# NVIDIA/vid2vid

Measured on AMD Instinct MI355X. Metric: synthesized frames/sec (Vid2VidModelG.inference, 512x256), higher is better.
Workload: dtype bf16; 1 GPU; label2city 512x256 inference, n_scales_spatial=1, --fg --use_instance, ngf=128 n_blocks=9 (411.3M params random-init, 2115 GFLOP/frame as dense convolutions, of which the 2 one-hot label stems (266 GFLOP dense) run as exact weight gather-sums), batch 1 per sequence, 1 sequence per GPU; launches_per_frame=113, hipgraph=True, graph_lanes=3, paired_launches=True, tile_selection=profiles/tune_cache.json, world_size=1, parallelism=replicas x1 (independent sequences, no collective), output_finite=True

## Files before the change

### include/v2v_hip.h

```cpp
#ifndef V2V_HIP_H
#define V2V_HIP_H

#include <stdint.h>

#ifdef __cplusplus
extern "C" {
#endif

#define V2V_EINVAL (-1)

#define V2V_F32  0
#define V2V_BF16 1

#define V2V_PAD_ZERO    0
#define V2V_PAD_REFLECT 1

#define V2V_ACT_NONE    0
#define V2V_ACT_RELU    1
#define V2V_ACT_LEAKY   2
#define V2V_ACT_TANH    3
#define V2V_ACT_SIGMOID 4

#define V2V_OUT_RAW_F32_NHWC 0
#define V2V_OUT_ACT_NHWC     1
// ... 376 lines not shown
int       v2v_plan_run(v2v_plan* p, void* stream);
int       v2v_plan_instantiate_graph(v2v_plan* p, void* stream);
int       v2v_plan_launch_graph(v2v_plan* p, void* stream);
int       v2v_plan_segment_program(const v2v_plan* p, int32_t* steps, int32_t max_steps, int32_t* seg_of_op, int32_t n_ops);
int       v2v_plan_profile(v2v_plan* p, void* stream, float* ms, int32_t n);
int       v2v_plan_timeline(v2v_plan* p, void* stream, float* t0_ms, float* t1_ms, int32_t* lanes, int32_t n);
int       v2v_plan_timeline_graph(v2v_plan* p, void* stream, float* t0_ms, float* t1_ms, int32_t* lanes, int32_t n);
const char* v2v_plan_op_name(const v2v_plan* p, int32_t i);
int       v2v_plan_op_lane(const v2v_plan* p, int32_t i);
int       v2v_plan_set_label(v2v_plan* p, const char* label);
const char* v2v_plan_op_label(const v2v_plan* p, int32_t i);
int       v2v_plan_set_lane(int32_t lane);
int       v2v_plan_lane_wait(int32_t waiter, int32_t signal);

int v2v_tensor2im(const float* x, uint8_t* out, int32_t C, int32_t H, int32_t W, int32_t normalize, void* stream);
int v2v_frames_u8(const float* frames, uint8_t* out, const int32_t* mode, const int32_t* row_slot, int32_t K, int32_t S,
                  int32_t C, int32_t H, int32_t W, int32_t normalize, void* stream);
int v2v_label_image(const void* labels, const void* inst, int32_t in_u8, const uint8_t* cmap, int32_t label_nc, uint8_t* out,
                    const int32_t* mode, const int32_t* row_slot, int32_t K, int32_t S, int32_t T, int32_t H, int32_t W,
                    void* stream);
int v2v_tensor2flow(const float* flow, uint8_t* out, uint32_t* range_ws, int32_t H, int32_t W, void* stream);
int v2v_tensor2label(const float* x, uint8_t* out, const uint8_t* cmap, int32_t n_label, int32_t C, int32_t H, int32_t W,
                     void* stream);

int     v2v_label_codes(const void* labels, const void* inst, int32_t in_u8, uint8_t* codes, int32_t T, int32_t H, int32_t W,
                        int32_t label_nc, void* stream);
int64_t v2v_onehot_conv_table_bytes(int32_t cin, int32_t cout, int32_t dtype, int32_t slice, int32_t T, int32_t label_nc);
int     v2v_onehot_conv_pack_weights(const float* w, void* table, int32_t cin, int32_t cout, int32_t dtype, int32_t slice,
                                     int32_t T, int32_t label_nc, void* stream);
int     v2v_onehot_conv_stats_rows(int32_t H, int32_t W);
int     v2v_onehot_conv7x7(const void* labels, const void* inst, int32_t in_u8, const void* table, const float* bias,
                           float* out, float* stats, int32_t T, int32_t H, int32_t W, int32_t label_nc,
                           int32_t cout, int32_t cout_stride, int32_t dtype, int32_t slice, void* stream);
typedef struct v2v_onehot_norm {
    int32_t* counter;
    const float* gamma;
    const float* beta;
    float* scale_shift;
    float* running_mean;
    float* running_var;
    float eps, momentum;
    int64_t count;
} v2v_onehot_norm;
int     v2v_onehot_conv7x7_norm(const void* labels, const void* inst, int32_t in_u8, const void* table, const float* bias,
                                float* out, float* stats, int32_t T, int32_t H, int32_t W, int32_t label_nc,
                                int32_t cout, int32_t cout_stride, int32_t dtype, int32_t slice, const v2v_onehot_norm* fin,
                                void* stream);
int     v2v_onehot_conv7x7_batch(const void* labels, const void* inst, int32_t in_u8, const void* table, const float* bias,
                                 float* out, float* stats, int32_t N, int32_t T, int32_t H, int32_t W, int32_t label_nc,
                                 int32_t cout, int32_t cout_stride, int32_t dtype, int32_t slice, void* stream);
int     v2v_onehot_conv_ppt(int32_t N, int32_t T, int32_t H, int32_t W, int32_t label_nc, int32_t has_inst,
                            int32_t cout, int32_t dtype, int32_t slice);

int v2v_memcpy_d2d(void* dst, const void* src, int64_t bytes, void* stream);

int         v2v_set_dry_run(int32_t on);
int         v2v_get_dry_run(void);

int         v2v_version(void);
const char* v2v_last_error(void);
int         v2v_device_status(int32_t clear);
int         v2v_device_info(int32_t* cus, int32_t* lds_per_cu, int64_t* hbm_bytes, char* arch, int32_t arch_len);

#ifdef __cplusplus
}
#endif
#endif
```

### vid2vid_amd/csrc/label_image.hip

```cpp
#include "v2v_internal.h"

namespace v2v {

struct LabelImageArgs {
    const void* labels; const void* inst; const unsigned char* cmap; unsigned char* out;
    const int* mode; const int* row_slot;
    int K, S, T, H, W, label_nc, planes;
};

static constexpr int LABEL_IMAGE_GRID_CAP = 256;

__device__ __forceinline__ int label_image_row(const LabelImageArgs& a, int s) {
    for (int k = 0; k < a.K; ++k) {
        if ((a.row_slot ? a.row_slot[k] : k) != s) continue;
        const int m = a.mode ? a.mode[k] : 0;
        if (m == 0 || m == 1) return k;
    }
    return -1;
}

template <typename T, int R>
__device__ __forceinline__ void load_run(const T* p, int n, T (&v)[R]) {
    constexpr int BYTES = R * (int)sizeof(T);
    constexpr int VB = BYTES < 16 ? 4 : 16;
    static_assert(BYTES % VB == 0, "whole vectors");
    if (n == R && (reinterpret_cast<uintptr_t>(p) & (VB - 1)) == 0) {
        if constexpr (VB == 4) {
            const unsigned w = *reinterpret_cast<const unsigned*>(p);
            __builtin_memcpy(v, &w, 4);
        } else {
            uint4 w[BYTES / 16];
#pragma unroll
            for (int i = 0; i < BYTES / 16; ++i) w[i] = reinterpret_cast<const uint4*>(p)[i];
            __builtin_memcpy(v, w, BYTES);
        }
    } else {
#pragma unroll
        for (int i = 0; i < R; ++i) v[i] = i < n ? p[i] : T(0);
    }
}

template <typename LT, typename IT, int R>
__global__ __launch_bounds__(256) void label_image_kernel(const LabelImageArgs a) {
    constexpr int NW = 3 * R / 4;
    constexpr unsigned BLACK = 255;
    __shared__ unsigned pal[256];
    {
        const int c = threadIdx.x;
        unsigned w = 0;
        if (c < a.label_nc) w = a.cmap[3 * c] | ((unsigned)a.cmap[3 * c + 1] << 8) | ((unsigned)a.cmap[3 * c + 2] << 16);
        pal[c] = w;
    }
    __syncthreads();
    const int s = blockIdx.y;
    const int row = label_image_row(a, s);
    const long long hw = (long long)a.H * a.W;
    const int rpr = (a.W + R - 1) / R;
    const long long runs = (long long)a.H * rpr;
    const long long stride = (long long)gridDim.x * blockDim.x;
    const long long frame = ((long long)(row < 0 ? 0 : row) * a.T + (a.T - 1)) * hw;
    const LT* const labels = reinterpret_cast<const LT*>(a.labels) + frame;
    const IT* const inst = a.inst ? reinterpret_cast<const IT*>(a.inst) + frame : nullptr;
    unsigned char* const out = a.out + (long long)s * hw * 3;
    for (long long r = (long long)blockIdx.x * blockDim.x + threadIdx.x; r < runs; r += stride) {
        const int y = (int)(r / rpr);
        const int x0 = (int)(r - (long long)y * rpr) * R;
        const int n = a.W - x0 < R ? a.W - x0 : R;
        const long long p0 = (long long)y * a.W + x0;
        unsigned w[NW + 1];
#pragma unroll
        for (int j = 0; j <= NW; ++j) w[j] = 0u;
        if (row >= 0) {
            LT lab[R];
            load_run<LT, R>(labels + p0, n, lab);
            int idx[R];
            bool outside = false;
#pragma unroll
            for (int i = 0; i < R; ++i) {
                idx[i] = (int)lab[i];
                outside |= i < n && (idx[i] < 0 || idx[i] >= a.label_nc);
            }
            bool edge[R];
#pragma unroll
            for (int i = 0; i < R; ++i) edge[i] = false;
            if (inst && outside) {
                IT c[R], up[R], dn[R];
                load_run<IT, R>(inst + p0, n, c);
                const bool has_up = y > 0, has_dn = y + 1 < a.H, has_l = x0 > 0, has_r = x0 + n < a.W;
                if (has_up) load_run<IT, R>(inst + p0 - a.W, n, up);
                if (has_dn) load_run<IT, R>(inst + p0 + a.W, n, dn);
                const IT lft = has_l ? inst[p0 - 1] : IT(0);
                const IT rgt = has_r ? inst[p0 + n] : IT(0);
#pragma unroll
                for (int i = 0; i < R; ++i) {
                    bool e = false;
                    if (i > 0) e |= c[i - 1] != c[i];
                    else       e |= has_l && lft != c[0];
                    if (i + 1 < n)       e |= c[(i + 1) % R] != c[i];
                    else if (i + 1 == n) e |= has_r && rgt != c[i];
                    if (has_up) e |= up[i] != c[i];
                    if (has_dn) e |= dn[i] != c[i];
                    edge[i] = e;
                }
            }
#pragma unroll
            for (int i = 0; i < R; ++i) {
                unsigned k;
                if (a.planes == 1) k = idx[i] == 0 ? BLACK : 0u;
                else if (idx[i] >= 0 && idx[i] < a.label_nc) k = (unsigned)idx[i];
                else k = edge[i] ? BLACK : 0u;
                const unsigned col = i < n ? pal[k] : 0u;
                const int word = (3 * i) >> 2, sh = ((3 * i) & 3) * 8;
                w[word] |= col << sh;
                if (sh > 8) w[word + 1] |= col >> (32 - sh);
            }
        }
        unsigned char* const dst = out + p0 * 3;
        const int nbytes = 3 * n;
        const uintptr_t addr = reinterpret_cast<uintptr_t>(dst);
        if (R == 16 && n == R && (addr & 15) == 0) {
#pragma unroll
            for (int j = 0; j < NW / 4; ++j)
                reinterpret_cast<uint4*>(dst)[j] = make_uint4(w[4 * j], w[4 * j + 1], w[4 * j + 2], w[4 * j + 3]);
        } else {
            int head = (int)((4 - (addr & 3)) & 3);
            if (head > nbytes) head = nbytes;
#pragma unroll
            for (int b = 0; b < 3; ++b)
                if (b < head) dst[b] = (unsigned char)(w[0] >> (8 * b));
            const int nd = (nbytes - head) >> 2, tail = (nbytes - head) & 3;
            unsigned* const dw = reinterpret_cast<unsigned*>(dst + head);
#pragma unroll
            for (int j = 0; j < NW; ++j) {
                const unsigned v = __builtin_amdgcn_alignbyte(w[j + 1], w[j], (unsigned)head);
                if (j < nd) dw[j] = v;
                else if (j == nd) {
#pragma unroll
                    for (int b = 0; b < 3; ++b)
                        if (b < tail) dst[head + 4 * nd + b] = (unsigned char)(v >> (8 * b));
                }
            }
        }
    }
}

struct LabelImageOp : Op {
    LabelImageArgs a; int in_u8;
    template <typename LT, typename IT>
    void go(hipStream_t s) {
        const dim3 b(256);
        if (a.W >= 16) {
            long long gx = ceil_div((long long)a.H * ceil_div(a.W, 16), 256);
            if (gx > LABEL_IMAGE_GRID_CAP) gx = LABEL_IMAGE_GRID_CAP;
            hipLaunchKernelGGL((label_image_kernel<LT, IT, 16>), dim3((unsigned)gx, (unsigned)a.S), b, 0, s, a);
        } else {
            long long gx = ceil_div((long long)a.H * ceil_div(a.W, 4), 256);
            if (gx > LABEL_IMAGE_GRID_CAP) gx = LABEL_IMAGE_GRID_CAP;
            hipLaunchKernelGGL((label_image_kernel<LT, IT, 4>), dim3((unsigned)gx, (unsigned)a.S), b, 0, s, a);
        }
    }
    int launch(hipStream_t s) override {
        if (in_u8) go<unsigned char, int>(s);
        else       go<float, float>(s);
        return check_launch();
    }
    const char* name() const override { return "label_image"; }
};

static bool ranges_overlap(const void* p, long long pb, const void* q, long long qb) {
    const char* a = (const char*)p; const char* b = (const char*)q;
    return p && q && a < b + qb && b < a + pb;
}

}

using namespace v2v;

extern "C" int v2v_label_image(const void* labels, const void* inst, int32_t in_u8, const uint8_t* cmap, int32_t label_nc,
                               uint8_t* out, const int32_t* mode, const int32_t* row_slot, int32_t K, int32_t S, int32_t T,
                               int32_t H, int32_t W, void* stream) {
    if (!labels || !cmap || !out) { set_error("label_image: null pointer"); return V2V_EINVAL; }
    if (label_nc < 1 || label_nc > 255) {
        set_error("label_image: label_nc %d (1..255: the palette and its black entry are 256 words of LDS)", label_nc); return V2V_EINVAL;
    }
    if ((in_u8 != 0 && in_u8 != 1) || K < 1 || S < K || S > 65535 || T < 1 || H < 1 || W < 1 ||
        (long long)K * T * H * W > 0x7fffffffffffll) {
        set_error("label_image: bad argument (1 <= K <= S <= 65535 rows / images, T, H, W >= 1)"); return V2V_EINVAL;
    }
    if (!row_slot && K != S) { set_error("label_image: without row_slot row k is image k: K == S"); return V2V_EINVAL; }
    const int lsize = in_u8 ? 1 : 4;
    if ((((uintptr_t)labels & (lsize - 1)) | ((uintptr_t)inst & 3) | ((uintptr_t)mode & 3) | ((uintptr_t)row_slot & 3)) != 0) {
        set_error("label_image: misaligned buffer (fp32 labels, inst, mode and row_slot are 4-byte aligned)"); return V2V_EINVAL;
    }
    const long long hw = (long long)H * W;
    const long long out_bytes = (long long)S * hw * 3, in_elems = (long long)K * T * hw;
    if (ranges_overlap(out, out_bytes, labels, in_elems * lsize) || ranges_overlap(out, out_bytes, inst, in_elems * 4) ||
        ranges_overlap(out, out_bytes, cmap, 3ll * label_nc) || ranges_overlap(out, out_bytes, mode, 4ll * K) ||
        ranges_overlap(out, out_bytes, row_slot, 4ll * K)) {
        set_error("label_image: out must not overlap an input"); return V2V_EINVAL;
    }
    auto op = std::make_unique<LabelImageOp>();
    op->a = LabelImageArgs{labels, inst, cmap, out, mode, row_slot, K, S, T, H, W, label_nc, label_nc + (inst ? 1 : 0)};
    op->in_u8 = in_u8;
    return submit(std::move(op), stream);
}
```

### vid2vid_amd/csrc/pointwise.hip

```cpp
#include "v2v_internal.h"
#include "layout_vec.h"

namespace v2v {

static inline unsigned grid_for(long long n, int threads = 256, long long cap = 4096) {
    long long b = ceil_div(n, threads);
    if (b > cap) b = cap;
    if (b < 1) b = 1;
    return (unsigned)b;
}

struct EncodeArgs {
    const void* labels; const void* inst; void* out; float* mask;
    int T, H, W, label_nc, c_stride; const int* fg; int n_fg;
};

template <typename T, typename LT, typename IT>
__global__ __launch_bounds__(256) void encode_labels_kernel(const EncodeArgs a) {
    constexpr int VEC = ElemTraits<T>::VEC;
    const int vpr = a.c_stride / VEC;
    const long long hw = (long long)a.H * a.W;
    const long long nvec = hw * vpr;
    const int per_frame = a.label_nc + (a.inst ? 1 : 0);
    const long long stride = (long long)gridDim.x * blockDim.x;
// ... 275 lines not shown
            const int c = cv * VEC + q;
            vals[q] = c < a.C ? a.x[(n * a.C + c) * hw + pix] : 0.f;
        }
        store_vec(y, pixg * a.c_stride + cv * VEC, vals);
    }
}

template <typename T>
__global__ __launch_bounds__(256) void unpack_nhwc_to_nchw_kernel(const PackArgs2 a) {
    constexpr int VEC = ElemTraits<T>::VEC;
    const int vpr = (a.C + VEC - 1) / VEC;
    const long long hw = (long long)a.H * a.W;
    const long long npix = (long long)a.N * hw;
    const long long nvec = npix * vpr;
    const long long stride = (long long)gridDim.x * blockDim.x;
    const T* y = reinterpret_cast<const T*>(a.y);
    float* x = const_cast<float*>(a.x);
    for (long long v = (long long)blockIdx.x * blockDim.x + threadIdx.x; v < nvec; v += stride) {
        const long long pixg = v % npix;
        const int cv = (int)(v / npix);
        const long long n = pixg / hw, pix = pixg - n * hw;
        float vals[VEC];
        load_vec(y, pixg * a.c_stride + cv * VEC, vals);
#pragma unroll
        for (int q = 0; q < VEC; ++q) {
            const int c = cv * VEC + q;
            if (c < a.C) x[(n * a.C + c) * hw + pix] = vals[q];
        }
    }
}

struct LayoutOp : Op {
    PackArgs2 a; int dtype; bool pack;
    int launch(hipStream_t s) override {
        const int vec = dtype == V2V_BF16 ? 8 : 4;
        const long long n = (long long)a.N * a.H * a.W * (pack ? (a.c_stride / vec) : ((a.C + vec - 1) / vec));
        if (pack) {
            if (dtype == V2V_BF16) hipLaunchKernelGGL(pack_nchw_to_nhwc_kernel<bf16_t>, dim3(grid_for(n)), dim3(256), 0, s, a);
            else                   hipLaunchKernelGGL(pack_nchw_to_nhwc_kernel<float>, dim3(grid_for(n)), dim3(256), 0, s, a);
        } else {
            if (dtype == V2V_BF16) hipLaunchKernelGGL(unpack_nhwc_to_nchw_kernel<bf16_t>, dim3(grid_for(n)), dim3(256), 0, s, a);
            else                   hipLaunchKernelGGL(unpack_nhwc_to_nchw_kernel<float>, dim3(grid_for(n)), dim3(256), 0, s, a);
        }
        return check_launch();
    }
    const char* name() const override { return pack ? "pack_nchw_to_nhwc" : "unpack_nhwc_to_nchw"; }
};

struct PrologueArgs {
    const void* labels; const void* inst; unsigned char* codes; float* mask; const int* fg; int n_fg;
    const float* window; void* packed; float* last;
    int T, H, W, label_nc, win_C, c_stride, last_C;
    int N = 1;
};

template <typename T, typename LT, typename IT>
__device__ __forceinline__ void frame_prologue_row(const PrologueArgs& a, long long nb, long long wrow, unsigned block_dim,
                                                   unsigned grid_dim) {
    constexpr int VEC = ElemTraits<T>::VEC;
    const long long hw = (long long)a.H * a.W;
    const long long ncode = hw * a.T;
    const int vpr = a.window ? a.c_stride / VEC : 0;
    const long long total = ncode + hw * vpr;
    const long long stride = (long long)grid_dim * block_dim;
    const LT* labels = reinterpret_cast<const LT*>(a.labels) + nb * ncode;
    const IT* inst = a.inst ? reinterpret_cast<const IT*>(a.inst) + nb * ncode : nullptr;
    unsigned char* codes = a.codes + nb * ncode;
    float* mask = a.mask ? a.mask + nb * hw : nullptr;
    const float* window = a.window ? a.window + wrow * a.win_C * hw : nullptr;
    float* last = a.last ? a.last + nb * a.last_C * hw : nullptr;
    T* y = reinterpret_cast<T*>(a.packed) + nb * hw * a.c_stride;
    for (long long e = (long long)blockIdx.x * block_dim + threadIdx.x; e < total; e += stride) {
        if (e < ncode) {
            const long long t = e / hw, q = e - t * hw;
            const int lab = (int)labels[e];
            bool edge = false;
            if (inst) {
                const int py = (int)(q / a.W), px = (int)(q - (long long)py * a.W);
                const IT* ip = inst + t * hw;
                const IT ctr = ip[q];
                if (px > 0)       edge |= ip[q - 1] != ctr;
                if (px < a.W - 1) edge |= ip[q + 1] != ctr;
                if (py > 0)       edge |= ip[q - a.W] != ctr;
                if (py < a.H - 1) edge |= ip[q + a.W] != ctr;
            }
            codes[e] = (unsigned char)(((unsigned)lab < (unsigned)a.label_nc ? lab : 127) | (edge ? 128 : 0));
            if (mask && t == a.T - 1) {
                float m = 0.f;
                for (int i = 0; i < a.n_fg; ++i) m += (a.fg[i] == lab) ? 1.f : 0.f;
                mask[q] = fminf(fmaxf(m, 0.f), 1.f);
            }
        } else {
            const long long v = e - ncode;
            window_pack_item<T>(window, y, last, v % hw, (int)(v / hw), hw, a.win_C, a.c_stride, a.last_C);
        }
    }
}

template <typename T, typename LT, typename IT, bool BATCH>
__global__ __launch_bounds__(256) void frame_prologue_kernel(const PrologueArgs a) {
    const long long nb = BATCH ? (long long)blockIdx.y : 0ll;
    frame_prologue_row<T, LT, IT>(a, nb, nb, blockDim.x, gridDim.x);
}

struct PrologueOp : Op {
    PrologueArgs a; int dtype; int in_u8;
    int launch(hipStream_t s) override {
        const int vec = dtype == V2V_BF16 ? 8 : 4;
        const long long hw = (long long)a.H * a.W;
        const dim3 g(grid_for(hw * a.T + (a.window ? hw * (a.c_stride / vec) : 0)), (unsigned)a.N), b(256);
        if (a.N > 1) return go<true>(g, b, s);
        return go<false>(g, b, s);
    }
    template <bool BATCH> int go(dim3 g, dim3 b, hipStream_t s) {
        if (in_u8) {
            if (dtype == V2V_BF16) hipLaunchKernelGGL((frame_prologue_kernel<bf16_t, unsigned char, int, BATCH>), g, b, 0, s, a);
            else                   hipLaunchKernelGGL((frame_prologue_kernel<float, unsigned char, int, BATCH>), g, b, 0, s, a);
        } else {
            if (dtype == V2V_BF16) hipLaunchKernelGGL((frame_prologue_kernel<bf16_t, float, float, BATCH>), g, b, 0, s, a);
            else                   hipLaunchKernelGGL((frame_prologue_kernel<float, float, float, BATCH>), g, b, 0, s, a);
        }
        return check_launch();
    }
    const char* name() const override { return "frame_prologue"; }
};

struct ProloguePoolArgs { PrologueArgs p; const int* row_slot; int S; };

template <typename T, typename LT, typename IT>
__global__ __launch_bounds__(256) void frame_prologue_pool_kernel(const ProloguePoolArgs s) {
    const PrologueArgs& a = s.p;
    const int slot = s.row_slot[blockIdx.y];
    if (slot < 0 || slot >= s.S) return;
    __builtin_assume(a.window != nullptr);
    frame_prologue_row<T, LT, IT>(a, blockIdx.y, slot, blockDim.x, gridDim.x);
}

struct ProloguePoolOp : Op {
    ProloguePoolArgs a; int dtype; int in_u8;
    int launch(hipStream_t s) override {
        const int vec = dtype == V2V_BF16 ? 8 : 4;
        const long long hw = (long long)a.p.H * a.p.W;
        const dim3 g(grid_for(hw * a.p.T + hw * (a.p.c_stride / vec)), (unsigned)a.p.N), b(256);
        if (in_u8) {
            if (dtype == V2V_BF16) hipLaunchKernelGGL((frame_prologue_pool_kernel<bf16_t, unsigned char, int>), g, b, 0, s, a);
            else                   hipLaunchKernelGGL((frame_prologue_pool_kernel<float, unsigned char, int>), g, b, 0, s, a);
        } else {
            if (dtype == V2V_BF16) hipLaunchKernelGGL((frame_prologue_pool_kernel<bf16_t, float, float>), g, b, 0, s, a);
            else                   hipLaunchKernelGGL((frame_prologue_pool_kernel<float, float, float>), g, b, 0, s, a);
        }
        return check_launch();
    }
    const char* name() const override { return "frame_prologue_pool"; }
};

struct PoolArgs { const void* x; void* y; long long planes; int N, H, W, OH, OW, c_stride; };

__global__ __launch_bounds__(256) void avgpool_planar_kernel(const PoolArgs a) {
    const float* x = reinterpret_cast<const float*>(a.x);
    float* y = reinterpret_cast<float*>(a.y);
    const long long total = a.planes * a.OH * a.OW;
    const long long stride = (long long)gridDim.x * blockDim.x;
    for (long long e = (long long)blockIdx.x * blockDim.x + threadIdx.x; e < total; e += stride) {
        const int ox = (int)(e % a.OW);
        const long long t = e / a.OW;
        const int oy = (int)(t % a.OH);
        const long long pl = t / a.OH;
        const float* xp = x + pl * (long long)a.H * a.W;
        float s = 0.f; int cnt = 0;
#pragma unroll
        for (int dy = -1; dy <= 1; ++dy) {
            const int iy = 2 * oy + dy;
            if (iy < 0 || iy >= a.H) continue;
#pragma unroll
            for (int dx = -1; dx <= 1; ++dx) {
                const int ix = 2 * ox + dx;
                if (ix < 0 || ix >= a.W) continue;
                s += xp[(long long)iy * a.W + ix];
                ++cnt;
            }
        }
        y[e] = s / (float)cnt;
    }
}

template <typename T>
__global__ __launch_bounds__(256) void avgpool_nhwc_kernel(const PoolArgs a) {
    constexpr int VEC = ElemTraits<T>::VEC;
// ... 43 lines not shown
            pk.w = pack_bf16x2(s[6] / fc, s[7] / fc);
            *reinterpret_cast<uint4*>(o) = pk;
        }
    }
}

struct PoolOp : Op {
    PoolArgs a; int dtype; bool planar;
    int launch(hipStream_t s) override {
        if (planar) {
            hipLaunchKernelGGL(avgpool_planar_kernel, dim3(grid_for(a.planes * a.OH * a.OW)), dim3(256), 0, s, a);
        } else {
            const long long n = (long long)a.N * a.OH * a.OW * (a.c_stride / (dtype == V2V_BF16 ? 8 : 4));
            if (dtype == V2V_BF16) hipLaunchKernelGGL(avgpool_nhwc_kernel<bf16_t>, dim3(grid_for(n)), dim3(256), 0, s, a);
            else                   hipLaunchKernelGGL(avgpool_nhwc_kernel<float>, dim3(grid_for(n)), dim3(256), 0, s, a);
        }
        return check_launch();
    }
    const char* name() const override { return planar ? "avgpool3s2_planar" : "avgpool3s2_nhwc"; }
};

__device__ __forceinline__ float unnormalize(float coord, int size, int align_corners) {
    if (align_corners) return ((coord + 1.f) / 2.f) * (float)(size - 1);
    return ((coord + 1.f) * (float)size - 1.f) / 2.f;
}

__device__ __forceinline__ void bilinear_setup(float fx, float fy, float gxv, float gyv, int H, int W, int ac,
                                               int& x0, int& y0, float& wx, float& wy) {
    const float nx = gxv + fx / (((float)W - 1.0f) / 2.0f);
    const float ny = gyv + fy / (((float)H - 1.0f) / 2.0f);
    float ix = unnormalize(nx, W, ac), iy = unnormalize(ny, H, ac);
    ix = fminf((float)(W - 1), fmaxf(ix, 0.f));
    iy = fminf((float)(H - 1), fmaxf(iy, 0.f));
    const float fx0 = floorf(ix), fy0 = floorf(iy);
    x0 = (int)fx0; y0 = (int)fy0;
    wx = ix - fx0; wy = iy - fy0;
}

__device__ __forceinline__ float bilinear_fetch(const float* img, int H, int W, int x0, int y0, float wx, float wy) {
    const int x1 = x0 + 1, y1 = y0 + 1;
    const bool xin = x1 < W, yin = y1 < H;
    const float nw = img[(long long)y0 * W + x0];
    const float ne = xin ? img[(long long)y0 * W + x1] : 0.f;
    const float sw = yin ? img[(long long)y1 * W + x0] : 0.f;
    const float se = (xin && yin) ? img[(long long)y1 * W + x1] : 0.f;
    return nw * ((1.f - wx) * (1.f - wy)) + ne * (wx * (1.f - wy)) + sw * ((1.f - wx) * wy) + se * (wx * wy);
}

struct WarpArgs {
    float* img_raw; const float* flow; const float* weight; const float* prev; const float* fg; const float* mask;
    float* img_final; float* img_warp; const float* gx; const float* gy;
    int N, C, H, W, align_corners;
    float* roll = nullptr; int roll_slots = 0;
};

__device__ __forceinline__ void warp_blend_pixel(const WarpArgs& a, long long n, long long pix, bool do_warp, float* win) {
    const long long hw = (long long)a.H * a.W;
    const int y = (int)(pix / a.W), x = (int)(pix - (long long)y * a.W);
    int x0 = 0, y0 = 0; float wx = 0.f, wy = 0.f;
    float wgt = 1.f;
    if (do_warp) {
        const float fx = a.flow[(n * 2 + 0) * hw + pix], fy = a.flow[(n * 2 + 1) * hw + pix];
        bilinear_setup(fx, fy, a.gx[x], a.gy[y], a.H, a.W, a.align_corners, x0, y0, wx, wy);
        wgt = a.weight[n * hw + pix];
    }
    const float m = a.fg ? a.mask[n * hw + pix] : 0.f;
    for (int c = 0; c < a.C; ++c) {
        const long long o = (n * a.C + c) * hw + pix;
        float raw = a.img_raw[o];
        float fin = raw;
        if (do_warp) {
            const float wv = bilinear_fetch(a.prev + (n * a.C + c) * hw, a.H, a.W, x0, y0, wx, wy);
            if (a.img_warp) a.img_warp[o] = wv;
            fin = raw * wgt + wv * (1.f - wgt);
        }
        if (a.fg) {
            const float f = a.fg[o];
            fin = f * m + fin * (1.f - m);
            raw = f * m + raw * (1.f - m);
            a.img_raw[o] = raw;
        }
        a.img_final[o] = fin;
        if (win) {
            float* w = win + c * hw + pix;
            const long long slot = (long long)a.C * hw;
            for (int k = 0; k + 1 < a.roll_slots; ++k) w[k * slot] = w[(k + 1) * slot];
            w[(a.roll_slots - 1) * slot] = fin;
        }
    }
}

__device__ __forceinline__ float* warp_row_window(const WarpArgs& a, long long n) {
    return a.roll ? a.roll + n * a.roll_slots * a.C * a.H * a.W : nullptr;
}

template <bool ROLLB>
__global__ __launch_bounds__(256) void warp_blend_kernel(const WarpArgs a) {
    const long long hw = (long long)a.H * a.W;
    const long long total = (long long)a.N * hw;
    const long long stride = (long long)gridDim.x * blockDim.x;
    for (long long e = (long long)blockIdx.x * blockDim.x + threadIdx.x; e < total; e += stride) {
        const long long n = e / hw;
        warp_blend_pixel(a, n, e - n * hw, a.flow != nullptr, ROLLB ? warp_row_window(a, n) : a.roll);
    }
}

struct WarpOp : Op {
    WarpArgs a;
    int launch(hipStream_t s) override {
        const dim3 g(grid_for((long long)a.N * a.H * a.W));
        if (a.roll && a.N > 1) hipLaunchKernelGGL(warp_blend_kernel<true>, g, dim3(256), 0, s, a);
        else                   hipLaunchKernelGGL(warp_blend_kernel<false>, g, dim3(256), 0, s, a);
        return check_launch();
    }
    const char* name() const override { return "warp_blend"; }
};

struct WarpSlotArgs { WarpArgs w; const int* mode; };

__global__ __launch_bounds__(256) void warp_blend_slots_kernel(const WarpSlotArgs s) {
    const WarpArgs& a = s.w;
    const long long hw = (long long)a.H * a.W;
    const long long total = (long long)a.N * hw;
    const long long stride = (long long)gridDim.x * blockDim.x;
    for (long long e = (long long)blockIdx.x * blockDim.x + threadIdx.x; e < total; e += stride) {
        const long long n = e / hw, pix = e - n * hw;
        const int md = s.mode[n];
        if (md != 0 && md != 1) {
            for (int c = 0; c < a.C; ++c) a.img_final[(n * a.C + c) * hw + pix] = 0.f;
            continue;
        }
        warp_blend_pixel(a, n, pix, a.flow != nullptr && md == 0, warp_row_window(a, n));
    }
}

struct WarpSlotsOp : Op {
    WarpSlotArgs a;
    int launch(hipStream_t s) override {
        hipLaunchKernelGGL(warp_blend_slots_kernel, dim3(grid_for((long long)a.w.N * a.w.H * a.w.W)), dim3(256), 0, s, a);
        return check_launch();
    }
    const char* name() const override { return "warp_blend_slots"; }
};

struct WindowRollArgs { float* window; const float* frame; const int* mode; long long frame_elems; int N, slots; };

__global__ __launch_bounds__(256) void window_roll_slots_kernel(const WindowRollArgs a) {
    const long long total = (long long)a.N * a.frame_elems;
    const long long stride = (long long)gridDim.x * blockDim.x;
    for (long long e = (long long)blockIdx.x * blockDim.x + threadIdx.x; e < total; e += stride) {
        const long long n = e / a.frame_elems, r = e - n * a.frame_elems;
        const int md = a.mode[n];
        if (md != 0 && md != 1) continue;
        float* w = a.window + n * a.slots * a.frame_elems + r;
        for (int k = 0; k + 1 < a.slots; ++k) w[k * a.frame_elems] = w[(k + 1) * a.frame_elems];
        w[(a.slots - 1) * a.frame_elems] = a.frame[e];
    }
}

struct WindowRollOp : Op {
    WindowRollArgs a;
    int launch(hipStream_t s) override {
        hipLaunchKernelGGL(window_roll_slots_kernel, dim3(grid_for((long long)a.N * a.frame_elems)), dim3(256), 0, s, a);
        return check_launch();
    }
// ... 613 lines not shown
extern "C" int v2v_avgpool3s2_nhwc(const void* x, void* y, int32_t N, int32_t H, int32_t W, int32_t c_stride,
                                   int32_t dtype, void* stream) {
    if (!x || !y || c_stride % (dtype == V2V_BF16 ? 8 : 4) != 0) { set_error("avgpool: null pointer or a channel stride that is not whole 16-byte vectors"); return V2V_EINVAL; }
    auto op = std::make_unique<PoolOp>();
    op->a = PoolArgs{x, y, 0, N, H, W, (H - 1) / 2 + 1, (W - 1) / 2 + 1, c_stride}; op->planar = false; op->dtype = dtype;
    return submit(std::move(op), stream);
}

extern "C" int v2v_warp_blend(float* img_raw, const float* flow, const float* weight, const float* prev,
                              const float* fg, const float* mask, float* img_final, float* img_warp,
                              const float* gx, const float* gy,
                              int32_t N, int32_t C, int32_t H, int32_t W, int32_t align_corners, void* stream) {
    if (!img_raw || !img_final || (flow && (!weight || !prev || !gx || !gy)) || (fg && !mask)) {
        set_error("warp_blend: bad argument"); return V2V_EINVAL;
    }
    auto op = std::make_unique<WarpOp>();
    op->a = WarpArgs{img_raw, flow, weight, prev, fg, mask, img_final, img_warp, gx, gy, N, C, H, W, align_corners};
    return submit(std::move(op), stream);
}

static bool warp_roll_args_ok(const char* who, const WarpArgs& a, bool need_window, long long win_rows, const char* what) {
    if (!a.img_raw || !a.img_final || (a.flow && (!a.weight || !a.prev || !a.gx || !a.gy)) || (a.fg && !a.mask) ||
        (need_window && !a.roll) || (a.roll && a.roll_slots < 1) || a.N < 1 || win_rows < 1 || a.C < 1 || a.H < 1 || a.W < 1) {
        set_error("%s: bad argument", who); return false;
    }
    if (!a.roll) return true;
    const float* wend = a.roll + win_rows * a.roll_slots * a.C * a.H * a.W;
    const long long frame = (long long)a.N * a.C * a.H * a.W;
    auto overlaps = [&](const float* p) { return p && p + frame > a.roll && p < wend; };
    if (overlaps(a.prev) || overlaps(a.img_final) || overlaps(a.img_raw) || overlaps(a.fg)) {
        set_error("%s: the %s must not overlap the gather source or the frame buffers", who, what); return false;
    }
    return true;
}

extern "C" int v2v_warp_blend_roll(float* img_raw, const float* flow, const float* weight, const float* prev,
                                   const float* fg, const float* mask, float* img_final, float* img_warp,
                                   const float* gx, const float* gy, float* window, int32_t slots,
                                   int32_t C, int32_t H, int32_t W, int32_t align_corners, void* stream) {
    return v2v_warp_blend_roll_batch(img_raw, flow, weight, prev, fg, mask, img_final, img_warp, gx, gy, window, slots, 1, C, H, W,
                                     align_corners, stream);
}

extern "C" int v2v_warp_blend_roll_batch(float* img_raw, const float* flow, const float* weight, const float* prev,
                                         const float* fg, const float* mask, float* img_final, float* img_warp,
                                         const float* gx, const float* gy, float* window, int32_t slots,
                                         int32_t N, int32_t C, int32_t H, int32_t W, int32_t align_corners, void* stream) {
    auto op = std::make_unique<WarpOp>();
    op->a = WarpArgs{img_raw, flow, weight, prev, fg, mask, img_final, img_warp, gx, gy, N, C, H, W, align_corners, window, slots};
    if (!warp_roll_args_ok("warp_blend_roll", op->a, true, N, "rolled window")) return V2V_EINVAL;
    return submit(std::move(op), stream);
}

extern "C" int v2v_warp_blend_slots(float* img_raw, const float* flow, const float* weight, const float* prev,
                                    const float* fg, const float* mask, float* img_final, float* img_warp,
                                    const float* gx, const float* gy, float* window, int32_t slots, const int32_t* mode,
                                    int32_t N, int32_t C, int32_t H, int32_t W, int32_t align_corners, void* stream) {
    if (!mode) { set_error("warp_blend_slots: null mode"); return V2V_EINVAL; }
    auto op = std::make_unique<WarpSlotsOp>();
    op->a.w = WarpArgs{img_raw, flow, weight, prev, fg, mask, img_final, img_warp, gx, gy, N, C, H, W, align_corners, window, slots};
    op->a.mode = mode;
    if (!warp_roll_args_ok("warp_blend_slots", op->a.w, false, N, "rolled window")) return V2V_EINVAL;
    if (!window) op->a.w.roll_slots = 0;
    return submit(std::move(op), stream);
}

extern "C" int v2v_window_roll_slots(float* window, const float* frame, const int32_t* mode, int32_t N, int32_t slots,
                                     int32_t C, int32_t H, int32_t W, void* stream) {
    if (!mode) { set_error("window_roll_slots: null mode"); return V2V_EINVAL; }
    if (!window || !frame || N < 1 || slots < 1 || C < 1 || H < 1 || W < 1) {
        set_error("window_roll_slots: bad argument"); return V2V_EINVAL;
    }
    const long long elems = (long long)C * H * W;
    if (frame + N * elems > window && frame < window + (long long)N * slots * elems) {
        set_error("window_roll_slots: the frame must not overlap the window"); return V2V_EINVAL;
    }
    auto op = std::make_unique<WindowRollOp>();
    op->a = WindowRollArgs{window, frame, mode, elems, N, slots};
    return submit(std::move(op), stream);
}

extern "C" int v2v_warp_blend_pool(float* img_raw, const float* flow, const float* weight, const float* prev,
                                   const float* fg, const float* mask, float* img_final, float* img_warp,
                                   const float* gx, const float* gy, float* window, int32_t slots, const int32_t* mode,
                                   const int32_t* row_slot, int32_t K, int32_t S, int32_t C, int32_t H, int32_t W,
                                   int32_t align_corners, void* stream) {
    if (!mode || !row_slot) { set_error("warp_blend_pool: null %s", !mode ? "mode" : "row_slot"); return V2V_EINVAL; }
    auto op = std::make_unique<WarpPoolOp>();
    op->a.w = WarpArgs{img_raw, flow, weight, prev, fg, mask, img_final, img_warp, gx, gy, K, C, H, W, align_corners, window, slots};
    op->a.mode = mode; op->a.row_slot = row_slot; op->a.S = S;
    if (K > 65535) { set_error("warp_blend_pool: bad argument"); return V2V_EINVAL; }
    if (!warp_roll_args_ok("warp_blend_pool", op->a.w, true, S, "pool")) return V2V_EINVAL;
    return submit(std::move(op), stream);
}

static int window_pool_copy(const char* what, float* dst, const float* src, bool scatter, const int32_t* row_slot, int32_t K,
                            int32_t S, int32_t slots, int32_t C, int32_t H, int32_t W, void* stream) {
    if (!dst || !src || !row_slot || K < 1 || K > 65535 || S < 1 || slots < 1 || C < 1 || H < 1 || W < 1) {
        set_error("%s: null pointer or bad argument", what); return V2V_EINVAL;
    }
    const long long elems = (long long)slots * C * H * W;
    const float* dense = scatter ? src : dst; const float* pool = scatter ? dst : src;
    if (dense + K * elems > pool && dense < pool + S * elems) {
        set_error("%s: dense and pool must not overlap", what); return V2V_EINVAL;
    }
    auto op = std::make_unique<WindowPoolOp>();
    op->a = WindowPoolArgs{dst, src, row_slot, elems, K, S}; op->scatter = scatter;
    return submit(std::move(op), stream);
}

extern "C" int v2v_window_gather_pool(float* dense, const float* pool, const int32_t* row_slot, int32_t K, int32_t S, int32_t slots,
                                      int32_t C, int32_t H, int32_t W, void* stream) {
    return window_pool_copy("window_gather_pool", dense, pool, false, row_slot, K, S, slots, C, H, W, stream);
}

extern "C" int v2v_window_scatter_pool(float* pool, const float* dense, const int32_t* row_slot, int32_t K, int32_t S, int32_t slots,
                                       int32_t C, int32_t H, int32_t W, void* stream) {
    return window_pool_copy("window_scatter_pool", pool, dense, true, row_slot, K, S, slots, C, H, W, stream);
}

static bool prologue_args_ok(const char* who, const PrologueArgs& a, int in_u8, int dtype) {
    const int vec = dtype == V2V_BF16 ? 8 : 4;
    if (!a.labels || !a.codes || a.T < 1 || a.H < 1 || a.W < 1 || a.label_nc < 1 || a.label_nc > 126 || (in_u8 != 0 && in_u8 != 1) ||
        (dtype != V2V_F32 && dtype != V2V_BF16) || a.n_fg < 0 || (a.mask && a.n_fg > 0 && !a.fg) ||
        (in_u8 ? ((uintptr_t)a.inst & 3) != 0 : (((uintptr_t)a.labels | (uintptr_t)a.inst) & 3) != 0)) {
        set_error("%s: bad argument (label_nc <= 126)", who); return false;
    }
    if (a.window && (!a.packed || a.win_C < 1 || a.c_stride % vec != 0 || a.win_C > a.c_stride || ((uintptr_t)a.packed & 15) != 0 ||
                     (a.last && (a.last_C < 1 || a.last_C > a.win_C)))) {
        set_error("%s: bad window pack argument", who); return false;
    }
    return true;
}

extern "C" int v2v_frame_prologue(const void* labels, const void* inst, int32_t in_u8, uint8_t* codes, float* mask,
                                  const int32_t* fg_labels_dev, int32_t n_fg, int32_t T, int32_t H, int32_t W, int32_t label_nc,
                                  const float* window, int32_t win_C, void* packed, int32_t c_stride, float* last, int32_t last_C,
                                  int32_t dtype, void* stream) {
    return v2v_frame_prologue_batch(labels, inst, in_u8, codes, mask, fg_labels_dev, n_fg, 1, T, H, W, label_nc, window, win_C, packed,
                                    c_stride, last, last_C, dtype, stream);
}

extern "C" int v2v_frame_prologue_batch(const void* labels, const void* inst, int32_t in_u8, uint8_t* codes, float* mask,
                                        const int32_t* fg_labels_dev, int32_t n_fg, int32_t N, int32_t T, int32_t H, int32_t W,
                                        int32_t label_nc, const float* window, int32_t win_C, void* packed, int32_t c_stride,
                                        float* last, int32_t last_C, int32_t dtype, void* stream) {
    if (N < 1 || N > 65535) { set_error("frame_prologue: bad sample count %d", N); return V2V_EINVAL; }
    auto op = std::make_unique<PrologueOp>();
    op->a = PrologueArgs{labels, inst, codes, mask, fg_labels_dev, n_fg, window, packed, last,
                         T, H, W, label_nc, win_C, c_stride, last_C, N};
    op->dtype = dtype; op->in_u8 = in_u8;
    if (!prologue_args_ok("frame_prologue", op->a, in_u8, dtype)) return V2V_EINVAL;
    if (!window) op->a.packed = op->a.last = nullptr;
    return submit(std::move(op), stream);
}

extern "C" int v2v_frame_prologue_pool(const void* labels, const void* inst, int32_t in_u8, uint8_t* codes, float* mask,
                                       const int32_t* fg_labels_dev, int32_t n_fg, int32_t K, int32_t T, int32_t H, int32_t W,
                                       int32_t label_nc, const float* window, int32_t S, const int32_t* row_slot, int32_t win_C,
                                       void* packed, int32_t c_stride, float* last, int32_t last_C, int32_t dtype, void* stream) {
    if (!row_slot || !window) { set_error("frame_prologue_pool: null %s", !row_slot ? "row_slot" : "window"); return V2V_EINVAL; }
    if (K < 1 || K > 65535 || S < 1) { set_error("frame_prologue_pool: bad row count %d / pool size %d", K, S); return V2V_EINVAL; }
    auto op = std::make_unique<ProloguePoolOp>();
    op->a.p = PrologueArgs{labels, inst, codes, mask, fg_labels_dev, n_fg, window, packed, last,
                           T, H, W, label_nc, win_C, c_stride, last_C, K};
    op->a.row_slot = row_slot; op->a.S = S;
    op->dtype = dtype; op->in_u8 = in_u8;
    if (!prologue_args_ok("frame_prologue_pool", op->a.p, in_u8, dtype)) return V2V_EINVAL;
    return submit(std::move(op), stream);
}

extern "C" int v2v_resample_flow(const float* img, const float* flow, float* out, const float* gx, const float* gy,
                                 int32_t N, int32_t C, int32_t H, int32_t W, int32_t align_corners, void* stream) {
    if (!img || !flow || !out || !gx || !gy) { set_error("resample_flow: null"); return V2V_EINVAL; }
    auto op = std::make_unique<ResampleOp>();
    op->a = ResampleArgs{img, flow, out, gx, gy, N, C, H, W, align_corners};
    return submit(std::move(op), stream);
}

extern "C" int v2v_add_nhwc(const void* a, const void* b, void* y, int64_t n_elems, int32_t dtype, void* stream) {
    const int vec = dtype == V2V_BF16 ? 8 : 4;
    if (!a || !b || !y || n_elems % vec != 0) { set_error("add: bad argument"); return V2V_EINVAL; }
    auto op = std::make_unique<AddOp>();
    op->a = AddArgs{a, b, y, n_elems / vec}; op->dtype = dtype;
    return submit(std::move(op), stream);
}

extern "C" int v2v_fg_mask_nhwc(const void* x, float* mask, int64_t P, int32_t c_stride, int32_t base_ch,
                                const int32_t* fg_labels_dev, int32_t n_fg, int32_t dtype, void* stream) {
    if (!x || !mask || !fg_labels_dev || n_fg <= 0) { set_error("fg_mask: bad argument"); return V2V_EINVAL; }
    auto op = std::make_unique<FgMaskOp>();
    op->a = FgMaskArgs{x, mask, P, c_stride, base_ch, fg_labels_dev, n_fg}; op->dtype = dtype;
    return submit(std::move(op), stream);
}

extern "C" int v2v_pack_concat_nhwc(const float* x0, int32_t C0, const float* x1, int32_t C1, float scale1, void* y,
                                    int32_t N, int32_t H, int32_t W, int32_t c_stride, int32_t dtype, void* stream) {
    const int vec = dtype == V2V_BF16 ? 8 : 4;
    if (!x0 || !y || (C1 > 0 && !x1) || c_stride % vec != 0 || C0 + C1 > c_stride) { set_error("pack_concat: bad argument"); return V2V_EINVAL; }
    auto op = std::make_unique<Pack2Op>();
    op->a = Pack2Args{x0, x1, y, N, C0, C1 > 0 ? C1 : 0, H, W, c_stride, scale1}; op->dtype = dtype;
    return submit(std::move(op), stream);
}

extern "C" int v2v_unpack_channels_nchw(const void* y, float* x, int32_t N, int32_t C, int32_t H, int32_t W,
                                        int32_t c_stride, int32_t c_offset, int32_t dtype, void* stream) {
// ... 45 lines not shown
```

### vid2vid_amd/csrc/v2v_internal.h

```cpp
#pragma once
#include <hip/hip_runtime.h>
#include <stdint.h>
#include <string>
#include <vector>
#include <memory>
#include "../../include/v2v_hip.h"

namespace v2v {

typedef __bf16 bf16_t;
typedef __attribute__((ext_vector_type(8)))  __bf16 bf16x8;
typedef __attribute__((ext_vector_type(4)))  float  f32x4;
typedef __attribute__((ext_vector_type(16))) float  f32x16;

__device__ __forceinline__ float bf16_bits_to_f32(unsigned short b) {
    return __uint_as_float(((unsigned)b) << 16);
}
typedef __attribute__((ext_vector_type(2))) float v2v_f32x2;
typedef __attribute__((ext_vector_type(2))) __bf16 v2v_bf16x2;
__device__ __forceinline__ unsigned pack_bf16x2(float lo, float hi) {
    const v2v_f32x2 v = {lo, hi};
    const v2v_bf16x2 r = __builtin_convertvector(v, v2v_bf16x2);
    return __builtin_bit_cast(unsigned, r);
}
// ... 23 lines not shown
}

__device__ __forceinline__ float apply_act(float v, int act, float param) {
    switch (act) {
        case V2V_ACT_RELU:    return v > 0.f ? v : 0.f;
        case V2V_ACT_LEAKY:   return v > 0.f ? v : v * param;
        case V2V_ACT_TANH:    return tanhf(v);
        case V2V_ACT_SIGMOID: return 1.f / (1.f + expf(-v));
        default:              return v;
    }
}

template <int U>
__device__ __forceinline__ void sum_stat_rows(const float* stats, long long col2, long long row_stride, int ph, int PH, int total,
                                              double& s1, double& s2) {
    const unsigned long long* const base = reinterpret_cast<const unsigned long long*>(stats + col2);
    const long long rs = row_stride / 2;
    int r = ph;
    for (; r + (U - 1) * PH < total; r += U * PH) {
        unsigned long long b[U];
#pragma unroll
        for (int u = 0; u < U; ++u)
            b[u] = __hip_atomic_load(base + (long long)(r + u * PH) * rs, __ATOMIC_RELAXED, __HIP_MEMORY_SCOPE_AGENT);
#pragma unroll
        for (int u = 0; u < U; ++u) {
            s1 += (double)__uint_as_float((unsigned)(b[u] & 0xffffffffull));
            s2 += (double)__uint_as_float((unsigned)(b[u] >> 32));
        }
    }
    for (; r < total; r += PH) {
        const unsigned long long b = __hip_atomic_load(base + (long long)r * rs, __ATOMIC_RELAXED, __HIP_MEMORY_SCOPE_AGENT);
        s1 += (double)__uint_as_float((unsigned)(b & 0xffffffffull));
        s2 += (double)__uint_as_float((unsigned)(b >> 32));
    }
}

struct Op {
    virtual ~Op() {}
    virtual int launch(hipStream_t s) = 0;
    virtual const char* name() const = 0;
    std::string label;
    int lane = 0;
};

int submit(std::unique_ptr<Op> op, void* stream);
void set_error(const char* fmt, ...);

inline int check_launch() {
    hipError_t e = hipGetLastError();
    if (e != hipSuccess) { set_error("HIP launch failed: %s", hipGetErrorString(e)); return (int)e; }
    return 0;
}

inline int64_t round_up(int64_t a, int64_t b) { return (a + b - 1) / b * b; }
inline int64_t ceil_div(int64_t a, int64_t b) { return (a + b - 1) / b; }

}
```

### vid2vid_amd/csrc/vgg_ops.hip

```cpp
#include "v2v_internal.h"

namespace v2v {

static inline unsigned grid_for(long long n, int threads = 256, long long cap = 8192) {
    long long g = (n + threads - 1) / threads;
    if (g < 1) g = 1;
    if (g > cap) g = cap;
    return (unsigned)g;
}

struct MaxPoolArgs {
    const void* x; const void* dy; void* y;
    int N, H, W, OH, OW, c_stride;
};

template <typename T>
__global__ __launch_bounds__(256) void maxpool2_nhwc_kernel(const MaxPoolArgs a) {
    constexpr int VEC = ElemTraits<T>::VEC;
    const T* x = reinterpret_cast<const T*>(a.x);
    T* y = reinterpret_cast<T*>(a.y);
    const int vpr = a.c_stride / VEC;
    const long long total = (long long)a.N * a.OH * a.OW * vpr;
    const long long stride = (long long)gridDim.x * blockDim.x;
    for (long long e = (long long)blockIdx.x * blockDim.x + threadIdx.x; e < total; e += stride) {
// ... 63 lines not shown
        const int vec = dtype == V2V_BF16 ? 8 : 4;
        const long long n = (long long)a.N * (bwd ? (long long)a.H * a.W : (long long)a.OH * a.OW) * (a.c_stride / vec);
        if (!bwd) {
            if (dtype == V2V_BF16) hipLaunchKernelGGL(maxpool2_nhwc_kernel<bf16_t>, dim3(grid_for(n)), dim3(256), 0, s, a);
            else                   hipLaunchKernelGGL(maxpool2_nhwc_kernel<float>, dim3(grid_for(n)), dim3(256), 0, s, a);
        } else {
            if (dtype == V2V_BF16) hipLaunchKernelGGL(maxpool2_nhwc_bwd_kernel<bf16_t>, dim3(grid_for(n)), dim3(256), 0, s, a);
            else                   hipLaunchKernelGGL(maxpool2_nhwc_bwd_kernel<float>, dim3(grid_for(n)), dim3(256), 0, s, a);
        }
        return check_launch();
    }
    const char* name() const override { return bwd ? "maxpool2_nhwc_backward" : "maxpool2_nhwc"; }
};

struct AvgPool2Args { const float* x; float* y; long long planes; int H, W, OH, OW; };

__global__ __launch_bounds__(256) void avgpool2_planar_kernel(const AvgPool2Args a) {
    const long long total = a.planes * a.OH * a.OW;
    const long long stride = (long long)gridDim.x * blockDim.x;
    for (long long e = (long long)blockIdx.x * blockDim.x + threadIdx.x; e < total; e += stride) {
        const int ow = (int)(e % a.OW);
        long long t = e / a.OW;
        const int oh = (int)(t % a.OH);
        const long long p = t / a.OH;
        const float* r0 = a.x + (p * a.H + 2 * oh) * a.W + 2 * ow;
        const float* r1 = r0 + a.W;
        a.y[e] = (r0[0] + r0[1] + r1[0] + r1[1]) * 0.25f;
    }
}

__global__ __launch_bounds__(256) void avgpool2_planar_bwd_kernel(const AvgPool2Args a) {
    const long long total = a.planes * a.H * a.W;
    const long long stride = (long long)gridDim.x * blockDim.x;
    for (long long e = (long long)blockIdx.x * blockDim.x + threadIdx.x; e < total; e += stride) {
        const int w = (int)(e % a.W);
        long long t = e / a.W;
        const int h = (int)(t % a.H);
        const long long p = t / a.H;
        const int oh = h >> 1, ow = w >> 1;
        a.y[e] = (oh < a.OH && ow < a.OW) ? a.x[(p * a.OH + oh) * a.OW + ow] * 0.25f : 0.f;
    }
}

struct AvgPool2Op : Op {
    AvgPool2Args a; bool bwd;
    int launch(hipStream_t s) override {
        if (!bwd) hipLaunchKernelGGL(avgpool2_planar_kernel, dim3(grid_for(a.planes * a.OH * a.OW)), dim3(256), 0, s, a);
        else      hipLaunchKernelGGL(avgpool2_planar_bwd_kernel, dim3(grid_for(a.planes * a.H * a.W)), dim3(256), 0, s, a);
        return check_launch();
    }
    const char* name() const override { return bwd ? "avgpool2_planar_backward" : "avgpool2_planar"; }
};

struct OneHotArgs { const void* labels; const void* inst; float* out; int H, W, label_nc; long long in_stride = 0; int N = 1; };

template <typename LT, typename IT, bool BATCH>
__global__ __launch_bounds__(256) void onehot_planar_kernel(const OneHotArgs a) {
    const long long hw = (long long)a.H * a.W;
    const long long stride = (long long)gridDim.x * blockDim.x;
    const long long nb = BATCH ? (long long)blockIdx.y : 0ll;
    const LT* labels = reinterpret_cast<const LT*>(a.labels) + nb * a.in_stride;
    const IT* inst = a.inst ? reinterpret_cast<const IT*>(a.inst) + nb * a.in_stride : nullptr;
    float* out = a.out + nb * (a.label_nc + (inst ? 1 : 0)) * hw;
    for (long long p = (long long)blockIdx.x * blockDim.x + threadIdx.x; p < hw; p += stride) {
        const int lab = (int)labels[p];
        for (int c = 0; c < a.label_nc; ++c) out[(long long)c * hw + p] = (c == lab) ? 1.f : 0.f;
        if (inst) {
            const int y = (int)(p / a.W), x = (int)(p - (long long)y * a.W);
            const IT v = inst[p];
            bool e = false;
            if (x > 0)       e |= inst[p - 1] != v;
            if (x + 1 < a.W) e |= inst[p + 1] != v;
            if (y > 0)       e |= inst[p - a.W] != v;
            if (y + 1 < a.H) e |= inst[p + a.W] != v;
            out[(long long)a.label_nc * hw + p] = e ? 1.f : 0.f;
        }
    }
}

struct OneHotOp : Op {
    OneHotArgs a; int in_u8 = 0;
    int launch(hipStream_t s) override {
        const dim3 g(grid_for((long long)a.H * a.W), (unsigned)a.N), b(256);
        if (a.N > 1) {
            if (in_u8) hipLaunchKernelGGL((onehot_planar_kernel<unsigned char, int, true>), g, b, 0, s, a);
            else       hipLaunchKernelGGL((onehot_planar_kernel<float, float, true>), g, b, 0, s, a);
        } else {
            if (in_u8) hipLaunchKernelGGL((onehot_planar_kernel<unsigned char, int, false>), g, b, 0, s, a);
            else       hipLaunchKernelGGL((onehot_planar_kernel<float, float, false>), g, b, 0, s, a);
        }
        return check_launch();
    }
    const char* name() const override { return "onehot_planar"; }
};

}

using namespace v2v;

extern "C" int v2v_maxpool2_nhwc(const void* x, void* y, int32_t N, int32_t H, int32_t W, int32_t c_stride,
                                 int32_t dtype, void* stream) {
    const int vec = dtype == V2V_BF16 ? 8 : 4;
    if (!x || !y || N <= 0 || H < 2 || W < 2 || c_stride <= 0 || c_stride % vec) { set_error("maxpool2: bad argument"); return V2V_EINVAL; }
    auto op = std::make_unique<MaxPoolOp>();
    op->a = MaxPoolArgs{x, nullptr, y, N, H, W, H / 2, W / 2, c_stride}; op->dtype = dtype; op->bwd = false;
    return submit(std::move(op), stream);
}

extern "C" int v2v_maxpool2_nhwc_backward(const void* dy, const void* x, void* dx, int32_t N, int32_t H, int32_t W,
                                          int32_t c_stride, int32_t dtype, void* stream) {
    const int vec = dtype == V2V_BF16 ? 8 : 4;
    if (!dy || !x || !dx || N <= 0 || H < 2 || W < 2 || c_stride <= 0 || c_stride % vec) { set_error("maxpool2_backward: bad argument"); return V2V_EINVAL; }
    auto op = std::make_unique<MaxPoolOp>();
    op->a = MaxPoolArgs{x, dy, dx, N, H, W, H / 2, W / 2, c_stride}; op->dtype = dtype; op->bwd = true;
    return submit(std::move(op), stream);
}

extern "C" int v2v_avgpool2_planar(const float* x, float* y, int64_t planes, int32_t H, int32_t W, void* stream) {
    if (!x || !y || planes <= 0 || H < 2 || W < 2) { set_error("avgpool2: bad argument"); return V2V_EINVAL; }
    auto op = std::make_unique<AvgPool2Op>();
    op->a = AvgPool2Args{x, y, planes, H, W, H / 2, W / 2}; op->bwd = false;
    return submit(std::move(op), stream);
}

extern "C" int v2v_avgpool2_planar_backward(const float* dy, float* dx, int64_t planes, int32_t H, int32_t W, void* stream) {
    if (!dy || !dx || planes <= 0 || H < 2 || W < 2) { set_error("avgpool2_backward: bad argument"); return V2V_EINVAL; }
    auto op = std::make_unique<AvgPool2Op>();
    op->a = AvgPool2Args{dy, dx, planes, H, W, H / 2, W / 2}; op->bwd = true;
    return submit(std::move(op), stream);
}

extern "C" int v2v_onehot_planar(const float* labels, const float* inst, float* out, int32_t H, int32_t W,
                                 int32_t label_nc, void* stream) {
    if (!labels || !out || H <= 0 || W <= 0 || label_nc <= 0) { set_error("onehot_planar: bad argument"); return V2V_EINVAL; }
    auto op = std::make_unique<OneHotOp>();
    op->a = OneHotArgs{labels, inst, out, H, W, label_nc};
    return submit(std::move(op), stream);
}

extern "C" int v2v_onehot_planar_u8(const uint8_t* labels, const int32_t* inst, float* out, int32_t H, int32_t W,
                                    int32_t label_nc, void* stream) {
    if (!labels || !out || H <= 0 || W <= 0 || label_nc <= 0 || label_nc > 256) { set_error("onehot_planar_u8: bad argument"); return V2V_EINVAL; }
    auto op = std::make_unique<OneHotOp>();
    op->a = OneHotArgs{labels, inst, out, H, W, label_nc}; op->in_u8 = 1;
    return submit(std::move(op), stream);
}

extern "C" int v2v_onehot_planar_batch(const void* labels, const void* inst, int32_t in_u8, float* out, int32_t N, int64_t in_stride,
                                       int32_t H, int32_t W, int32_t label_nc, void* stream) {
    if (!labels || !out || N <= 0 || N > 65535 || H <= 0 || W <= 0 || label_nc <= 0 || (in_u8 != 0 && in_u8 != 1) || (in_u8 && label_nc > 256) ||
        in_stride < (int64_t)H * W) {
        set_error("onehot_planar_batch: bad argument"); return V2V_EINVAL;
    }
    auto op = std::make_unique<OneHotOp>();
    op->a = OneHotArgs{labels, inst, out, H, W, label_nc}; op->a.in_stride = in_stride; op->a.N = N; op->in_u8 = in_u8;
    return submit(std::move(op), stream);
}
```

### vid2vid_amd/csrc/visual_ops.hip

```cpp
#include "v2v_internal.h"

namespace v2v {

static inline unsigned grid_for(long long n, int threads = 256, long long cap = 4096) {
    long long b = (n + threads - 1) / threads;
    if (b > cap) b = cap;
    if (b < 1) b = 1;
    return (unsigned)b;
}

struct Im2Args { const float* x; unsigned char* out; int C, H, W, normalize; };

__global__ __launch_bounds__(256) void tensor2im_kernel(const Im2Args a) {
    const long long hw = (long long)a.H * a.W;
    const long long total = hw * a.C;
    const long long stride = (long long)gridDim.x * blockDim.x;
    for (long long e = (long long)blockIdx.x * blockDim.x + threadIdx.x; e < total; e += stride) {
        const long long pix = e / a.C;
        const int c = (int)(e - pix * a.C);
        const float x = a.x[(long long)c * hw + pix];
        float v = a.normalize ? ((x + 1.f) / 2.f) * 255.f : x * 255.f;
        v = fminf(fmaxf(v, 0.f), 255.f);
        a.out[e] = (unsigned char)(int)v;
    }
}

struct FramesU8Args {
    const float* x; unsigned char* out; const int* mode; const int* row_slot;
    long long hw; int K, S, C, normalize;
};

__device__ __forceinline__ unsigned frames_u8_byte(float x, int normalize) {
    float v = normalize ? ((x + 1.f) / 2.f) * 255.f : x * 255.f;
    v = fminf(fmaxf(v, 0.f), 255.f);
    return (unsigned)(unsigned char)(int)v;
}

__device__ __forceinline__ int frames_u8_row(const FramesU8Args& a, int s) {
    for (int k = 0; k < a.K; ++k) {
        if ((a.row_slot ? a.row_slot[k] : k) != s) continue;
        const int m = a.mode ? a.mode[k] : 0;
        if (m == 0 || m == 1) return k;
    }
    return -1;
}

template <int CC>
__global__ __launch_bounds__(256) void frames_u8_wide_kernel(const FramesU8Args a) {
    const int s = blockIdx.y;
    const int row = frames_u8_row(a, s);
    const long long nvec = a.hw >> 2;
    const long long stride = (long long)gridDim.x * blockDim.x;
    unsigned* const out = reinterpret_cast<unsigned*>(a.out + (long long)s * a.hw * CC);
    const float* const x = a.x + (long long)(row < 0 ? 0 : row) * CC * a.hw;
    for (long long v = (long long)blockIdx.x * blockDim.x + threadIdx.x; v < nvec; v += stride) {
        unsigned w[CC];
#pragma unroll
        for (int j = 0; j < CC; ++j) w[j] = 0u;
        if (row >= 0) {
#pragma unroll
            for (int c = 0; c < CC; ++c) {
                const f32x4 p = *reinterpret_cast<const f32x4*>(x + (long long)c * a.hw + 4 * v);
#pragma unroll
                for (int i = 0; i < 4; ++i) {
                    const int byte = i * CC + c;
                    w[byte >> 2] |= frames_u8_byte(p[i], a.normalize) << (8 * (byte & 3));
                }
            }
        }
#pragma unroll
        for (int j = 0; j < CC; ++j) out[v * CC + j] = w[j];
    }
}

__global__ __launch_bounds__(256) void frames_u8_scalar_kernel(const FramesU8Args a) {
    const int s = blockIdx.y;
    const int row = frames_u8_row(a, s);
    const long long total = a.hw * a.C;
    const long long stride = (long long)gridDim.x * blockDim.x;
    unsigned char* const out = a.out + (long long)s * total;
    const float* const x = a.x + (long long)(row < 0 ? 0 : row) * total;
    for (long long e = (long long)blockIdx.x * blockDim.x + threadIdx.x; e < total; e += stride) {
        unsigned char b = 0;
        if (row >= 0) {
            const long long pix = e / a.C;
            const int c = (int)(e - pix * a.C);
            b = (unsigned char)frames_u8_byte(x[(long long)c * a.hw + pix], a.normalize);
        }
        out[e] = b;
    }
}

struct Lab2Args { const float* x; unsigned char* out; const unsigned char* cmap; int C, H, W, n; };

__global__ __launch_bounds__(256) void tensor2label_kernel(const Lab2Args a) {
    const long long hw = (long long)a.H * a.W;
    const long long stride = (long long)gridDim.x * blockDim.x;
    for (long long p = (long long)blockIdx.x * blockDim.x + threadIdx.x; p < hw; p += stride) {
        int lab = -1;
        if (a.C > 1) {
            float best = a.x[p];
            lab = 0;
            for (int c = 1; c < a.C; ++c) {
                const float v = a.x[(long long)c * hw + p];
                if (v > best) { best = v; lab = c; }
            }
        } else {
            const float v = a.x[p];
            const int iv = (int)v;
            lab = ((float)iv == v) ? iv : -1;
        }
        unsigned char r = 0, g = 0, b = 0;
        if (lab >= 0 && lab < a.n) { r = a.cmap[lab * 3]; g = a.cmap[lab * 3 + 1]; b = a.cmap[lab * 3 + 2]; }
        a.out[p * 3 + 0] = r; a.out[p * 3 + 1] = g; a.out[p * 3 + 2] = b;
    }
}

struct FlowImArgs { const float* flow; unsigned char* out; unsigned* range; int H, W; };

__global__ __launch_bounds__(256) void flow_range_kernel(const FlowImArgs a) {
    const long long hw = (long long)a.H * a.W;
    const long long stride = (long long)gridDim.x * blockDim.x;
    unsigned lo = 0x7f800000u, hi = 0u;
    for (long long p = (long long)blockIdx.x * blockDim.x + threadIdx.x; p < hw; p += stride) {
        const float fx = a.flow[p], fy = a.flow[hw + p];
        const unsigned m = __float_as_uint(sqrtf(fx * fx + fy * fy));
        lo = m < lo ? m : lo; hi = m > hi ? m : hi;
    }
    for (int off = 32; off > 0; off >>= 1) {
        const unsigned l2 = __shfl_down(lo, off), h2 = __shfl_down(hi, off);
        lo = l2 < lo ? l2 : lo; hi = h2 > hi ? h2 : hi;
    }
    if ((threadIdx.x & 63) == 0) { atomicMin(a.range, lo); atomicMax(a.range + 1, hi); }
}

__global__ __launch_bounds__(256) void flow_colour_kernel(const FlowImArgs a) {
    const long long hw = (long long)a.H * a.W;
    const long long stride = (long long)gridDim.x * blockDim.x;
    const float mn = __uint_as_float(a.range[0]), mx = __uint_as_float(a.range[1]);
    const float scale = (mx - mn) > 1.1920929e-07f ? 255.f / (mx - mn) : 0.f;
    for (long long p = (long long)blockIdx.x * blockDim.x + threadIdx.x; p < hw; p += stride) {
        const float fx = a.flow[p], fy = a.flow[hw + p];
        float ang = atan2f(fy, fx);
        if (ang < 0.f) ang += 6.283185307179586f;
        const float mag = sqrtf(fx * fx + fy * fy);
        const int H8 = (int)(ang * 180.f / 3.14159265358979323846f / 2.f) & 255;
        const int V8 = (int)((mag - mn) * scale) & 255;
        const float v = (float)V8 * (1.f / 255.f);
        float h = (float)H8 * (6.f / 180.f);
        int sector = (int)floorf(h);
        h -= (float)sector;
        sector = ((sector % 6) + 6) % 6;
        const float tab[4] = {v, 0.f, v * (1.f - h), v * h};
        const int sd[6][3] = {{1, 3, 0}, {1, 0, 2}, {3, 0, 1}, {0, 2, 1}, {0, 1, 3}, {2, 1, 0}};
        const float b = tab[sd[sector][0]], g = tab[sd[sector][1]], r = tab[sd[sector][2]];
        a.out[p * 3 + 0] = (unsigned char)__float2int_rn(fminf(fmaxf(r * 255.f, 0.f), 255.f));
        a.out[p * 3 + 1] = (unsigned char)__float2int_rn(fminf(fmaxf(g * 255.f, 0.f), 255.f));
        a.out[p * 3 + 2] = (unsigned char)__float2int_rn(fminf(fmaxf(b * 255.f, 0.f), 255.f));
    }
}

struct FlowImOp : Op {
    FlowImArgs a;
    int launch(hipStream_t s) override {
        const unsigned init[2] = {0x7f800000u, 0u};
        if (hipMemcpyAsync(a.range, init, sizeof(init), hipMemcpyHostToDevice, s) != hipSuccess) return check_launch();
        const dim3 g(grid_for((long long)a.H * a.W, 256, 1024)), b(256);
        hipLaunchKernelGGL(flow_range_kernel, g, b, 0, s, a);
        hipLaunchKernelGGL(flow_colour_kernel, g, b, 0, s, a);
        return check_launch();
    }
    const char* name() const override { return "tensor2flow"; }
};

struct Im2Op : Op {
    Im2Args a;
    int launch(hipStream_t s) override {
        hipLaunchKernelGGL(tensor2im_kernel, dim3(grid_for((long long)a.H * a.W * a.C)), dim3(256), 0, s, a);
        return check_launch();
    }
    const char* name() const override { return "tensor2im"; }
};
struct FramesU8Op : Op {
    FramesU8Args a;
    bool wide;
    int launch(hipStream_t s) override {
        const dim3 b(256);
        if (wide) {
            const dim3 g(grid_for(a.hw >> 2, 256, 1024), (unsigned)a.S);
            switch (a.C) {
                case 1: hipLaunchKernelGGL(frames_u8_wide_kernel<1>, g, b, 0, s, a); break;
                case 2: hipLaunchKernelGGL(frames_u8_wide_kernel<2>, g, b, 0, s, a); break;
                case 3: hipLaunchKernelGGL(frames_u8_wide_kernel<3>, g, b, 0, s, a); break;
                default: hipLaunchKernelGGL(frames_u8_wide_kernel<4>, g, b, 0, s, a); break;
            }
        } else {
            hipLaunchKernelGGL(frames_u8_scalar_kernel, dim3(grid_for(a.hw * a.C, 256, 1024), (unsigned)a.S), b, 0, s, a);
        }
        return check_launch();
    }
    const char* name() const override { return "frames_u8"; }
};
struct Lab2Op : Op {
    Lab2Args a;
    int launch(hipStream_t s) override {
        hipLaunchKernelGGL(tensor2label_kernel, dim3(grid_for((long long)a.H * a.W)), dim3(256), 0, s, a);
        return check_launch();
    }
    const char* name() const override { return "tensor2label"; }
};

}

using namespace v2v;

extern "C" int v2v_tensor2im(const float* x, uint8_t* out, int32_t C, int32_t H, int32_t W, int32_t normalize, void* stream) {
    if (!x || !out || C < 1 || C > 3 || H < 1 || W < 1) { set_error("tensor2im: bad argument (1..3 planes)"); return V2V_EINVAL; }
    auto op = std::make_unique<Im2Op>();
    op->a = Im2Args{x, out, C, H, W, normalize};
    return submit(std::move(op), stream);
}

extern "C" int v2v_frames_u8(const float* frames, uint8_t* out, const int32_t* mode, const int32_t* row_slot, int32_t K, int32_t S,
                             int32_t C, int32_t H, int32_t W, int32_t normalize, void* stream) {
    if (!frames || !out || K < 1 || S < K || S > 65535 || C < 1 || C > 4 || H < 1 || W < 1) {
        set_error("frames_u8: bad argument (1 <= K <= S <= 65535 rows / images, 1..4 planes)"); return V2V_EINVAL;
    }
    if (!row_slot && K != S) { set_error("frames_u8: without row_slot row k is image k: K == S"); return V2V_EINVAL; }
    const long long hw = (long long)H * W;
    const unsigned char* const fb = reinterpret_cast<const unsigned char*>(frames);
    if (fb + 4 * hw * C * K > out && fb < out + hw * C * S) { set_error("frames_u8: out must not overlap frames"); return V2V_EINVAL; }
    auto op = std::make_unique<FramesU8Op>();
    op->a = FramesU8Args{frames, out, mode, row_slot, hw, K, S, C, normalize};
    op->wide = hw % 4 == 0 && reinterpret_cast<uintptr_t>(frames) % 16 == 0 && reinterpret_cast<uintptr_t>(out) % 4 == 0;
    return submit(std::move(op), stream);
}

extern "C" int v2v_tensor2label(const float* x, uint8_t* out, const uint8_t* cmap, int32_t n_label, int32_t C, int32_t H, int32_t W,
                                void* stream) {
    if (!x || !out || !cmap || C < 1 || H < 1 || W < 1 || n_label < 1) { set_error("tensor2label: bad argument"); return V2V_EINVAL; }
    auto op = std::make_unique<Lab2Op>();
    op->a = Lab2Args{x, out, cmap, C, H, W, n_label};
    return submit(std::move(op), stream);
}

extern "C" int v2v_tensor2flow(const float* flow, uint8_t* out, uint32_t* range_ws, int32_t H, int32_t W, void* stream) {
    if (!flow || !out || !range_ws || H < 1 || W < 1) { set_error("tensor2flow: bad argument"); return V2V_EINVAL; }
    auto op = std::make_unique<FlowImOp>();
    op->a = FlowImArgs{flow, out, range_ws, H, W};
    return submit(std::move(op), stream);
}
```

### vid2vid_amd/engine.py

```python
import contextlib
import ctypes as C
import json
import math
import os
import sys

import torch
import torch.nn as nn

from . import lib as L
from .lib import lib, check, ConvDesc
from . import tile_search as TS
from .tile_search import (TILE_CFGS, PATCH_CFGS, S2_CFGS, T2_CFGS, S7_CFGS, ABLATION_TILES, PAIR_TILES, BWD_PATCH_TILES,
                          ONE_TILES, PERSISTENT_TILES, ONE_FIN, EXP_TILES, HEAD_TILE, C8_TILE, ROWSUM_TILE, tile_korder,
                          is_patch_tile, _flag, _cfg3)

_TORCH_DTYPE = {L.F32: torch.float32, L.BF16: torch.bfloat16}


def _ptr(t):
    return None if t is None else C.c_void_p(t.data_ptr())


_HAS_GPU = []
# ... 262 lines not shown
    @property
    def weight(self):
        w = self.src.weight.detach().float()
        cin = w.shape[0]
        w3 = torch.zeros(2, 32, 2, 16, 3, 3, dtype=torch.float32, device=w.device)
        for b in range(2):
            for e in range(2):
                for kxp, kx in ((1, e + 1 - 2 * b), (2, 3 + e - 2 * b), (0, e - 1 - 2 * b)):
                    if 0 <= kx <= 2:
                        w3[b, :cin, e, :, :, kxp] = w[:, :, :, kx]
        return w3.view(64, 32, 3, 3)

    @property
    def bias(self):
        return None if self.src.bias is None else torch.cat([self.src.bias.detach(), self.src.bias.detach()], 0)


class PackedOneHot:

    def __init__(self, eng, mod, slice_, T, label_nc):
        self.mod = mod
        self.cout, self.cin = mod.weight.shape[0], mod.weight.shape[1]
        self.dtype, self.slice, self.T, self.label_nc = eng.dtype, slice_, T, label_nc
        n = lib.v2v_onehot_conv_table_bytes(self.cin, self.cout, self.dtype, slice_, T, label_nc)
        if n <= 0:
            raise RuntimeError("onehot_conv_table_bytes(%d, %d) failed" % (self.cin, self.cout))
        self.buf = torch.empty(n, dtype=torch.uint8, device=eng.device)
        self.bias = None
        self.version = None
        self.refresh()

    def refresh(self, force=False):
        w = self.mod.weight
        box = getattr(w, "_v2v_epoch", None)
        ver = (w._version, w.data_ptr(), None if self.mod.bias is None else self.mod.bias._version, _PARAM_EPOCH[0],
               0 if box is None else box[0])
        if not force and ver == self.version:
            return
        w32 = w.detach()
        if w32.dtype != torch.float32 or not w32.is_contiguous():
            w32 = w32.float().contiguous()
        check(lib.v2v_onehot_conv_pack_weights(_ptr(w32), _ptr(self.buf), self.cin, self.cout, self.dtype, self.slice,
                                               self.T, self.label_nc, _stream()),
              "onehot_conv_pack_weights")
        self.bias = None if self.mod.bias is None else self.mod.bias.detach().float().contiguous()
        self.version = ver


class Plan:

    def __init__(self):
        self.h = C.c_void_p(lib.v2v_plan_create())
        self.keep = []
        self.graph_ready = False

    def __enter__(self):
        check(lib.v2v_plan_begin_record(self.h), "plan_begin_record")
        return self

    def __exit__(self, *exc):
        check(lib.v2v_plan_end_record(self.h), "plan_end_record")
        return False

    def label(self, text):
        lib.v2v_plan_set_label(self.h, text.encode())

    @property
    def num_ops(self):
        return lib.v2v_plan_num_ops(self.h)

    def run(self):
        check(lib.v2v_plan_run(self.h, _stream()), "plan_run")

    def instantiate_graph(self):
        check(lib.v2v_plan_instantiate_graph(self.h, _stream()), "plan_instantiate_graph")
        self.graph_ready = True

    def launch(self):
        if self.graph_ready:
            check(lib.v2v_plan_launch_graph(self.h, _stream()), "plan_launch_graph")
        else:
            self.run()

    def profile(self):
        n = self.num_ops
        ms = (C.c_float * n)()
        check(lib.v2v_plan_profile(self.h, _stream(), ms, n), "plan_profile")
        out = []
        for i in range(n):
            out.append((lib.v2v_plan_op_name(self.h, i).decode(), lib.v2v_plan_op_label(self.h, i).decode(), ms[i]))
        return out

    def timeline(self, graph=True):
        n = self.num_ops
        t0, t1, ln = (C.c_float * n)(), (C.c_float * n)(), (C.c_int32 * n)()
        fn = lib.v2v_plan_timeline_graph if graph else lib.v2v_plan_timeline
        check(fn(self.h, _stream(), t0, t1, ln, n), "plan_timeline")
        return [(lib.v2v_plan_op_name(self.h, i).decode(), lib.v2v_plan_op_label(self.h, i).decode(), int(ln[i]), t0[i], t1[i])
                for i in range(n)]

    def __del__(self):
        try:
            lib.v2v_plan_destroy(self.h)
        except Exception:
            pass


FUSE_FINALIZE_MAX_PIXELS = 32768
PREFETCH_DIST = 12


FIN_ONEHOT_OFFSET = 256 + 64 * 128
FIN_TAG_OFFSET = FIN_ONEHOT_OFFSET + 256
FIN_COUNTER_WORDS = FIN_TAG_OFFSET + 128


class Engine:

    def __init__(self, device, dtype=L.F32, align_corners=False, record_only=False, x3=False):
        self.device = torch.device(device)
        self.x3 = bool(x3) and dtype == L.F32
        self._x3_engine = None
        self._x3_convs = {}
        self.record_only = record_only
        if self.device.type != "cuda" and not record_only:
            raise RuntimeError("vid2vid_amd runs on MI355X only (got device %s); there is no CPU path" % device)
        if record_only:
            lib.v2v_set_dry_run(1)
        elif lib.v2v_get_dry_run():
            raise RuntimeError("v2v dry-run mode is on (a record-only Engine was created in this process): call "
                               "vid2vid_amd.networks.set_record_only(False) before creating a GPU engine")
        self.dtype = dtype
        self.tdtype = _TORCH_DTYPE[dtype]
        self.align_corners = align_corners
        self._packed = {}
        self._label_cmaps = {}
        self._packed_onehot = {}
        self.onehot_stem = bool(int(os.environ.get("V2V_ONEHOT_STEM", "1")))
        self.onehot_slice = int(os.environ.get("V2V_ONEHOT_SLICE", "0"))
        self.fused_norm = bool(int(os.environ.get("V2V_FUSED_NORM", "1")))
        self.raw_bf16 = bool(int(os.environ.get("V2V_RAW_BF16", "0")))
        self.raw_bf16_one = os.environ.get("V2V_RAW_BF16_ONE", "1") != "0"
        self.rowsum_heads = bool(int(os.environ.get("V2V_HEAD_ROWSUM", "1")))
        self._fused_norm_wgs = None
        self.merge_heads = bool(int(os.environ.get("V2V_MERGE_HEADS", "1")))
        self._merged_heads = {}
        self._scratch = {}
        self._grids = {}
        self._zero_page = None
        self._fin_counters = {}
        self._sk_counters = {}
        self._lane = 0
        self._sset = 0
        self.per_stream = False
        self.last_rows_per_sample = 0
        self.twin_enabled = False
        self.pair_override = None
        if os.environ.get("V2V_PAIR_TILE"):
            self.pair_override = tuple(int(v) for v in os.environ["V2V_PAIR_TILE"].split(","))
        self.lanes_enabled = False
        self._thrash = None
        self.pair_tune_log = {}
        self.wgrad_stream_on = os.environ.get("V2V_WGRAD_STREAM", "1") != "0"
        self._wgrad_stream = None
        self._wgrad_join_queued = False
        self.repack_async_on = os.environ.get("V2V_REPACK_ASYNC", "1") != "0"
        self._repack_event = None
        import weakref
        _ENGINES.append(weakref.ref(self))
        self.plan = None
        self.conv_log = []
        self.tile_override = {}
        for item in os.environ.get("V2V_TILE_OVERRIDE", "").split(";"):
            if ":" in item:
                k, v = item.split(":")
                self.tile_override[tuple(int(x) for x in k.split(","))] = tuple(int(x) for x in v.split(","))
        self.autotune = False
        self._tuned = {}
        self.bwd_tile_override = {}
        self._tune_alts = {}
        self._tune_wide = {}
        self._tune_cache_path = os.environ.get("V2V_TUNE_CACHE", "")
        if self._tune_cache_path and os.path.exists(self._tune_cache_path):
            try:
                with open(self._tune_cache_path) as f:
                    for k, v in json.load(f).get(str(dtype), {}).items():
                        self._tuned[tuple(int(x) for x in k.split(","))] = tuple(v)
            except (OSError, ValueError):
                pass
        self.update_running_stats = False
        self.fused_finalize = True
        self.fused_finalize2 = bool(int(os.environ.get("V2V_FIN2", "0")))
        self.last_finalized = False
        self.ablate = 0

    def empty_act(self, N, H, W, C):
        t = torch.empty((N, H, W, pad_channels(C, self.dtype)), dtype=self.tdtype, device=self.device)
        self._keep(t)
        return Act(t, C)

    def zeros_act(self, N, H, W, C):
        a = self.empty_act(N, H, W, C)
        a.t.zero_()
        return a

    def empty_f32(self, *shape):
        t = torch.empty(shape, dtype=torch.float32, device=self.device)
        self._keep(t)
        return t

    def scratch(self, name, numel, dtype=torch.float32, zero=False):
        key = (name, dtype, self._lane, self._sset)
        t = self._scratch.get(key)
        if t is None or t.numel() < numel:
            if self.plan is not None and t is not None and not self.record_only:
                raise RuntimeError("scratch '%s' must not grow while a plan is recording" % name)
            t = (torch.zeros if zero else torch.empty)(int(numel), dtype=dtype, device=self.device)
            self._scratch[key] = t
        self._keep(t)
        return t

    def reserve_scratch(self, raw_elems, stats_elems):
        self.scratch("raw", raw_elems)
        self.scratch("stats", stats_elems)

    def _keep(self, t):
        if self.plan is not None:
            self.plan.keep.append(t)

    def label(self, text):
        if self.plan is not None:
            self.plan.label(text)

    @property
    def _sk_counter(self):
        return self._sk_counters.get((0, 0))

    @property
    def _fin_counter(self):
        return self._fin_counters.get((0, 0))

    @contextlib.contextmanager
    def scratch_set(self, k):
        prev, self._sset = self._sset, k
        try:
            yield
        finally:
            self._sset = prev

    @contextlib.contextmanager
    def on_lane(self, k):
        parent = self._lane
        if not self.lanes_enabled or k == parent:
            yield
            return
        check(lib.v2v_plan_lane_wait(k, parent), "plan_lane_wait")
        self._lane = k
        check(lib.v2v_plan_set_lane(k), "plan_set_lane")
        try:
            yield
        finally:
            self._lane = parent
            check(lib.v2v_plan_set_lane(parent), "plan_set_lane")

    def join(self, k):
        if self.lanes_enabled and k != self._lane:
            check(lib.v2v_plan_lane_wait(self._lane, k), "plan_lane_wait")

    def wgrad_side_stream(self):
        if not self.wgrad_stream_on or self.record_only or self.device.type != "cuda":
            return None
        if self._wgrad_stream is None:
            self._wgrad_stream = torch.cuda.Stream(device=self.device)
            from . import parallel
            parallel.register_grad_stream(self._wgrad_stream)
        return self._wgrad_stream

    def queue_wgrad_join(self):
        if self._wgrad_join_queued:
            return
        self._wgrad_join_queued = True
        side = self._wgrad_stream

        def join():
            self._wgrad_join_queued = False
            torch.cuda.current_stream(self.device).wait_stream(side)
# ... 38 lines not shown
    def repack_async(self, flat=None):
        side = self.wgrad_side_stream()
        if side is None or self.plan is not None or not self.repack_async_on or torch.cuda.is_current_stream_capturing():
            return
        fid = id(flat) if flat is not None else None
        todo = [pc for pc in self._packed.values() if pc.used and (fid is None or pc.flat_id == fid)]
        if not todo:
            return
        cur = torch.cuda.current_stream(self.device)
        side.wait_stream(cur)
        with torch.cuda.stream(side):
            for pc in todo:
                pc.used = False
                pc.refresh()
            ev = torch.cuda.Event()
            ev.record(side)
        self._repack_event = ev

    def wait_repack(self):
        ev = self._repack_event
        if ev is not None:
            self._repack_event = None
            torch.cuda.current_stream(self.device).wait_event(ev)

    def refresh_weights(self, force=False):
        for pc in self._packed.values():
            pc.refresh(force)
        for pc in self._packed_onehot.values():
            pc.refresh(force)
        if self._x3_engine is not None:
            self._x3_engine.refresh_weights(force)

    def onehot_conv_ok(self, conv, cin, H, W, pad_mode=L.PAD_REFLECT, pad=3):
        return (self.onehot_stem and isinstance(conv, nn.Conv2d) and conv.kernel_size == (7, 7)
                and conv.stride == (1, 1) and conv.groups == 1 and pad_mode == L.PAD_REFLECT and pad == 3
                and conv.out_channels <= 128 and conv.in_channels == cin and H >= 4 and W >= 4
                and not (self.plan is None and torch.is_grad_enabled()))

    def onehot_eligible(self, x, conv, pad_mode, pad_override):
        return (x.onehot is not None and (x.N == 1 or (self.per_stream and x.onehot.codes is not None))
                and self.onehot_conv_ok(conv, x.C, x.H, x.W, pad_mode, conv.padding[0] if pad_override is None else pad_override))

    def label_codes(self, src, H, W):
        if src.label_nc > 126:
            return None
        codes = torch.empty((src.T, H, W), dtype=torch.uint8, device=self.device)
        self._keep(codes)
        check(lib.v2v_label_codes(_ptr(src.labels), _ptr(src.inst), int(src.labels.dtype == torch.uint8), _ptr(codes), src.T, H, W,
                                  src.label_nc, _stream()), "label_codes")
        self.label("label_codes")
        src.codes = codes
        return codes

    def frame_prologue(self, src, H, W, fg_labels, want_mask, window=None, last_C=0, row_slot=None):
        labels, inst, T = src.labels, src.inst, src.T
        N = labels.shape[0] if labels.dim() == 4 else 1
        u8 = labels.dtype == torch.uint8
        if u8 and inst is not None and inst.dtype != torch.int32:
            raise TypeError("uint8 label maps go with int32 instance maps")
        if not u8 and (labels.dtype != torch.float32 or (inst is not None and inst.dtype != torch.float32)):
            raise TypeError("label / instance maps must be fp32-encoded integers, or uint8 + int32")
        if row_slot is not None:
            if (window is None or window.dim() != 4 or window.dtype != torch.float32 or not window.is_contiguous()
                    or row_slot.dtype != torch.int32 or tuple(row_slot.shape) != (N,) or not row_slot.is_contiguous()):
                raise ValueError("frame_prologue: a pooled head reads an fp32 pool (S, C, H, W) through int32 row_slot (N,)")
            self._keep(row_slot)
        elif N > 1 and window is not None and window.shape[0] != N:
            raise ValueError("frame_prologue: %d label streams, window of %d" % (N, window.shape[0]))
        per = src.label_nc + (1 if inst is not None else 0)
        codes = torch.empty((T, H, W) if N == 1 else (N, T, H, W), dtype=torch.uint8, device=self.device)
        self._keep(codes)
        mask = self.empty_f32(N, 1, H, W) if want_mask else None
        fg = None
        if want_mask:
            fg = self._fg_labels(fg_labels)
            self._keep(fg)
        packed = last = None
        win_C = cs = 0
        if window is not None:
            win_C = window.shape[1]
            packed = self.empty_act(N, H, W, win_C)
            cs = packed.Cs
            if last_C:
                last = self.empty_f32(N, last_C, H, W)
        entry, pool = ("frame_prologue_batch", ()) if row_slot is None else ("frame_prologue_pool", (window.shape[0], _ptr(row_slot)))
        check(getattr(lib, "v2v_" + entry)(_ptr(labels), _ptr(inst), int(u8), _ptr(codes), _ptr(mask), _ptr(fg),
                                           0 if fg is None else fg.numel(), N, T, H, W, src.label_nc, _ptr(window), *pool, win_C,
                                           _ptr(None if packed is None else packed.t), cs, _ptr(last), last_C, self.dtype,
                                           _stream()), entry)
        self.label("frame_prologue")
        src.codes = codes
        x0 = Act(torch.empty((N, H, W, pad_channels(T * per, self.dtype)), dtype=self.tdtype, device="meta"), T * per, onehot=src)
        return x0, mask, packed, last

    def image_prologue(self, win, lut, window=None, last_C=0, advance=True, slot_mode=None, row_slot=None, pooled_window=False):
        if not isinstance(win, torch.Tensor) or win.dtype != torch.uint8:
            raise TypeError("image_prologue: the input window is uint8 (N, T, H, W, Cin)")
        if not isinstance(lut, torch.Tensor) or lut.dtype != torch.float32:
            raise TypeError("image_prologue: the table is fp32 (Cin, 256)")
        if win.dim() != 5 or not win.is_contiguous():
            raise ValueError("image_prologue: the input window is contiguous uint8 (N, T, H, W, Cin)")
        N, T, H, W, Cin = win.shape
        S_win = S_window = 0
        if row_slot is not None:
            if (not isinstance(row_slot, torch.Tensor) or row_slot.dtype != torch.int32 or row_slot.dim() != 1
                    or not 1 <= row_slot.numel() <= N or not row_slot.is_contiguous() or row_slot.device != win.device):
                raise ValueError("image_prologue: a pooled head reads a uint8 pool (S, T, H, W, Cin) through int32 row_slot (N,), N <= S")
            S_win, N = N, row_slot.numel()
        elif pooled_window:
            raise ValueError("image_prologue: a pooled generated-frame window goes with row_slot")
        if slot_mode is not None and (not isinstance(slot_mode, torch.Tensor) or slot_mode.dtype != torch.int32
                                      or tuple(slot_mode.shape) != (N,) or not slot_mode.is_contiguous()
                                      or slot_mode.device != win.device):
            raise ValueError("image_prologue: slot_mode is int32 (%d,) on the window's device" % N)
        if Cin > 32:
            raise ValueError("image_prologue: %d input channels; the table of at most 32 channels is held in LDS" % Cin)
        if tuple(lut.shape) != (Cin, 256) or not lut.is_contiguous() or lut.device != win.device:
            raise ValueError("image_prologue: the table is contiguous fp32 (%d, 256) on the window's device, got %s"
                             % (Cin, tuple(lut.shape)))
        if window is not None:
            if window.dtype != torch.float32:
                raise TypeError("image_prologue: the generated-frame window is fp32 (N, C, H, W)")
            if pooled_window:
                if window.dim() != 4 or window.shape[0] < N or tuple(window.shape[2:]) != (H, W) or not window.is_contiguous():
                    raise ValueError("image_prologue: %d rows at %dx%d, pooled window %s" % (N, W, H, tuple(window.shape)))
                S_window = window.shape[0]
            elif window.dim() != 4 or tuple(window.shape[::3]) != (N, W) or window.shape[2] != H or not window.is_contiguous():
                raise ValueError("image_prologue: %d image streams at %dx%d, window %s" % (N, W, H, tuple(window.shape)))
            if not 0 <= last_C <= window.shape[1]:
                raise ValueError("image_prologue: last_C = %d of a window of %d planes" % (last_C, window.shape[1]))
        self._keep(win)
        self._keep(lut)
        x0 = self.empty_act(N, H, W, T * Cin)
        real_last = self.empty_f32(N, Cin, H, W)
        packed = last = None
        win_C = cs = 0
        if window is not None:
            self._keep(window)
            win_C = window.shape[1]
            packed = self.empty_act(N, H, W, win_C)
            cs = packed.Cs
            if last_C:
# ... 1006 lines not shown
        out = self.empty_f32(x.N, x.C, x.H, x.W)
        check(lib.v2v_unpack_nhwc_to_nchw(_ptr(x.t), _ptr(out), x.N, x.C, x.H, x.W, x.Cs, self.dtype, _stream()), "unpack")
        self.label("unpack_nhwc_to_nchw")
        return out

    def avgpool_nhwc(self, x):
        OH, OW = (x.H - 1) // 2 + 1, (x.W - 1) // 2 + 1
        if self._training() and x.t.requires_grad:
            from . import autograd as AG
            return Act(AG.AvgPoolFn.apply(self, x.t), x.C)
        out = self.empty_act(x.N, OH, OW, x.C)
        if out.Cs != x.Cs:
            t = torch.empty((x.N, OH, OW, x.Cs), dtype=self.tdtype, device=self.device)
            self._keep(t)
            out = Act(t, x.C)
        check(lib.v2v_avgpool3s2_nhwc(_ptr(x.t), _ptr(out.t), x.N, x.H, x.W, x.Cs, self.dtype, _stream()), "avgpool_nhwc")
        self.label("avgpool3s2_nhwc")
        return out

    def maxpool2_nhwc(self, x):
        if self._training() and x.t.requires_grad:
            from . import autograd as AG
            return Act(AG.MaxPool2Fn.apply(self, x.t), x.C)
        t = torch.empty((x.N, x.H // 2, x.W // 2, x.Cs), dtype=self.tdtype, device=self.device)
        self._keep(t)
        check(lib.v2v_maxpool2_nhwc(_ptr(x.t), _ptr(t), x.N, x.H, x.W, x.Cs, self.dtype, _stream()), "maxpool2_nhwc")
        self.label("maxpool2_nhwc")
        return Act(t, x.C)

    def avgpool2_planar(self, x):
        if self._training() and x.requires_grad:
            from . import autograd as AG
            return AG.AvgPool2PlanarFn.apply(self, x)
        x = x.contiguous().float()
        H, W = x.shape[-2], x.shape[-1]
        out = self.empty_f32(*x.shape[:-2], H // 2, W // 2)
        check(lib.v2v_avgpool2_planar(_ptr(x), _ptr(out), x.numel() // (H * W), H, W, _stream()), "avgpool2_planar")
        self.label("avgpool2_planar")
        return out

    def instance_mean(self, feat, inst):
        feat = feat.contiguous().float()
        inst = inst.contiguous().float()
        N, Cc, H, W = feat.shape
        out = self.empty_f32(N, Cc, H, W)
        nbytes = lib.v2v_instance_mean_workspace(Cc, H * W)
        ws = self.scratch("instance_mean_ws", (nbytes + 3) // 4)
        for n in range(N):
            check(lib.v2v_instance_mean_planar(_ptr(feat[n]), _ptr(inst[n]), _ptr(out[n]), _ptr(ws), Cc, H * W, _stream()),
                  "instance_mean")
            self.label("instance_mean")
        return out

    def onehot_planar(self, labels, inst, H, W, label_nc):
        per = label_nc + (1 if inst is not None else 0)
        if labels.dim() == 3:
            N = labels.shape[0]
            if labels.stride(1) != W or labels.stride(2) != 1 or (inst is not None and inst.stride() != labels.stride()):
                raise ValueError("onehot_planar: dense frames, the same sample stride for labels and instance maps")
            out = self.empty_f32(N, per, H, W)
            check(lib.v2v_onehot_planar_batch(_ptr(labels), _ptr(inst), int(labels.dtype == torch.uint8), _ptr(out), N,
                                              labels.stride(0), H, W, label_nc, _stream()), "onehot_planar_batch")
            self.label("onehot_planar")
            return out
        out = self.empty_f32(per, H, W)
        fn = lib.v2v_onehot_planar_u8 if labels.dtype == torch.uint8 else lib.v2v_onehot_planar
        check(fn(_ptr(labels), _ptr(inst), _ptr(out), H, W, label_nc, _stream()), "onehot_planar")
        self.label("onehot_planar")
        return out

    def avgpool_planar(self, x):
        H, W = x.shape[-2], x.shape[-1]
        OH, OW = (H - 1) // 2 + 1, (W - 1) // 2 + 1
        planes = x.numel() // (H * W)
        out = self.empty_f32(*x.shape[:-2], OH, OW)
        check(lib.v2v_avgpool3s2_planar(_ptr(x), _ptr(out), planes, H, W, _stream()), "avgpool_planar")
        self.label("avgpool3s2_planar")
        return out

    def warp_blend(self, img_raw, flow, weight, prev, fg, mask, want_warp=False, roll=None, slot_mode=None, row_slot=None):
        N, Cc, H, W = img_raw.shape
        if self._training() and any(t is not None and t.requires_grad for t in (img_raw, flow, weight, prev, fg)):
            from . import autograd as AG
            final, raw_blend = AG.WarpBlendFn.apply(self, img_raw, flow, weight, prev, fg, mask)
            return (final, raw_blend), None
        gx, gy = self.grid(H, W)
        final = self.empty_f32(N, Cc, H, W)
        warp = self.empty_f32(N, Cc, H, W) if (want_warp and flow is not None) else None
        for t in (gx, gy):
            self._keep(t)
        words = [t for t in (slot_mode, row_slot) if t is not None]
        if row_slot is not None and (slot_mode is None or roll is None):
            raise ValueError("warp_blend: a pooled blend rolls an fp32 pool (S, slots, C, H, W) under int32 slot_mode, row_slot (N,)")
        if any(t.dtype != torch.int32 or tuple(t.shape) != (N,) or not t.is_contiguous() for t in words):
            raise ValueError("warp_blend: slot_mode and row_slot are int32 (N,)")
        if roll is not None:
            lead = tuple(roll.shape[:-4])
            if (roll.dim() < 4 or tuple(roll.shape[-3:]) != (Cc, H, W) or roll.dtype != torch.float32 or not roll.is_contiguous()
                    or not (len(lead) == 1 if row_slot is not None else lead == (N,) or (lead == () and N == 1 and not words))):
                raise ValueError("warp_blend: the rolled window is fp32 (slots, C, H, W) of one sample, (N, slots, C, H, W) of N "
                                 "streams, or with row_slot the pool (S, slots, C, H, W)")
        for t in words:
            self._keep(t)
        win = (_ptr(roll), 0 if roll is None else roll.shape[-4])
        if row_slot is not None:
            entry, extra = "warp_blend_pool", win + (_ptr(slot_mode), _ptr(row_slot), N, roll.shape[0])
        elif slot_mode is not None:
            entry, extra = "warp_blend_slots", win + (_ptr(slot_mode), N)
        elif roll is None:
            entry, extra = "warp_blend", (N,)
        else:
            entry, extra = ("warp_blend_roll", win) if roll.dim() == 4 else ("warp_blend_roll_batch", win + (N,))
        check(getattr(lib, "v2v_" + entry)(_ptr(img_raw), _ptr(flow), _ptr(weight), _ptr(prev), _ptr(fg), _ptr(mask), _ptr(final),
                                           _ptr(warp), _ptr(gx), _ptr(gy), *extra, Cc, H, W, int(self.align_corners), _stream()), entry)
        self.label("warp_blend")
        return final, warp

    def window_roll(self, window, frame, slot_mode):
        N, slots, Cc, H, W = window.shape
        if (tuple(frame.shape) != (N, Cc, H, W) or tuple(slot_mode.shape) != (N,) or slot_mode.dtype != torch.int32
                or window.dtype != torch.float32 or frame.dtype != torch.float32
                or not (window.is_contiguous() and frame.is_contiguous() and slot_mode.is_contiguous())):
            raise ValueError("window_roll: fp32 window (N, slots, C, H, W), fp32 frame (N, C, H, W), int32 slot_mode (N,)")
        self._keep(slot_mode)
        check(lib.v2v_window_roll_slots(_ptr(window), _ptr(frame), _ptr(slot_mode), N, slots, Cc, H, W, _stream()),
              "window_roll_slots")
        self.label("window_roll")

    def _window_pool_args(self, dense, pool, row_slot, what):
        K, S = dense.shape[0], pool.shape[0]
        if (dense.dim() != 5 or pool.dim() != 5 or tuple(dense.shape[1:]) != tuple(pool.shape[1:]) or tuple(row_slot.shape) != (K,)
                or row_slot.dtype != torch.int32 or dense.dtype != torch.float32 or pool.dtype != torch.float32
                or not (dense.is_contiguous() and pool.is_contiguous() and row_slot.is_contiguous())):
            raise ValueError("%s: fp32 dense (K, slots, C, H, W), fp32 pool (S, slots, C, H, W), int32 row_slot (K,)" % what)
        self._keep(row_slot)
        return (_ptr(row_slot), K, S) + tuple(dense.shape[1:]) + (_stream(),)

    def window_gather(self, dense, pool, row_slot):
        check(lib.v2v_window_gather_pool(_ptr(dense), _ptr(pool), *self._window_pool_args(dense, pool, row_slot, "window_gather")),
              "window_gather_pool")
        self.label("window_gather")

    def window_scatter(self, pool, dense, row_slot):
        check(lib.v2v_window_scatter_pool(_ptr(pool), _ptr(dense), *self._window_pool_args(dense, pool, row_slot, "window_scatter")),
              "window_scatter_pool")
        self.label("window_scatter")

    def frames_u8(self, frames, mode=None, row_slot=None, S=None, normalize=True):
        K, Cc, H, W = frames.shape
        S = K if S is None else int(S)
        if frames.dtype != torch.float32 or not frames.is_contiguous():
            raise ValueError("frames_u8: contiguous fp32 frames (K, C, H, W)")
        for t in (mode, row_slot):
            if t is not None and (t.dtype != torch.int32 or tuple(t.shape) != (K,) or not t.is_contiguous()):
                raise ValueError("frames_u8: mode and row_slot are int32 (K,)")
            if t is not None:
                self._keep(t)
        out = torch.empty((S, H, W, Cc), dtype=torch.uint8, device=self.device)
        self._keep(out)
        check(lib.v2v_frames_u8(_ptr(frames), _ptr(out), _ptr(mode), _ptr(row_slot), K, S, Cc, H, W, int(bool(normalize)),
                                _stream()), "frames_u8")
        self.label("frames_u8")
        return out

    def label_image(self, labels, inst, label_nc, slot_mode=None, row_slot=None, S=None):
        if labels.dim() != 4 or not labels.is_contiguous() or labels.dtype not in (torch.uint8, torch.float32):
            raise ValueError("label_image: contiguous uint8 or fp32 label maps (K, T, H, W)")
        K, T, H, W = labels.shape
        u8 = labels.dtype == torch.uint8
        if inst is not None and (inst.dtype != (torch.int32 if u8 else torch.float32) or inst.shape != labels.shape
                                 or not inst.is_contiguous()):
            raise ValueError("label_image: the instance maps are int32 beside uint8 labels, fp32 beside fp32 ones, of their shape")
        if not 1 <= label_nc <= 255:
            raise ValueError("label_image: label_nc within 1..255, got %d" % label_nc)
        S = K if S is None else int(S)
        for t in (slot_mode, row_slot):
            if t is not None and (t.dtype != torch.int32 or tuple(t.shape) != (K,) or not t.is_contiguous()):
                raise ValueError("label_image: slot_mode and row_slot are int32 (K,)")
            if t is not None:
                self._keep(t)
        cmap = self._label_cmaps.get(label_nc)
        if cmap is None:
            from .visual import labelcolormap
            cmap = self._label_cmaps[label_nc] = torch.from_numpy(labelcolormap(label_nc)[:label_nc].copy()).to(self.device)
        out = torch.empty((S, H, W, 3), dtype=torch.uint8, device=self.device)
        for t in (labels, inst, cmap, out):
            if t is not None:
                self._keep(t)
        check(lib.v2v_label_image(_ptr(labels), _ptr(inst), int(u8), _ptr(cmap), label_nc, _ptr(out), _ptr(slot_mode), _ptr(row_slot),
                                  K, S, T, H, W, _stream()), "label_image")
        self.label("label_image")
        return out

    def resample_flow(self, img, flow):
        N, Cc, H, W = img.shape
        if self._training() and (img.requires_grad or flow.requires_grad):
            from . import autograd as AG
            return AG.ResampleFn.apply(self, img, flow)
        gx, gy = self.grid(H, W)
        out = self.empty_f32(N, Cc, H, W)
        check(lib.v2v_resample_flow(_ptr(img), _ptr(flow), _ptr(out), _ptr(gx), _ptr(gy), N, Cc, H, W,
                                    int(self.align_corners), _stream()), "resample_flow")
        self.label("resample_flow")
        return out
```

### vid2vid_amd/lib.py

```python
import ctypes as C
import os

_HERE = os.path.dirname(os.path.abspath(__file__))
LIB_PATH = os.environ.get("V2V_LIB_PATH") or os.path.join(_HERE, "libv2v_hip.so")

F32, BF16 = 0, 1
PAD_ZERO, PAD_REFLECT = 0, 1
ACT_NONE, ACT_RELU, ACT_LEAKY, ACT_TANH, ACT_SIGMOID = 0, 1, 2, 3, 4
OUT_RAW_F32_NHWC, OUT_ACT_NHWC, OUT_F32_NCHW, OUT_NORM_ACT_NHWC, OUT_RAW_ACT_NHWC = 0, 1, 2, 3, 4


class ConvDesc(C.Structure):
    _fields_ = [
        ("in_", C.c_void_p), ("w", C.c_void_p), ("bias", C.c_void_p), ("out", C.c_void_p),
        ("stats", C.c_void_p), ("zero_page", C.c_void_p),
        ("N", C.c_int32), ("H", C.c_int32), ("W", C.c_int32),
        ("cin", C.c_int32), ("cin_stride", C.c_int32),
        ("cout", C.c_int32), ("cout_stride", C.c_int32),
        ("KH", C.c_int32), ("KW", C.c_int32),
        ("stride", C.c_int32), ("pad", C.c_int32), ("pad_mode", C.c_int32),
        ("transposed", C.c_int32),
        ("OH", C.c_int32), ("OW", C.c_int32),
        ("dtype", C.c_int32), ("out_mode", C.c_int32), ("act", C.c_int32),
        ("act_param", C.c_float), ("out_scale", C.c_float),
        ("tile", C.c_int32),
        ("fin_counter", C.c_void_p), ("fin_gamma", C.c_void_p), ("fin_beta", C.c_void_p),
        ("fin_scale_shift", C.c_void_p), ("fin_running_mean", C.c_void_p), ("fin_running_var", C.c_void_p),
        ("fin_eps", C.c_float), ("fin_momentum", C.c_float), ("fin_count", C.c_int64),
        ("splitk", C.c_int32), ("prefetch", C.c_int32), ("slabs", C.c_void_p), ("sk_counter", C.c_void_p),
        ("w_korder", C.c_int32), ("ablate", C.c_int32),
        ("res0", C.c_void_p), ("res1", C.c_void_p),
        ("act_split", C.c_int32), ("act_b", C.c_int32), ("act_param_b", C.c_float), ("out_scale_b", C.c_float),
        ("fin_workspace", C.c_void_p),
    ]


class ConvTileInfo(C.Structure):
    _fields_ = [(n, C.c_int32) for n in ("id", "family", "bm", "bn", "th", "tw", "korder", "flags")]


(TILE_IGEMM, TILE_PATCH, TILE_PP, TILE_PP2, TILE_PP3, TILE_S7, TILE_S2, TILE_T2, TILE_ONE, TILE_T2_ONE, TILE_HEAD, TILE_C8,
 TILE_ROWSUM) = range(13)
(TILE_GROUPED, TILE_FUSED_NORM, TILE_PAD2, TILE_SINGLE_CHUNK, TILE_PERSISTENT, TILE_HELPER, TILE_BF16_ONLY, TILE_ABLATION,
 TILE_EXPERIMENT, TILE_EXACT_BN) = (1 << i for i in range(10))


class OneHotNorm(C.Structure):
    _fields_ = [
        ("counter", C.c_void_p), ("gamma", C.c_void_p), ("beta", C.c_void_p), ("scale_shift", C.c_void_p),
        ("running_mean", C.c_void_p), ("running_var", C.c_void_p), ("eps", C.c_float), ("momentum", C.c_float),
        ("count", C.c_int64),
    ]


class WgradDesc(C.Structure):
    _fields_ = [
        ("p", C.c_void_p), ("q", C.c_void_p), ("grad", C.c_void_p), ("workspace", C.c_void_p), ("zero_page", C.c_void_p),
        ("N", C.c_int32), ("OH", C.c_int32), ("OW", C.c_int32), ("QH", C.c_int32), ("QW", C.c_int32),
        ("rows", C.c_int32), ("cols", C.c_int32), ("p_stride", C.c_int32), ("q_stride", C.c_int32),
        ("KH", C.c_int32), ("KW", C.c_int32), ("stride", C.c_int32), ("pad", C.c_int32), ("pad_mode", C.c_int32),
        ("dtype", C.c_int32), ("accumulate", C.c_int32),
    ]


LOSS_MSE_CONST, LOSS_L1 = 0, 1
FACE_DENSEPOSE, FACE_OPENPOSE = 0, 1
FACE_WIN_WORDS = 8

_P, _I, _L, _F = C.c_void_p, C.c_int32, C.c_int64, C.c_float
PROTOTYPES = {
    "v2v_conv_packed_elems": (_L, [_I, _I, _I, _I, _I, _I, _I, _I, _I]),
    "v2v_conv_pack_weights": (C.c_int, [_P, _P, _I, _I, _I, _I, _I, _I, _I, _I, _I, _I, _P]),
    "v2v_conv_stats_rows": (C.c_int, [C.POINTER(ConvDesc)]),
    "v2v_conv_stats_rows_per_sample": (C.c_int, [C.POINTER(ConvDesc)]),
    "v2v_conv_debug_clocks": (C.c_int, [_P]),
    "v2v_conv_tile_config": (C.c_int, [C.POINTER(ConvDesc)]),
    "v2v_conv_tile_count": (C.c_int, []),
    "v2v_conv_tile_info": (C.c_int, [_I, C.POINTER(ConvTileInfo)]),
    "v2v_conv_fused_norm_max_workgroups": (C.c_int, []),
    "v2v_fastdiv_magic": (C.c_int, [C.c_uint32, C.POINTER(C.c_uint32), C.POINTER(_I)]),
    "v2v_conv_splitk_workspace": (_L, [C.POINTER(ConvDesc), C.POINTER(_I)]),
    "v2v_conv2d": (C.c_int, [C.POINTER(ConvDesc), _P]),
    "v2v_conv2d_pair": (C.c_int, [C.POINTER(ConvDesc), C.POINTER(ConvDesc), _P]),
    "v2v_conv_wgrad_workspace": (_L, [C.POINTER(WgradDesc)]),
    "v2v_conv_wgrad": (C.c_int, [C.POINTER(WgradDesc), _P]),
    "v2v_bn_backward_rows": (C.c_int, [_L]),
    "v2v_bn_backward": (C.c_int, [_P, _P, _I, _P, _P, _I, _P, _P, _I, _P, _L, _I, _I, _I, _F, _I, _P]),
    "v2v_channel_sum": (C.c_int, [_P, _P, _I, _P, _L, _I, _I, _I, _P]),
    "v2v_act_backward": (C.c_int, [_P, _P, _P, _I, _I, _I, _I, _I, _I, _I, _I, _F, _F, _I, _P]),
    "v2v_avgpool3s2_nhwc_backward": (C.c_int, [_P, _P, _I, _I, _I, _I, _I, _P]),
    "v2v_pack_concat_nhwc": (C.c_int, [_P, _I, _P, _I, _F, _P, _I, _I, _I, _I, _I, _P]),
    "v2v_unpack_channels_nchw": (C.c_int, [_P, _P, _I, _I, _I, _I, _I, _I, _I, _P]),
    "v2v_face_window": (C.c_int, [_P, _I, _I, _I, _I, _I, _I, _I, _P, _P]),
    "v2v_pack_concat_window_nhwc": (C.c_int, [_P, _I, _P, _I, _I, _I, _I, _P, _I, _I, _P, _I, _I, _P]),
    "v2v_unpack_window_nchw": (C.c_int, [_P, _P, _I, _I, _I, _I, _I, _I, _I, _I, _P, _I, _P]),
    "v2v_reflect_pad_fold": (C.c_int, [_P, _P, _I, _I, _I, _I, _I, _I, _P]),
    "v2v_warp_blend_backward": (C.c_int, [_P] * 15 + [_I] * 5 + [_P]),
    "v2v_resample_flow_backward": (C.c_int, [_P] * 7 + [_I] * 5 + [_P]),
    "v2v_flownet_normalize": (C.c_int, [_P, _P, _P, _P, _P, _I, _I, _I, _F, _P]),
    "v2v_warp_diff_norm": (C.c_int, [_P, _L, _P, _L, _P, _P, _P, _I, _I, _I, _I, _I, _F, _P]),
    "v2v_resize_planar": (C.c_int, [_P, _P, _L, _I, _I, _I, _I, _I, _F, _P]),
    "v2v_pack_channels_nhwc": (C.c_int, [_P, _P, _I, _I, _I, _I, _I, _I, _F, _F, _I, _P]),
    "v2v_concat_channels_nhwc": (C.c_int, [_P, _I, _I, _P, _I, _I, _I, _L, _I, _P]),
    "v2v_loss_workspace_floats": (C.c_int, []),
    "v2v_loss_forward": (C.c_int, [_I, _P, _P, _P, _F, _F, _L, _I, _I, _L, _L, _L, _I, _P, _P, _I, _P]),
    "v2v_loss_backward": (C.c_int, [_I, _P, _P, _P, _F, _F, _L, _I, _I, _L, _L, _L, _I, _P, _P, _I, _P]),
    "v2v_adam_step": (C.c_int, [_P, _P, _P, _P, _L, _F, _F, _F, _F, _F, _F, _I, _P]),
    "v2v_adam_step_dev": (C.c_int, [_P, _P, _P, _P, _L, _F, _F, _F, _F, _F, _P, _P]),
    "v2v_adam_step_ema": (C.c_int, [_P, _P, _P, _P, _P, _L, _F, _F, _F, _F, _F, _F, _I, _F, _P]),
    "v2v_adam_step_dev_ema": (C.c_int, [_P, _P, _P, _P, _P, _L, _F, _F, _F, _F, _F, _P, _F, _P]),
    "v2v_adam_guard_workspace_bytes": (_L, []),
    "v2v_grad_sumsq": (C.c_int, [_P, _L, _P, _P]),
    "v2v_adam_step_dev_guard": (C.c_int, [_P, _P, _P, _P, _L, _F, _F, _F, _F, _F, _P, _P, _F, _I, _P]),
    "v2v_adam_step_dev_guard_ema": (C.c_int, [_P, _P, _P, _P, _P, _L, _F, _F, _F, _F, _F, _P, _F, _P, _F, _I, _P]),
# ... 3 lines not shown
    "v2v_bn_apply": (C.c_int, [_P, _I, _P, _P, _P, _P, _L, _I, _I, _I, _F, _I, _P]),
    "v2v_bn_apply_pair": (C.c_int, [_P] * 10 + [_I, _L, _I, _I, _I, _F, _I, _P]),
    "v2v_bn_apply_raw": (C.c_int, [_P, _I, _I, _P, _P, _P, _P, _L, _I, _I, _I, _F, _I, _P]),
    "v2v_in_groups": (C.c_int, [_L, _I, _I]),
    "v2v_in_workspace_bytes": (_L, [_L, _I, _I]),
    "v2v_in_ticket_words": (C.c_int, [_I, _I]),
    "v2v_in_stats": (C.c_int, [_P, _I, _I, _P, _P, _F, _P, _P, _P, _I, _L, _I, _P]),
    "v2v_in_finalize_rows_workspace": (_L, [_I, _I, _I]),
    "v2v_in_finalize_rows": (C.c_int, [_P, _I, _I, _I, _L, _P, _P, _F, _P, _P, _P]),
    "v2v_in_apply": (C.c_int, [_P, _I, _I, _P, _P, _P, _P, _P, _I, _L, _I, _I, _I, _F, _I, _P]),
    "v2v_in_backward": (C.c_int, [_P, _P, _I, _P, _P, _I, _P, _P, _I, _P, _P, _I, _L, _I, _I, _I, _F, _I, _P]),
    "v2v_avgpool3s2_planar": (C.c_int, [_P, _P, _L, _I, _I, _P]),
    "v2v_avgpool3s2_nhwc": (C.c_int, [_P, _P, _I, _I, _I, _I, _I, _P]),
    "v2v_maxpool2_nhwc": (C.c_int, [_P, _P, _I, _I, _I, _I, _I, _P]),
    "v2v_maxpool2_nhwc_backward": (C.c_int, [_P, _P, _P, _I, _I, _I, _I, _I, _P]),
    "v2v_avgpool2_planar": (C.c_int, [_P, _P, _L, _I, _I, _P]),
    "v2v_avgpool2_planar_backward": (C.c_int, [_P, _P, _L, _I, _I, _P]),
    "v2v_onehot_planar": (C.c_int, [_P, _P, _P, _I, _I, _I, _P]),
    "v2v_onehot_planar_u8": (C.c_int, [_P, _P, _P, _I, _I, _I, _P]),
    "v2v_onehot_planar_batch": (C.c_int, [_P, _P, _I, _P, _I, _L, _I, _I, _I, _P]),
    "v2v_instance_mean_workspace": (_L, [_I, _L]),
    "v2v_instance_mean_planar": (C.c_int, [_P, _P, _P, _P, _I, _L, _P]),
    "v2v_tensor2im": (C.c_int, [_P, _P, _I, _I, _I, _I, _P]),
    "v2v_frames_u8": (C.c_int, [_P, _P, _P, _P, _I, _I, _I, _I, _I, _I, _P]),
    "v2v_label_image": (C.c_int, [_P, _P, _I, _P, _I, _P, _P, _P, _I, _I, _I, _I, _I, _P]),
    "v2v_tensor2label": (C.c_int, [_P, _P, _P, _I, _I, _I, _I, _P]),
    "v2v_tensor2flow": (C.c_int, [_P, _P, _P, _I, _I, _P]),
    "v2v_onehot_conv_table_bytes": (_L, [_I, _I, _I, _I, _I, _I]),
    "v2v_onehot_conv_pack_weights": (C.c_int, [_P, _P, _I, _I, _I, _I, _I, _I, _P]),
    "v2v_onehot_conv_stats_rows": (C.c_int, [_I, _I]),
    "v2v_label_codes": (C.c_int, [_P, _P, _I, _P, _I, _I, _I, _I, _P]),
    "v2v_onehot_conv7x7": (C.c_int, [_P, _P, _I, _P, _P, _P, _P, _I, _I, _I, _I, _I, _I, _I, _I, _P]),
    "v2v_onehot_conv7x7_batch": (C.c_int, [_P, _P, _I, _P, _P, _P, _P, _I, _I, _I, _I, _I, _I, _I, _I, _I, _P]),
    "v2v_onehot_conv_ppt": (C.c_int, [_I, _I, _I, _I, _I, _I, _I, _I, _I]),
    "v2v_onehot_conv7x7_norm": (C.c_int, [_P, _P, _I, _P, _P, _P, _P, _I, _I, _I, _I, _I, _I, _I, _I, C.POINTER(OneHotNorm), _P]),
    "v2v_encode_labels": (C.c_int, [_P, _P, _P, _P, _I, _I, _I, _I, _I, _P, _I, _I, _P]),
    "v2v_encode_labels_u8": (C.c_int, [_P, _P, _P, _P, _I, _I, _I, _I, _I, _P, _I, _I, _P]),
    "v2v_encode_labels_pooled": (C.c_int, [_P, _P, _P, _P, _I, _I, _I, _I, _I, _P, _I, _I, _I, _P]),
    "v2v_fg_mask_nhwc": (C.c_int, [_P, _P, _L, _I, _I, _P, _I, _I, _P]),
    "v2v_pack_nchw_to_nhwc": (C.c_int, [_P, _P, _I, _I, _I, _I, _I, _I, _P]),
    "v2v_unpack_nhwc_to_nchw": (C.c_int, [_P, _P, _I, _I, _I, _I, _I, _I, _P]),
    "v2v_add_nhwc": (C.c_int, [_P, _P, _P, _L, _I, _P]),
    "v2v_warp_blend": (C.c_int, [_P, _P, _P, _P, _P, _P, _P, _P, _P, _P, _I, _I, _I, _I, _I, _P]),
    "v2v_warp_blend_roll": (C.c_int, [_P] * 11 + [_I] * 5 + [_P]),
    "v2v_warp_blend_roll_batch": (C.c_int, [_P] * 11 + [_I] * 6 + [_P]),
    "v2v_warp_blend_slots": (C.c_int, [_P] * 11 + [_I] + [_P] + [_I] * 5 + [_P]),
    "v2v_window_roll_slots": (C.c_int, [_P, _P, _P, _I, _I, _I, _I, _I, _P]),
    "v2v_frame_prologue": (C.c_int, [_P, _P, _I, _P, _P, _P, _I, _I, _I, _I, _I, _P, _I, _P, _I, _P, _I, _I, _P]),
    "v2v_frame_prologue_batch": (C.c_int, [_P, _P, _I, _P, _P, _P, _I, _I, _I, _I, _I, _I, _P, _I, _P, _I, _P, _I, _I, _P]),
    "v2v_frame_prologue_pool": (C.c_int, [_P, _P, _I, _P, _P, _P, _I, _I, _I, _I, _I, _I, _P, _I, _P, _I, _P, _I, _P, _I, _I, _P]),
    "v2v_image_prologue": (C.c_int, [_P, _P, _I, _P, _I, _P, _I, _I, _I, _I, _I, _P, _I, _P, _I, _P, _I, _I, _P]),
    "v2v_image_prologue_slots": (C.c_int, [_P, _P, _I, _P, _I, _P, _I, _I, _I, _I, _I, _P, _I, _P, _I, _P, _I, _I, _P,
                                           _P, _P, _I, _I]),
    "v2v_warp_blend_pool": (C.c_int, [_P] * 11 + [_I] + [_P, _P] + [_I] * 6 + [_P]),
    "v2v_window_gather_pool": (C.c_int, [_P, _P, _P, _I, _I, _I, _I, _I, _I, _P]),
    "v2v_window_scatter_pool": (C.c_int, [_P, _P, _P, _I, _I, _I, _I, _I, _I, _P]),
    "v2v_resample_flow": (C.c_int, [_P, _P, _P, _P, _P, _I, _I, _I, _I, _I, _P]),
    "v2v_correlation_out_size": (C.c_int, [_I, _I, _I, _I, _I, _I, _I, C.POINTER(_I), C.POINTER(_I), C.POINTER(_I)]),
    "v2v_correlation_forward": (C.c_int, [_P, _P, _P, _I, _I, _I, _I, _I, _I, _I, _I, _I, _I, _P]),
    "v2v_correlation_nhwc": (C.c_int, [_P, _P, _P, _I, _I, _I, _I, _I, _I, _I, _I, _I, _F, _I, _P]),
    "v2v_resample2d_forward": (C.c_int, [_P, _P, _P, _I, _I, _I, _I, _I, _I, _I, _P]),
    "v2v_channelnorm_forward": (C.c_int, [_P, _P, _I, _I, _I, _I, _I, _P]),
    "v2v_correlation_backward": (C.c_int, [_P] * 5 + [_I] * 13 + [_P]),
    "v2v_resample2d_backward": (C.c_int, [_P] * 5 + [_I] * 7 + [_P]),
    "v2v_channelnorm_backward": (C.c_int, [_P] * 4 + [_I] * 5 + [_P]),
    "v2v_plan_create": (_P, []),
    "v2v_plan_destroy": (None, [_P]),
    "v2v_plan_begin_record": (C.c_int, [_P]),
    "v2v_plan_end_record": (C.c_int, [_P]),
    "v2v_plan_num_ops": (C.c_int, [_P]),
    "v2v_plan_run": (C.c_int, [_P, _P]),
    "v2v_plan_instantiate_graph": (C.c_int, [_P, _P]),
    "v2v_plan_launch_graph": (C.c_int, [_P, _P]),
    "v2v_plan_segment_program": (C.c_int, [_P, C.POINTER(_I), _I, C.POINTER(_I), _I]),
    "v2v_plan_profile": (C.c_int, [_P, _P, C.POINTER(C.c_float), _I]),
    "v2v_plan_timeline": (C.c_int, [_P, _P, C.POINTER(C.c_float), C.POINTER(C.c_float), C.POINTER(_I), _I]),
    "v2v_plan_timeline_graph": (C.c_int, [_P, _P, C.POINTER(C.c_float), C.POINTER(C.c_float), C.POINTER(_I), _I]),
    "v2v_plan_op_name": (C.c_char_p, [_P, _I]),
    "v2v_plan_op_lane": (C.c_int, [_P, _I]),
    "v2v_plan_set_label": (C.c_int, [_P, C.c_char_p]),
    "v2v_plan_op_label": (C.c_char_p, [_P, _I]),
    "v2v_plan_set_lane": (C.c_int, [_I]),
    "v2v_plan_lane_wait": (C.c_int, [_I, _I]),
    "v2v_memcpy_d2d": (C.c_int, [_P, _P, _L, _P]),
    "v2v_split_x3": (C.c_int, [_P, _P, _L, _I, _I, _I, _P]),
    "v2v_bn_apply_x3": (C.c_int, [_P] * 12 + [_I, _L, _I, _I, _F, _P]),
    "v2v_set_dry_run": (C.c_int, [_I]),
    "v2v_get_dry_run": (C.c_int, []),
    "v2v_version": (C.c_int, []),
    "v2v_last_error": (C.c_char_p, []),
    "v2v_device_status": (C.c_int, [_I]),
    "v2v_device_info": (C.c_int, [C.POINTER(_I), C.POINTER(_I), C.POINTER(_L), C.c_char_p, _I]),
}


def _load():
    if not os.path.exists(LIB_PATH):
        raise ImportError(
            "vid2vid_amd: %s is missing -- build it with `python -c 'import __graft_entry__ as g; g.build()'` "
            "(or `make -C vid2vid_amd/csrc`).  There is no CPU fallback." % LIB_PATH)
    lib = C.CDLL(LIB_PATH)
    for name, (res, args) in PROTOTYPES.items():
        fn = getattr(lib, name)
        fn.restype = res
        fn.argtypes = args
    return lib

# ... 22 lines not shown
```

### vid2vid_amd/models/vid2vid_model_G.py

```python
import os

import torch

from .. import lib as L
from .. import networks
from ..engine import Act, Plan
from ..optim import FusedAdam
from .base_model import BaseModel


def nearest_face_features(feat_map, inst, features, feat_num):
    import numpy as np
    inst_l = inst.long()
    labels = [int(l) for l in torch.unique(inst_l)]
    num_images = features[6].shape[0]
    ori = torch.zeros(7, feat_num, 1)
    ref = torch.zeros(7, feat_num, num_images)
    for label in labels:
        idx = (inst_l == label).nonzero()
        b, _, y, x = [int(v) for v in idx[0]]
        ori[label, :, 0] = feat_map[b, :feat_num, y, x].detach().float().cpu()
        ref[label] = torch.from_numpy(np.ascontiguousarray(features[label][:num_images, :feat_num].T)).float()
    dists = ((ori - ref) ** 2).sum(0).sum(0)
    cluster = int(torch.argmin(dists))
    out = torch.zeros(inst.size(0), feat_num, inst.size(2), inst.size(3), dtype=torch.float32, device=inst.device)
    for label in labels:
        feat = features[label][:, :-1]
        row = torch.as_tensor(np.asarray(feat[min(cluster, feat.shape[0] - 1), :feat_num], dtype=np.float32), device=inst.device)
        mask = (inst_l[:, 0] == label)
        out.permute(0, 2, 3, 1)[mask] = row
    return out


class _StreamPool:

    def __init__(self, S, tG, nc, H, W, n_scales, device):
        self.S, self.H, self.W = S, H, W
        self.tG, self.device = tG, device
        self.windows = [torch.zeros(S, tG - 1, nc, H >> si, W >> si, dtype=torch.float32, device=device) for si in range(n_scales)]
        self.inputs = {}
        self.idle = []

    def input_windows(self, in_ch):
        win = self.inputs.get(in_ch)
        if win is None:
            win = self.inputs[in_ch] = torch.zeros(self.S, self.tG, self.H, self.W, in_ch, dtype=torch.uint8, device=self.device)
        return win


class _FramePlan:

    def __init__(self, model, H, W, in_ch, has_inst, use_raw_only, use_graph=True, u8=False, B=1, slots=False, pool=None,
                 frames_u8=False, inputs_u8=False, real_A_u8=False, inputs_u8_slots=False):
        opt, eng = model.opt, model.engine
        self.model, self.eng = model, eng
        self.H, self.W, self.use_raw_only, self.B = H, W, use_raw_only, B
        self.slots = bool(slots)
        self.frames_u8 = bool(frames_u8)
        self.real_A_u8 = bool(real_A_u8)
        if self.slots and (B < 2 or use_raw_only):
            raise ValueError("a slot plan has B > 1 streams and decides raw-only frames per stream (slot_mode 1)")
        self.pool = pool
        if pool is not None and (self.slots or use_raw_only or not 1 <= B <= pool.S or (pool.H, pool.W) != (H, W)):
            raise ValueError("a pool plan has 1..S rows at the pool's resolution and decides raw-only frames per row (row_mode 1)")
        lead = (B,) if B > 1 else ()
        tG, S = opt.n_frames_G, model.n_scales
        self.label_mode = opt.label_nc != 0
        dev = eng.device
        self.win_u8 = self.lut = self._lut_src = None
        if inputs_u8 and (self.label_mode or ((self.slots or pool is not None) and not inputs_u8_slots)):
            raise ValueError("uint8 image inputs (opt.inputs_u8) go with label_nc == 0 and plain plans")
        if self.label_mode:
            self.labels = torch.zeros(*lead, tG, H, W, dtype=torch.uint8 if u8 else torch.float32, device=dev)
            self.inst = torch.zeros(*lead, tG, H, W, dtype=torch.int32 if u8 else torch.float32, device=dev) if has_inst else None
            self.raw_in = None
        else:
            self.labels = self.inst = None
            self.raw_in = None if inputs_u8 else torch.zeros(B, tG * in_ch, H, W, dtype=torch.float32, device=dev)
            if inputs_u8:
                self.win_u8 = torch.zeros(B, tG, H, W, in_ch, dtype=torch.uint8, device=dev) if pool is None else \
                    pool.input_windows(in_ch)
                self.lut = torch.zeros(in_ch, 256, dtype=torch.float32, device=dev)
        if pool is not None:
            self.prev = pool.windows
        else:
            self.prev = [torch.zeros(*lead, tG - 1, opt.output_nc, H >> si, W >> si, dtype=torch.float32, device=dev)
                         for si in range(S)]
        self.slot_mode = self.row_slot = self._words = self._words_host = self._words_copied = None
        if self.slots:
            self.slot_mode = self._words = torch.zeros(B, dtype=torch.int32, device=dev)
            self.blend_launch = getattr(model, "netG" + str(S - 1)).blends_in_tail()
        if pool is not None:
            self._words = torch.cat([torch.arange(B, dtype=torch.int32), torch.zeros(B, dtype=torch.int32)]).to(dev)
            self.row_slot, self.slot_mode = self._words[:B], self._words[B:]
            self.dense = {}
        if self._words is not None:
            self._words_host = torch.zeros(self._words.numel(), dtype=torch.int32)
            if dev.type == "cuda":
                self._words_host = self._words_host.pin_memory()
        self.out = {}
        self.lanes = bool(int(getattr(opt, "lanes", os.environ.get("V2V_LANES", "1")))) and use_graph
        self.twin = bool(int(getattr(opt, "twin", os.environ.get("V2V_TWIN", "1"))))
        eng.lanes_enabled = self.lanes
        eng.twin_enabled = self.twin
        eng.per_stream = B > 1
        try:
            self._build(model, opt, eng, use_graph)
        finally:
            eng.lanes_enabled = False
            eng.twin_enabled = False
            eng.per_stream = False

    def _build(self, model, opt, eng, use_graph):
        dev = eng.device
        if not eng.record_only:
            prev_autotune = eng.autotune
            eng.autotune = bool(getattr(opt, "autotune", True))
            try:
                self._emit()
            finally:
                eng.autotune = prev_autotune
            torch.cuda.synchronize(dev)
        self._record(use_graph)
        if use_graph and not eng.record_only and self.lanes and bool(int(getattr(opt, "frame_tune", os.environ.get("V2V_FRAME_TUNE", "1")))):
            self._frame_tune(use_graph)

    def _record(self, use_graph):
        eng = self.eng
        self.plan = Plan()
        eng.plan = self.plan
        try:
            with self.plan:
                self._emit()
        finally:
            eng.plan = None
        if use_graph and not eng.record_only:
            self.plan.instantiate_graph()

    def _time_frames(self, n=16, reps=3):
        ts = []
        for _ in range(reps):
            e0, e1 = torch.cuda.Event(enable_timing=True), torch.cuda.Event(enable_timing=True)
            e0.record()
            for _ in range(n):
                self.plan.launch()
            e1.record()
            e1.synchronize()
            ts.append(e0.elapsed_time(e1) / n)
        return sorted(ts)[len(ts) // 2]

    def _frame_tune(self, use_graph, max_trials=160, min_gain=0.005, max_seconds=40.0):
        eng = self.eng
        work = {}
# ... 86 lines not shown
                return self._emit_image_head()
            if self.slots or self.pool is not None:
                x0, real_last, _, _ = eng.image_prologue(self.win_u8, self.lut, slot_mode=self.slot_mode if self.slots else None,
                                                         row_slot=self.row_slot)
            else:
                x0, real_last, _, _ = eng.image_prologue(self.win_u8, self.lut)
            mask0 = x1 = None
        else:
            x0, mask0, x1 = eng.pack(self.raw_in), None, None
        xs, masks = [x0], [mask0]
        for si in range(1, S):
            xs.append(x1 if (si == 1 and x1 is not None) else eng.avgpool_nhwc(xs[-1]))
            masks.append(None)
        per = x0.C // tG
        feat = flow_feat = fg_feat = None
        fake_B = None
        for s in range(S):
            si = S - 1 - s
            netG = getattr(m, "netG" + str(s))
            x = xs[si]
            mask = masks[si]
            if opt.fg and mask is None:
                mask = self._mask_from_pooled(x, per, tG)
            window = self._gathered(si) if self.pool is not None else self.prev[si]
            prev_nchw = window.view(B, -1, H >> si, W >> si)
            fake_B, flow, weight, raw, feat, flow_feat, fg_feat = netG.emit(
                eng, x, eng.pack(prev_nchw), prev_nchw, mask, feat, flow_feat, fg_feat, self.use_raw_only,
                tag="G%d" % s, slot_mode=self.slot_mode)
            self._roll(window, fake_B)
            if self.pool is not None:
                eng.window_scatter(self.prev[si], window, self.row_slot)
            self.out["flow%d" % si], self.out["weight%d" % si], self.out["raw%d" % si] = flow, weight, raw
        self.out["fake_B"] = fake_B
        if self.label_mode:
            self._emit_real_A()
        elif self.win_u8 is not None:
            self.out["real_A_last"] = real_last[0] if B == 1 else real_last
        else:
            last = Act(x0.t[..., (tG - 1) * per:], per)
            last = eng.unpack(last)
            self.out["real_A_last"] = last[0] if B == 1 else last
        self._emit_input_image()
        self._emit_image()
        self.conv_log = list(eng.conv_log)

    def _emit_real_A(self):
        if self.real_A_u8:
            opt = self.model.opt
            labels, inst = (self.labels, self.inst) if self.B > 1 else \
                (self.labels.unsqueeze(0), None if self.inst is None else self.inst.unsqueeze(0))
            if self.pool is not None:
                self.out["real_A_image"] = self.eng.label_image(labels, inst, opt.label_nc, self.slot_mode, self.row_slot, S=self.pool.S)
            else:
                self.out["real_A_image"] = self.eng.label_image(labels, inst, opt.label_nc, self.slot_mode if self.slots else None)
        else:
            self.out["real_A_last"] = self._real_A_last()

    def _emit_input_image(self):
        if not self.real_A_u8 or self.label_mode:
            return
        H, W, B = self.H, self.W, self.B
        last = self.out["real_A_last"].view(B, -1, H, W)
        c = 3 if last.shape[1] == 3 else 1
        planes = last[:, :c]
        if not planes.is_contiguous():
            planes = self.eng.empty_f32(B, c, H, W)
            for b in range(B):
                self.eng.memcpy(planes[b], last[b], c * H * W * 4)
        if self.pool is not None:
            self.out["real_A_image"] = self.eng.frames_u8(planes, self.slot_mode, self.row_slot, S=self.pool.S, normalize=False)
        else:
            self.out["real_A_image"] = self.eng.frames_u8(planes, self.slot_mode if self.slots else None, normalize=False)

    def _real_A_last(self):
        tG, opt = self.model.opt.n_frames_G, self.model.opt
        lab = self.labels[tG - 1] if self.B == 1 else self.labels[:, tG - 1]
        inst = None if self.inst is None else (self.inst[tG - 1] if self.B == 1 else self.inst[:, tG - 1])
        return self.eng.onehot_planar(lab, inst, self.H, self.W, opt.label_nc)

    def _emit_fused_head(self, src):
        m, eng, opt = self.model, self.eng, self.model.opt
        tG, H, W = opt.n_frames_G, self.H, self.W
        netG = m.netG0
        prev = self.prev[0]
        rolls = netG.rolls_in_tail(self.use_raw_only)
        row_slot = None
        if self.pool is not None and rolls:
            row_slot = self.row_slot
            x0, mask0, prev_act, last = eng.frame_prologue(src, H, W, opt.fg_labels, opt.fg, window=prev.view(self.pool.S, -1, H, W),
                                                           last_C=opt.output_nc, row_slot=row_slot)
        else:
            if self.pool is not None:
                prev = self._gathered(0)
            x0, mask0, prev_act, last = eng.frame_prologue(src, H, W, opt.fg_labels, opt.fg, window=prev.view(self.B, -1, H, W),
                                                           last_C=opt.output_nc)

        roll = prev if rolls else None
        fake_B, flow, weight, raw, _, _, _ = netG.emit(eng, x0, prev_act, last, mask0, None, None, None, self.use_raw_only,
                                                       tag="G0", roll=roll, side=self._emit_real_A,
                                                       slot_mode=self.slot_mode, row_slot=row_slot)
        if roll is None:
            self._roll(prev, fake_B)
            if self.pool is not None:
                eng.window_scatter(self.prev[0], prev, self.row_slot)
        self.out["flow0"], self.out["weight0"], self.out["raw0"] = flow, weight, raw
        self.out["fake_B"] = fake_B
        self._emit_image()
        self.conv_log = list(eng.conv_log)

    def _emit_image_head(self):
        m, eng, opt = self.model, self.eng, self.model.opt
        H, W, B = self.H, self.W, self.B
        netG = m.netG0
        prev = self.prev[0]
        rolls = netG.rolls_in_tail(self.use_raw_only)
        row_slot = None
        if self.pool is not None:
            if rolls:
                row_slot = self.row_slot
                window = prev.view(self.pool.S, -1, H, W)
            else:
                prev = self._gathered(0)
                window = prev.view(B, -1, H, W)
            x0, real_last, prev_act, last = eng.image_prologue(self.win_u8, self.lut, window=window, last_C=opt.output_nc,
                                                               row_slot=self.row_slot, pooled_window=rolls)
        elif self.slots:
            x0, real_last, prev_act, last = eng.image_prologue(self.win_u8, self.lut, window=prev.view(B, -1, H, W),
                                                               last_C=opt.output_nc, slot_mode=self.slot_mode)
        else:
            x0, real_last, prev_act, last = eng.image_prologue(self.win_u8, self.lut, window=prev.view(B, -1, H, W),
                                                               last_C=opt.output_nc)
        self.out["real_A_last"] = real_last[0] if B == 1 else real_last
        roll = prev if rolls else None
        fake_B, flow, weight, raw, _, _, _ = netG.emit(eng, x0, prev_act, last, None, None, None, None, self.use_raw_only,
                                                       tag="G0", roll=roll, slot_mode=self.slot_mode, row_slot=row_slot)
        if roll is None:
            self._roll(prev, fake_B)
            if self.pool is not None:
                eng.window_scatter(self.prev[0], prev, self.row_slot)
        self.out["flow0"], self.out["weight0"], self.out["raw0"] = flow, weight, raw
        self.out["fake_B"] = fake_B
        self._emit_input_image()
        self._emit_image()
        self.conv_log = list(eng.conv_log)

    def _emit_image(self):
        if not self.frames_u8:
            return
        fake_B = self.out["fake_B"]
        fake_B = fake_B.view(self.B, -1, self.H, self.W)
        if self.pool is not None:
            self.out["image"] = self.eng.frames_u8(fake_B, self.slot_mode, self.row_slot, S=self.pool.S)
        else:
            self.out["image"] = self.eng.frames_u8(fake_B, self.slot_mode if self.slots else None)

    def _gathered(self, si):
        dense = self.dense.get(si)
        if dense is None:
            dense = self.dense[si] = torch.zeros((self.B,) + tuple(self.prev[si].shape[1:]), dtype=torch.float32,
                                                 device=self.prev[si].device)
        self.eng.window_gather(dense, self.prev[si], self.row_slot)
        return dense

    def _roll(self, prev, fake_B):
        if self.slots or self.pool is not None:
            self.eng.window_roll(prev, fake_B, self.slot_mode)
        elif self.B > 1:
            for b in range(self.B):
                self._roll_one(prev[b], fake_B[b])
        else:
            self._roll_one(prev, fake_B)

    def _roll_one(self, prev, fake_B):
        n = prev.shape[0]
        frame_bytes = prev[0].numel() * 4
        for k in range(n - 1):
            self.eng.memcpy(prev[k], prev[k + 1], frame_bytes)
        self.eng.memcpy(prev[n - 1], fake_B, frame_bytes)

    def _mask_from_pooled(self, x, per, tG):
        return self.eng.fg_mask(x, (tG - 1) * per, self.model.opt.fg_labels)

    def set_words(self, words):
        if self._words_copied is not None:
            self._words_copied.synchronize()
        self._words_host.copy_(torch.as_tensor(words, dtype=torch.int32))
        self._words.copy_(self._words_host, non_blocking=True)
        if self._words.device.type == "cuda":
            self._words_copied = torch.cuda.Event()
            self._words_copied.record()

    def run(self):
        if self.eng.record_only:
            return
        self.plan.launch()


class Vid2VidModelG(BaseModel):
    def name(self):
        return "Vid2VidModelG"

    def initialize(self, opt):
        BaseModel.initialize(self, opt)
        self.n_scales = opt.n_scales_spatial
        self.use_single_G = opt.use_single_G
        self.split_gpus = bool(getattr(opt, "role_group_size", 0))
        if (opt.n_gpus_gen < len(opt.gpu_ids)) and (opt.batchSize == 1) and opt.isTrain:
            raise RuntimeError("n_gpus_gen=%d < %d GPUs selects the generator / discriminator rank roles: launch one process per GPU "
                               "(python -m torch.distributed.run --nproc-per-node %d train.py ...)" % (opt.n_gpus_gen, len(opt.gpu_ids), len(opt.gpu_ids)))

        input_nc = opt.label_nc if opt.label_nc != 0 else opt.input_nc
        netG_input_nc = input_nc * opt.n_frames_G
        if opt.use_instance:
            netG_input_nc += opt.n_frames_G
        prev_output_nc = (opt.n_frames_G - 1) * opt.output_nc
        if opt.openpose_only:
            opt.no_flow = True
        self.netG_input_nc, self.prev_output_nc = netG_input_nc, prev_output_nc

        gpu_ids = self.dev_ids
        self.netG0 = networks.define_G(netG_input_nc, opt.output_nc, prev_output_nc, opt.ngf, opt.netG,
                                       opt.n_downsample_G, opt.norm, 0, gpu_ids, opt)
        for s in range(1, self.n_scales):
            setattr(self, "netG" + str(s),
                    networks.define_G(netG_input_nc, opt.output_nc, prev_output_nc, opt.ngf // (2 ** s),
                                      opt.netG + "Local", opt.n_downsample_G, opt.norm, s, gpu_ids, opt))
        print("---------- Networks initialized -------------")

        if not self.isTrain or opt.continue_train or opt.load_pretrain:
            label = "G%d_ema" if (not self.isTrain and getattr(opt, "use_ema", False)) else "G%d"
            for s in range(self.n_scales):
                self.load_network(getattr(self, "netG" + str(s)), label % s, opt.which_epoch, opt.load_pretrain)
        self.netG_i = self.load_single_G() if self.use_single_G else None
        self._plans = {}
        self._pools = {}

        if self.isTrain:
            self.n_gpus = opt.n_gpus_gen if opt.batchSize == 1 else 1
            self.n_frames_bp = 1
            self.n_frames_per_gpu = min(opt.max_frames_per_gpu, opt.n_frames_total // self.n_gpus)
            self.n_frames_load = self.n_gpus * self.n_frames_per_gpu
            self.old_lr = opt.lr
            self.finetune_all = opt.niter_fix_global == 0
# ... 100 lines not shown
                lut = self._check_inputs_u8(input_A, restart, active)
                B, t_in, H, W, in_ch = input_A.shape
            else:
                B, t_in, in_ch, H, W = input_A.shape
                if t_in < tG:
                    raise ValueError("inference needs n_frames_G=%d label frames, got %d" % (tG, t_in))
            for name, t in (("inst_A", inst_A if opt.use_instance else None), ("input_B", input_B)):
                if t is not None and t.shape[0] != B:
                    raise ValueError("inference: input_A holds %d sequence(s), %s %d" % (B, name, t.shape[0]))
            slot_call = restart is not None or active is not None
            if slot_call:
                act = [True] * B if active is None else self._slot_set(active, B, "active")
                rst = [False] * B if restart is None else self._slot_set(restart, B, "restart")
                both = [b for b in range(B) if rst[b] and not act[b]]
                if both:
                    raise ValueError("inference: stream(s) %s are restarted and idle in the same call" % both)
            self._check_device_status()
            self.is_first_frame = not hasattr(self, "fake_B_prev") or self.fake_B_prev is None
            if not self.is_first_frame and self._active_plan is not None:
                running = self._active_plan.B if self._active_plan.pool is None else self._active_plan.pool.S
                if running != B:
                    raise ValueError("inference: %d sequence(s) given while %d are running; assign fake_B_prev = None to restart"
                                     % (B, running))
            has_inst = bool(opt.use_instance and inst_A is not None and opt.label_nc != 0)
            img = bool(getattr(opt, "frames_u8", False))
            pic = bool(getattr(opt, "real_A_u8", False))
            if slot_call and B == 1:
                if not act[0]:
                    last_C = in_ch if opt.label_nc == 0 else opt.label_nc + int(has_inst)
                    idle = torch.zeros(1, H, W, opt.output_nc, dtype=torch.uint8, device=self.device) if img else \
                        torch.zeros(1, opt.output_nc, H, W, dtype=torch.float32, device=self.device)
                    if pic:
                        return idle, torch.zeros(1, H, W, self._picture_channels(in_ch), dtype=torch.uint8, device=self.device)
                    return idle, torch.zeros(last_C, H, W, dtype=torch.float32, device=self.device)
                if rst[0]:
                    self.fake_B_prev = None
                    self.is_first_frame = True
                slot_call = False
            if self.is_first_frame:
                self._slots_on = False
            if slot_call:
                self._slots_on = True
            u8 = bool(opt.label_nc != 0 and input_A.dtype == torch.uint8)
            if B > 1 and getattr(opt, "compact_streams", False):
                if not slot_call:
                    act, rst = [True] * B, [False] * B
                return self._inference_pool(input_A, input_B, inst_A, act, rst, has_inst, u8, img, pic, lut)
            if self._slots_on:
                if not slot_call:
                    act, rst = [True] * B, [False] * B
                return self._inference_slots(input_A, input_B, inst_A, act, rst, has_inst, u8, img, pic, lut)
            use_raw_only = bool(opt.no_first_img and self.is_first_frame)
            fp = self._frame_plan(H, W, in_ch, has_inst, use_raw_only, u8, B, frames_u8=img, inputs_u8=in_u8, real_A_u8=pic)
            if not in_u8:
                self._stage_inputs(fp, input_A, inst_A, has_inst, list(range(B)))
            if self.is_first_frame:
                from ..visual import decode_inputs
                planes = decode_inputs(input_A.to(self.device), lut) if in_u8 else input_A
                self._seed_windows(fp.prev, planes, input_B, inst_A)
            else:
                self._carry_windows(fp)
            if in_u8:
                self._stage_inputs_u8(fp, input_A, lut)
            self._active_plan = fp
            self.fake_B_prev = fp.prev
            fp.run()
            return fp.out["image" if img else "fake_B"].clone(), fp.out["real_A_image" if pic else "real_A_last"].clone()

    def _picture_channels(self, in_ch):
        return 3 if self.opt.label_nc != 0 or in_ch == 3 else 1

    def _stage_inputs(self, fp, input_A, inst_A, has_inst, rows, in_place=False):
        tG, dev = self.opt.n_frames_G, self.device
        every = len(rows) == input_A.shape[0] > 1
        if in_place and not every:
            pairs = [(b, b) for b in rows]
        else:
            pairs = [(slice(None) if every else rows[0] if len(rows) == 1 else rows, Ellipsis)]
        for src, dst in pairs:
            if fp.label_mode:
                fp.labels[dst].copy_(input_A[src, :tG, 0].to(dev, fp.labels.dtype, non_blocking=True))
                if has_inst:
                    fp.inst[dst].copy_(inst_A[src, :tG, 0].to(dev, fp.inst.dtype, non_blocking=True))
            else:
                raw = fp.raw_in[dst]
                raw.copy_(input_A[src, :tG].reshape(raw.shape).to(dev, torch.float32, non_blocking=True))

    def _input_table(self, in_ch):
        lut = getattr(self.opt, "input_lut", None)
        if lut is None:
            cache = self.__dict__.setdefault("_default_luts", {})
            if in_ch not in cache:
                from ..visual import input_lut
                cache[in_ch] = input_lut(in_ch).to(self.device)
            return cache[in_ch]
        if not isinstance(lut, torch.Tensor) or lut.dtype != torch.float32 or tuple(lut.shape) != (in_ch, 256):
            raise ValueError("inference: opt.input_lut is an fp32 tensor (%d, 256): one row per channel of input_A" % in_ch)
        return lut

    def _check_inputs_u8(self, input_A, restart, active):
        opt, tG = self.opt, self.opt.n_frames_G
        if opt.label_nc != 0:
            raise ValueError("inference: opt.inputs_u8 is for image inputs (label_nc == 0); label maps are uint8 already")
        if not isinstance(input_A, torch.Tensor) or input_A.dtype != torch.uint8 or input_A.dim() != 5:
            raise ValueError("inference: with opt.inputs_u8 input_A is torch.uint8 (B, t, H, W, in_ch)")
        B, t_in, _, _, in_ch = input_A.shape
        if in_ch > 32:
            raise ValueError("inference: opt.inputs_u8 decodes at most 32 input channels, input_A has %d" % in_ch)
        running = hasattr(self, "fake_B_prev") and self.fake_B_prev is not None
        if getattr(opt, "inputs_u8_slots", False):
            self._check_inputs_u8_slots(input_A, restart, active, running)
        else:
            if restart is not None or active is not None:
                raise ValueError("inference: restart= / active= (slot plans) take fp32 inputs; opt.inputs_u8 runs plain plans only")
            if B > 1 and getattr(opt, "compact_streams", False):
                raise ValueError("inference: opt.compact_streams (pool plans) takes fp32 inputs; opt.inputs_u8 runs plain plans only")
            if running and self._slots_on:
                raise ValueError("inference: the running sequences are in a slot plan, which takes fp32 inputs")
        if t_in not in (1, tG):
            raise ValueError("inference: with opt.inputs_u8 input_A holds the whole window (t = %d) or the newest frame (t = 1), "
# ... 366 lines not shown
```

Measured before the change: 397.5 frames/s.

## Read inputs and write outputs in place via device-side frame IO table

Adds a device-resident frame IO descriptor holding input label/instance pointers with strides and output sink pointers. Graph-captured kernels (prologue, warp blend, label image, frames_u8, onehot planar) read it at run time, so later frames skip staging copies into plan buffers and the final output clones. Each call patches the pointer table through a pinned ring and an async copy. This adds host-side bookkeeping and an indirect pointer load per kernel, and relies on caller tensors staying alive while the graph runs.

```diff
diff --git a/include/v2v_hip.h b/include/v2v_hip.h
--- a/include/v2v_hip.h
+++ b/include/v2v_hip.h
@@ -452,6 +452,34 @@
 int     v2v_onehot_conv_ppt(int32_t N, int32_t T, int32_t H, int32_t W, int32_t label_nc, int32_t has_inst,
                             int32_t cout, int32_t dtype, int32_t slice);
 
+typedef struct v2v_frame_io {
+    const void* labels;
+    int64_t labels_sample_stride, labels_frame_stride, labels_row_stride;
+    const void* inst;
+    int64_t inst_sample_stride, inst_frame_stride, inst_row_stride;
+    void* fake_B;
+    void* real_A_last;
+    void* image;
+    void* real_A_image;
+    int64_t reserved[4];
+} v2v_frame_io;
+
+int v2v_frame_prologue_io(const void* labels, const void* inst, int32_t in_u8, uint8_t* codes, float* mask,
+                          const int32_t* fg_labels_dev, int32_t n_fg, int32_t N, int32_t T, int32_t H, int32_t W,
+                          int32_t label_nc, const float* window, int32_t win_C, void* packed, int32_t c_stride,
+                          float* last, int32_t last_C, int32_t dtype, const v2v_frame_io* io, void* stream);
+int v2v_warp_blend_roll_io(float* img_raw, const float* flow, const float* weight, const float* prev,
+                           const float* fg, const float* mask, float* img_final, float* img_warp,
+                           const float* gx, const float* gy, float* window, int32_t slots,
+                           int32_t N, int32_t C, int32_t H, int32_t W, int32_t align_corners, const v2v_frame_io* io, void* stream);
+int v2v_onehot_planar_io(const void* labels, const void* inst, int32_t in_u8, float* out, int32_t N, int32_t T,
+                         int32_t H, int32_t W, int32_t label_nc, const v2v_frame_io* io, void* stream);
+int v2v_frames_u8_io(const float* frames, uint8_t* out, const int32_t* mode, const int32_t* row_slot, int32_t K, int32_t S,
+                     int32_t C, int32_t H, int32_t W, int32_t normalize, const v2v_frame_io* io, void* stream);
+int v2v_label_image_io(const void* labels, const void* inst, int32_t in_u8, const uint8_t* cmap, int32_t label_nc, uint8_t* out,
+                       const int32_t* mode, const int32_t* row_slot, int32_t K, int32_t S, int32_t T, int32_t H, int32_t W,
+                       const v2v_frame_io* io, void* stream);
+
 int v2v_memcpy_d2d(void* dst, const void* src, int64_t bytes, void* stream);
 
 int         v2v_set_dry_run(int32_t on);
diff --git a/vid2vid_amd/csrc/label_image.hip b/vid2vid_amd/csrc/label_image.hip
--- a/vid2vid_amd/csrc/label_image.hip
+++ b/vid2vid_amd/csrc/label_image.hip
@@ -6,6 +6,7 @@
     const void* labels; const void* inst; const unsigned char* cmap; unsigned char* out;
     const int* mode; const int* row_slot;
     int K, S, T, H, W, label_nc, planes;
+    const v2v_frame_io* io = nullptr;
 };
 
 static constexpr int LABEL_IMAGE_GRID_CAP = 256;
@@ -40,7 +41,7 @@
     }
 }
 
-template <typename LT, typename IT, int R>
+template <typename LT, typename IT, int R, bool IO>
 __global__ __launch_bounds__(256) void label_image_kernel(const LabelImageArgs a) {
     constexpr int NW = 3 * R / 4;
     constexpr unsigned BLACK = 255;
@@ -58,10 +59,18 @@
     const int rpr = (a.W + R - 1) / R;
     const long long runs = (long long)a.H * rpr;
     const long long stride = (long long)gridDim.x * blockDim.x;
-    const long long frame = ((long long)(row < 0 ? 0 : row) * a.T + (a.T - 1)) * hw;
-    const LT* const labels = reinterpret_cast<const LT*>(a.labels) + frame;
-    const IT* const inst = a.inst ? reinterpret_cast<const IT*>(a.inst) + frame : nullptr;
-    unsigned char* const out = a.out + (long long)s * hw * 3;
+    const long long smp = row < 0 ? 0 : row;
+    const long long frame = (smp * a.T + (a.T - 1)) * hw;
+    const LT* labels = reinterpret_cast<const LT*>(a.labels) + frame;
+    const IT* inst = a.inst ? reinterpret_cast<const IT*>(a.inst) + frame : nullptr;
+    unsigned char* out = a.out;
+    if (IO) {
+        const v2v_frame_io& io = *a.io;
+        labels = reinterpret_cast<const LT*>(io.labels) + smp * io.labels_sample_stride + (a.T - 1) * io.labels_frame_stride;
+        if (inst) inst = reinterpret_cast<const IT*>(io.inst) + smp * io.inst_sample_stride + (a.T - 1) * io.inst_frame_stride;
+        out = reinterpret_cast<unsigned char*>(io.real_A_image);
+    }
+    out += (long long)s * hw * 3;
     for (long long r = (long long)blockIdx.x * blockDim.x + threadIdx.x; r < runs; r += stride) {
         const int y = (int)(r / rpr);
         const int x0 = (int)(r - (long long)y * rpr) * R;
@@ -146,22 +155,22 @@
 
 struct LabelImageOp : Op {
     LabelImageArgs a; int in_u8;
-    template <typename LT, typename IT>
+    template <typename LT, typename IT, bool IO>
     void go(hipStream_t s) {
         const dim3 b(256);
         if (a.W >= 16) {
             long long gx = ceil_div((long long)a.H * ceil_div(a.W, 16), 256);
             if (gx > LABEL_IMAGE_GRID_CAP) gx = LABEL_IMAGE_GRID_CAP;
-            hipLaunchKernelGGL((label_image_kernel<LT, IT, 16>), dim3((unsigned)gx, (unsigned)a.S), b, 0, s, a);
+            hipLaunchKernelGGL((label_image_kernel<LT, IT, 16, IO>), dim3((unsigned)gx, (unsigned)a.S), b, 0, s, a);
         } else {
             long long gx = ceil_div((long long)a.H * ceil_div(a.W, 4), 256);
             if (gx > LABEL_IMAGE_GRID_CAP) gx = LABEL_IMAGE_GRID_CAP;
-            hipLaunchKernelGGL((label_image_kernel<LT, IT, 4>), dim3((unsigned)gx, (unsigned)a.S), b, 0, s, a);
+            hipLaunchKernelGGL((label_image_kernel<LT, IT, 4, IO>), dim3((unsigned)gx, (unsigned)a.S), b, 0, s, a);
         }
     }
     int launch(hipStream_t s) override {
-        if (in_u8) go<unsigned char, int>(s);
-        else       go<float, float>(s);
+        if (a.io) { if (in_u8) go<unsigned char, int, true>(s); else go<float, float, true>(s); }
+        else      { if (in_u8) go<unsigned char, int, false>(s); else go<float, float, false>(s); }
         return check_launch();
     }
     const char* name() const override { return "label_image"; }
@@ -176,9 +185,9 @@
 
 using namespace v2v;
 
-extern "C" int v2v_label_image(const void* labels, const void* inst, int32_t in_u8, const uint8_t* cmap, int32_t label_nc,
-                               uint8_t* out, const int32_t* mode, const int32_t* row_slot, int32_t K, int32_t S, int32_t T,
-                               int32_t H, int32_t W, void* stream) {
+static int label_image_submit(const void* labels, const void* inst, int32_t in_u8, const uint8_t* cmap, int32_t label_nc,
+                              uint8_t* out, const int32_t* mode, const int32_t* row_slot, int32_t K, int32_t S, int32_t T,
+                              int32_t H, int32_t W, const v2v_frame_io* io, void* stream) {
     if (!labels || !cmap || !out) { set_error("label_image: null pointer"); return V2V_EINVAL; }
     if (label_nc < 1 || label_nc > 255) {
         set_error("label_image: label_nc %d (1..255: the palette and its black entry are 256 words of LDS)", label_nc); return V2V_EINVAL;
@@ -201,6 +210,19 @@
     }
     auto op = std::make_unique<LabelImageOp>();
     op->a = LabelImageArgs{labels, inst, cmap, out, mode, row_slot, K, S, T, H, W, label_nc, label_nc + (inst ? 1 : 0)};
-    op->in_u8 = in_u8;
+    op->in_u8 = in_u8; op->a.io = io;
     return submit(std::move(op), stream);
 }
+
+extern "C" int v2v_label_image(const void* labels, const void* inst, int32_t in_u8, const uint8_t* cmap, int32_t label_nc,
+                               uint8_t* out, const int32_t* mode, const int32_t* row_slot, int32_t K, int32_t S, int32_t T,
+                               int32_t H, int32_t W, void* stream) {
+    return label_image_submit(labels, inst, in_u8, cmap, label_nc, out, mode, row_slot, K, S, T, H, W, nullptr, stream);
+}
+
+extern "C" int v2v_label_image_io(const void* labels, const void* inst, int32_t in_u8, const uint8_t* cmap, int32_t label_nc,
+                                  uint8_t* out, const int32_t* mode, const int32_t* row_slot, int32_t K, int32_t S, int32_t T,
+                                  int32_t H, int32_t W, const v2v_frame_io* io, void* stream) {
+    if (!frame_io_arg_ok("label_image_io", io)) return V2V_EINVAL;
+    return label_image_submit(labels, inst, in_u8, cmap, label_nc, out, mode, row_slot, K, S, T, H, W, io, stream);
+}
diff --git a/vid2vid_amd/csrc/pointwise.hip b/vid2vid_amd/csrc/pointwise.hip
--- a/vid2vid_amd/csrc/pointwise.hip
+++ b/vid2vid_amd/csrc/pointwise.hip
@@ -351,19 +351,35 @@
     const float* window; void* packed; float* last;
     int T, H, W, label_nc, win_C, c_stride, last_C;
     int N = 1;
-};
-
-template <typename T, typename LT, typename IT>
-__device__ __forceinline__ void frame_prologue_row(const PrologueArgs& a, long long nb, long long wrow, unsigned block_dim,
-                                                   unsigned grid_dim) {
+    const v2v_frame_io* io = nullptr;
+};
+
+template <typename LT, typename IT, bool IO> struct PrologueMaps { const LT* labels; const IT* inst; long long lfs, ifs; };
+
+template <typename LT, typename IT, bool IO>
+__device__ __forceinline__ PrologueMaps<LT, IT, IO> prologue_maps(const PrologueArgs& a, long long nb) {
+    const long long hw = (long long)a.H * a.W;
+    if (IO) {
+        const v2v_frame_io& io = *a.io;
+        return {reinterpret_cast<const LT*>(io.labels) + nb * io.labels_sample_stride,
+                a.inst ? reinterpret_cast<const IT*>(io.inst) + nb * io.inst_sample_stride : nullptr,
+                io.labels_frame_stride, io.inst_frame_stride};
+    }
+    return {reinterpret_cast<const LT*>(a.labels) + nb * hw * a.T,
+            a.inst ? reinterpret_cast<const IT*>(a.inst) + nb * hw * a.T : nullptr, hw, hw};
+}
+
+template <typename T, typename LT, typename IT, bool IO>
+__device__ __forceinline__ void frame_prologue_row(const PrologueArgs& a, const PrologueMaps<LT, IT, IO> m, long long nb, long long wrow,
+                                                   unsigned block_dim, unsigned grid_dim) {
     constexpr int VEC = ElemTraits<T>::VEC;
     const long long hw = (long long)a.H * a.W;
     const long long ncode = hw * a.T;
     const int vpr = a.window ? a.c_stride / VEC : 0;
     const long long total = ncode + hw * vpr;
     const long long stride = (long long)grid_dim * block_dim;
-    const LT* labels = reinterpret_cast<const LT*>(a.labels) + nb * ncode;
-    const IT* inst = a.inst ? reinterpret_cast<const IT*>(a.inst) + nb * ncode : nullptr;
+    const LT* labels = m.labels;
+    const IT* inst = m.inst;
     unsigned char* codes = a.codes + nb * ncode;
     float* mask = a.mask ? a.mask + nb * hw : nullptr;
     const float* window = a.window ? a.window + wrow * a.win_C * hw : nullptr;
@@ -372,11 +388,11 @@
     for (long long e = (long long)blockIdx.x * block_dim + threadIdx.x; e < total; e += stride) {
         if (e < ncode) {
             const long long t = e / hw, q = e - t * hw;
-            const int lab = (int)labels[e];
+            const int lab = (int)labels[IO ? t * m.lfs + q : e];
             bool edge = false;
             if (inst) {
                 const int py = (int)(q / a.W), px = (int)(q - (long long)py * a.W);
-                const IT* ip = inst + t * hw;
+                const IT* ip = inst + t * (IO ? m.ifs : hw);
                 const IT ctr = ip[q];
                 if (px > 0)       edge |= ip[q - 1] != ctr;
                 if (px < a.W - 1) edge |= ip[q + 1] != ctr;
@@ -396,10 +412,10 @@
     }
 }
 
-template <typename T, typename LT, typename IT, bool BATCH>
+template <typename T, typename LT, typename IT, bool BATCH, bool IO>
 __global__ __launch_bounds__(256) void frame_prologue_kernel(const PrologueArgs a) {
     const long long nb = BATCH ? (long long)blockIdx.y : 0ll;
-    frame_prologue_row<T, LT, IT>(a, nb, nb, blockDim.x, gridDim.x);
+    frame_prologue_row<T, LT, IT, IO>(a, prologue_maps<LT, IT, IO>(a, nb), nb, nb, blockDim.x, gridDim.x);
 }
 
 struct PrologueOp : Op {
@@ -408,16 +424,16 @@
         const int vec = dtype == V2V_BF16 ? 8 : 4;
         const long long hw = (long long)a.H * a.W;
         const dim3 g(grid_for(hw * a.T + (a.window ? hw * (a.c_stride / vec) : 0)), (unsigned)a.N), b(256);
-        if (a.N > 1) return go<true>(g, b, s);
-        return go<false>(g, b, s);
-    }
-    template <bool BATCH> int go(dim3 g, dim3 b, hipStream_t s) {
+        if (a.io) return a.N > 1 ? go<true, true>(g, b, s) : go<false, true>(g, b, s);
+        return a.N > 1 ? go<true, false>(g, b, s) : go<false, false>(g, b, s);
+    }
+    template <bool BATCH, bool IO> int go(dim3 g, dim3 b, hipStream_t s) {
         if (in_u8) {
-            if (dtype == V2V_BF16) hipLaunchKernelGGL((frame_prologue_kernel<bf16_t, unsigned char, int, BATCH>), g, b, 0, s, a);
-            else                   hipLaunchKernelGGL((frame_prologue_kernel<float, unsigned char, int, BATCH>), g, b, 0, s, a);
+            if (dtype == V2V_BF16) hipLaunchKernelGGL((frame_prologue_kernel<bf16_t, unsigned char, int, BATCH, IO>), g, b, 0, s, a);
+            else                   hipLaunchKernelGGL((frame_prologue_kernel<float, unsigned char, int, BATCH, IO>), g, b, 0, s, a);
         } else {
-            if (dtype == V2V_BF16) hipLaunchKernelGGL((frame_prologue_kernel<bf16_t, float, float, BATCH>), g, b, 0, s, a);
-            else                   hipLaunchKernelGGL((frame_prologue_kernel<float, float, float, BATCH>), g, b, 0, s, a);
+            if (dtype == V2V_BF16) hipLaunchKernelGGL((frame_prologue_kernel<bf16_t, float, float, BATCH, IO>), g, b, 0, s, a);
+            else                   hipLaunchKernelGGL((frame_prologue_kernel<float, float, float, BATCH, IO>), g, b, 0, s, a);
         }
         return check_launch();
     }
@@ -432,7 +448,7 @@
     const int slot = s.row_slot[blockIdx.y];
     if (slot < 0 || slot >= s.S) return;
     __builtin_assume(a.window != nullptr);
-    frame_prologue_row<T, LT, IT>(a, blockIdx.y, slot, blockDim.x, gridDim.x);
+    frame_prologue_row<T, LT, IT, false>(a, prologue_maps<LT, IT, false>(a, blockIdx.y), blockIdx.y, slot, blockDim.x, gridDim.x);
 }
 
 struct ProloguePoolOp : Op {
@@ -582,6 +598,7 @@
     float* img_final; float* img_warp; const float* gx; const float* gy;
     int N, C, H, W, align_corners;
     float* roll = nullptr; int roll_slots = 0;
+    const v2v_frame_io* io = nullptr;
 };
 
 __device__ __forceinline__ void warp_blend_pixel(const WarpArgs& a, long long n, long long pix, bool do_warp, float* win) {
@@ -624,8 +641,10 @@
     return a.roll ? a.roll + n * a.roll_slots * a.C * a.H * a.W : nullptr;
 }
 
-template <bool ROLLB>
-__global__ __launch_bounds__(256) void warp_blend_kernel(const WarpArgs a) {
+template <bool ROLLB, bool IO>
+__global__ __launch_bounds__(256) void warp_blend_kernel(const WarpArgs a_) {
+    WarpArgs a = a_;
+    if (IO) a.img_final = reinterpret_cast<float*>(a_.io->fake_B);
     const long long hw = (long long)a.H * a.W;
     const long long total = (long long)a.N * hw;
     const long long stride = (long long)gridDim.x * blockDim.x;
@@ -639,8 +658,14 @@
     WarpArgs a;
     int launch(hipStream_t s) override {
         const dim3 g(grid_for((long long)a.N * a.H * a.W));
-        if (a.roll && a.N > 1) hipLaunchKernelGGL(warp_blend_kernel<true>, g, dim3(256), 0, s, a);
-        else                   hipLaunchKernelGGL(warp_blend_kernel<false>, g, dim3(256), 0, s, a);
+        const bool rollb = a.roll && a.N > 1;
+        if (a.io) {
+            if (rollb) hipLaunchKernelGGL((warp_blend_kernel<true, true>), g, dim3(256), 0, s, a);
+            else       hipLaunchKernelGGL((warp_blend_kernel<false, true>), g, dim3(256), 0, s, a);
+        } else {
+            if (rollb) hipLaunchKernelGGL((warp_blend_kernel<true, false>), g, dim3(256), 0, s, a);
+            else       hipLaunchKernelGGL((warp_blend_kernel<false, false>), g, dim3(256), 0, s, a);
+        }
         return check_launch();
     }
     const char* name() const override { return "warp_blend"; }
@@ -1360,6 +1385,19 @@
     return submit(std::move(op), stream);
 }
 
+extern "C" int v2v_warp_blend_roll_io(float* img_raw, const float* flow, const float* weight, const float* prev,
+                                      const float* fg, const float* mask, float* img_final, float* img_warp,
+                                      const float* gx, const float* gy, float* window, int32_t slots,
+                                      int32_t N, int32_t C, int32_t H, int32_t W, int32_t align_corners,
+                                      const v2v_frame_io* io, void* stream) {
+    if (!frame_io_arg_ok("warp_blend_roll_io", io)) return V2V_EINVAL;
+    auto op = std::make_unique<WarpOp>();
+    op->a = WarpArgs{img_raw, flow, weight, prev, fg, mask, img_final, img_warp, gx, gy, N, C, H, W, align_corners, window, slots};
+    if (!warp_roll_args_ok("warp_blend_roll_io", op->a, true, N, "rolled window")) return V2V_EINVAL;
+    op->a.io = io;
+    return submit(std::move(op), stream);
+}
+
 extern "C" int v2v_warp_blend_slots(float* img_raw, const float* flow, const float* weight, const float* prev,
                                     const float* fg, const float* mask, float* img_final, float* img_warp,
                                     const float* gx, const float* gy, float* window, int32_t slots, const int32_t* mode,
@@ -1460,6 +1498,22 @@
     op->dtype = dtype; op->in_u8 = in_u8;
     if (!prologue_args_ok("frame_prologue", op->a, in_u8, dtype)) return V2V_EINVAL;
     if (!window) op->a.packed = op->a.last = nullptr;
+    return submit(std::move(op), stream);
+}
+
+extern "C" int v2v_frame_prologue_io(const void* labels, const void* inst, int32_t in_u8, uint8_t* codes, float* mask,
+                                     const int32_t* fg_labels_dev, int32_t n_fg, int32_t N, int32_t T, int32_t H, int32_t W,
+                                     int32_t label_nc, const float* window, int32_t win_C, void* packed, int32_t c_stride,
+                                     float* last, int32_t last_C, int32_t dtype, const v2v_frame_io* io, void* stream) {
+    if (!frame_io_arg_ok("frame_prologue_io", io)) return V2V_EINVAL;
+    if (N < 1 || N > 65535) { set_error("frame_prologue_io: bad sample count %d", N); return V2V_EINVAL; }
+    auto op = std::make_unique<PrologueOp>();
+    op->a = PrologueArgs{labels, inst, codes, mask, fg_labels_dev, n_fg, window, packed, last,
+                         T, H, W, label_nc, win_C, c_stride, last_C, N};
+    op->dtype = dtype; op->in_u8 = in_u8;
+    if (!prologue_args_ok("frame_prologue_io", op->a, in_u8, dtype)) return V2V_EINVAL;
+    if (!window) op->a.packed = op->a.last = nullptr;
+    op->a.io = io;
     return submit(std::move(op), stream);
 }
 
diff --git a/vid2vid_amd/csrc/v2v_internal.h b/vid2vid_amd/csrc/v2v_internal.h
--- a/vid2vid_amd/csrc/v2v_internal.h
+++ b/vid2vid_amd/csrc/v2v_internal.h
@@ -99,6 +99,14 @@
     return 0;
 }
 
+inline bool frame_io_arg_ok(const char* who, const v2v_frame_io* io) {
+    static_assert(sizeof(v2v_frame_io) == 128, "v2v_frame_io is 128 bytes");
+    if (!io || (reinterpret_cast<uintptr_t>(io) & 15) != 0) {
+        set_error("%s: the frame I/O table is null or not 16-byte aligned", who); return false;
+    }
+    return true;
+}
+
 inline int64_t round_up(int64_t a, int64_t b) { return (a + b - 1) / b * b; }
 inline int64_t ceil_div(int64_t a, int64_t b) { return (a + b - 1) / b; }
 
diff --git a/vid2vid_amd/csrc/vgg_ops.hip b/vid2vid_amd/csrc/vgg_ops.hip
--- a/vid2vid_amd/csrc/vgg_ops.hip
+++ b/vid2vid_amd/csrc/vgg_ops.hip
@@ -139,16 +139,24 @@
     const char* name() const override { return bwd ? "avgpool2_planar_backward" : "avgpool2_planar"; }
 };
 
-struct OneHotArgs { const void* labels; const void* inst; float* out; int H, W, label_nc; long long in_stride = 0; int N = 1; };
-
-template <typename LT, typename IT, bool BATCH>
+struct OneHotArgs { const void* labels; const void* inst; float* out; int H, W, label_nc; long long in_stride = 0; int N = 1;
+                    int T = 1; const v2v_frame_io* io = nullptr; };
+
+template <typename LT, typename IT, bool BATCH, bool IO>
 __global__ __launch_bounds__(256) void onehot_planar_kernel(const OneHotArgs a) {
     const long long hw = (long long)a.H * a.W;
     const long long stride = (long long)gridDim.x * blockDim.x;
     const long long nb = BATCH ? (long long)blockIdx.y : 0ll;
     const LT* labels = reinterpret_cast<const LT*>(a.labels) + nb * a.in_stride;
     const IT* inst = a.inst ? reinterpret_cast<const IT*>(a.inst) + nb * a.in_stride : nullptr;
-    float* out = a.out + nb * (a.label_nc + (inst ? 1 : 0)) * hw;
+    float* out = a.out;
+    if (IO) {
+        const v2v_frame_io& io = *a.io;
+        labels = reinterpret_cast<const LT*>(io.labels) + nb * io.labels_sample_stride + (a.T - 1) * io.labels_frame_stride;
+        if (inst) inst = reinterpret_cast<const IT*>(io.inst) + nb * io.inst_sample_stride + (a.T - 1) * io.inst_frame_stride;
+        out = reinterpret_cast<float*>(io.real_A_last);
+    }
+    out += nb * (a.label_nc + (inst ? 1 : 0)) * hw;
     for (long long p = (long long)blockIdx.x * blockDim.x + threadIdx.x; p < hw; p += stride) {
         const int lab = (int)labels[p];
         for (int c = 0; c < a.label_nc; ++c) out[(long long)c * hw + p] = (c == lab) ? 1.f : 0.f;
@@ -169,12 +177,15 @@
     OneHotArgs a; int in_u8 = 0;
     int launch(hipStream_t s) override {
         const dim3 g(grid_for((long long)a.H * a.W), (unsigned)a.N), b(256);
-        if (a.N > 1) {
-            if (in_u8) hipLaunchKernelGGL((onehot_planar_kernel<unsigned char, int, true>), g, b, 0, s, a);
-            else       hipLaunchKernelGGL((onehot_planar_kernel<float, float, true>), g, b, 0, s, a);
+        if (a.io) {
+            if (in_u8) hipLaunchKernelGGL((onehot_planar_kernel<unsigned char, int, true, true>), g, b, 0, s, a);
+            else       hipLaunchKernelGGL((onehot_planar_kernel<float, float, true, true>), g, b, 0, s, a);
+        } else if (a.N > 1) {
+            if (in_u8) hipLaunchKernelGGL((onehot_planar_kernel<unsigned char, int, true, false>), g, b, 0, s, a);
+            else       hipLaunchKernelGGL((onehot_planar_kernel<float, float, true, false>), g, b, 0, s, a);
         } else {
-            if (in_u8) hipLaunchKernelGGL((onehot_planar_kernel<unsigned char, int, false>), g, b, 0, s, a);
-            else       hipLaunchKernelGGL((onehot_planar_kernel<float, float, false>), g, b, 0, s, a);
+            if (in_u8) hipLaunchKernelGGL((onehot_planar_kernel<unsigned char, int, false, false>), g, b, 0, s, a);
+            else       hipLaunchKernelGGL((onehot_planar_kernel<float, float, false, false>), g, b, 0, s, a);
         }
         return check_launch();
     }
@@ -243,3 +254,16 @@
     op->a = OneHotArgs{labels, inst, out, H, W, label_nc}; op->a.in_stride = in_stride; op->a.N = N; op->in_u8 = in_u8;
     return submit(std::move(op), stream);
 }
+
+extern "C" int v2v_onehot_planar_io(const void* labels, const void* inst, int32_t in_u8, float* out, int32_t N, int32_t T,
+                                    int32_t H, int32_t W, int32_t label_nc, const v2v_frame_io* io, void* stream) {
+    if (!frame_io_arg_ok("onehot_planar_io", io)) return V2V_EINVAL;
+    if (!labels || !out || N <= 0 || N > 65535 || T < 1 || H <= 0 || W <= 0 || label_nc <= 0 || (in_u8 != 0 && in_u8 != 1) ||
+        (in_u8 && label_nc > 256)) {
+        set_error("onehot_planar_io: bad argument"); return V2V_EINVAL;
+    }
+    auto op = std::make_unique<OneHotOp>();
+    op->a = OneHotArgs{labels, inst, out, H, W, label_nc}; op->a.in_stride = (int64_t)T * H * W; op->a.N = N; op->in_u8 = in_u8;
+    op->a.T = T; op->a.io = io;
+    return submit(std::move(op), stream);
+}
diff --git a/vid2vid_amd/csrc/visual_ops.hip b/vid2vid_amd/csrc/visual_ops.hip
--- a/vid2vid_amd/csrc/visual_ops.hip
+++ b/vid2vid_amd/csrc/visual_ops.hip
@@ -28,7 +28,13 @@
 struct FramesU8Args {
     const float* x; unsigned char* out; const int* mode; const int* row_slot;
     long long hw; int K, S, C, normalize;
-};
+    const v2v_frame_io* io = nullptr;
+};
+
+template <bool IO>
+__device__ __forceinline__ unsigned char* frames_u8_out(const FramesU8Args& a) {
+    return IO ? reinterpret_cast<unsigned char*>(a.io->image) : a.out;
+}
 
 __device__ __forceinline__ unsigned frames_u8_byte(float x, int normalize) {
     float v = normalize ? ((x + 1.f) / 2.f) * 255.f : x * 255.f;
@@ -45,13 +51,13 @@
     return -1;
 }
 
-template <int CC>
+template <int CC, bool IO>
 __global__ __launch_bounds__(256) void frames_u8_wide_kernel(const FramesU8Args a) {
     const int s = blockIdx.y;
     const int row = frames_u8_row(a, s);
     const long long nvec = a.hw >> 2;
     const long long stride = (long long)gridDim.x * blockDim.x;
-    unsigned* const out = reinterpret_cast<unsigned*>(a.out + (long long)s * a.hw * CC);
+    unsigned* const out = reinterpret_cast<unsigned*>(frames_u8_out<IO>(a) + (long long)s * a.hw * CC);
     const float* const x = a.x + (long long)(row < 0 ? 0 : row) * CC * a.hw;
     for (long long v = (long long)blockIdx.x * blockDim.x + threadIdx.x; v < nvec; v += stride) {
         unsigned w[CC];
@@ -73,12 +79,13 @@
     }
 }
 
+template <bool IO>
 __global__ __launch_bounds__(256) void frames_u8_scalar_kernel(const FramesU8Args a) {
     const int s = blockIdx.y;
     const int row = frames_u8_row(a, s);
     const long long total = a.hw * a.C;
     const long long stride = (long long)gridDim.x * blockDim.x;
-    unsigned char* const out = a.out + (long long)s * total;
+    unsigned char* const out = frames_u8_out<IO>(a) + (long long)s * total;
     const float* const x = a.x + (long long)(row < 0 ? 0 : row) * total;
     for (long long e = (long long)blockIdx.x * blockDim.x + threadIdx.x; e < total; e += stride) {
         unsigned char b = 0;
@@ -184,18 +191,19 @@
 struct FramesU8Op : Op {
     FramesU8Args a;
     bool wide;
-    int launch(hipStream_t s) override {
+    int launch(hipStream_t s) override { return a.io ? go<true>(s) : go<false>(s); }
+    template <bool IO> int go(hipStream_t s) {
         const dim3 b(256);
         if (wide) {
             const dim3 g(grid_for(a.hw >> 2, 256, 1024), (unsigned)a.S);
             switch (a.C) {
-                case 1: hipLaunchKernelGGL(frames_u8_wide_kernel<1>, g, b, 0, s, a); break;
-                case 2: hipLaunchKernelGGL(frames_u8_wide_kernel<2>, g, b, 0, s, a); break;
-                case 3: hipLaunchKernelGGL(frames_u8_wide_kernel<3>, g, b, 0, s, a); break;
-                default: hipLaunchKernelGGL(frames_u8_wide_kernel<4>, g, b, 0, s, a); break;
+                case 1: hipLaunchKernelGGL((frames_u8_wide_kernel<1, IO>), g, b, 0, s, a); break;
+                case 2: hipLaunchKernelGGL((frames_u8_wide_kernel<2, IO>), g, b, 0, s, a); break;
+                case 3: hipLaunchKernelGGL((frames_u8_wide_kernel<3, IO>), g, b, 0, s, a); break;
+                default: hipLaunchKernelGGL((frames_u8_wide_kernel<4, IO>), g, b, 0, s, a); break;
             }
         } else {
-            hipLaunchKernelGGL(frames_u8_scalar_kernel, dim3(grid_for(a.hw * a.C, 256, 1024), (unsigned)a.S), b, 0, s, a);
+            hipLaunchKernelGGL(frames_u8_scalar_kernel<IO>, dim3(grid_for(a.hw * a.C, 256, 1024), (unsigned)a.S), b, 0, s, a);
         }
         return check_launch();
     }
@@ -221,19 +229,31 @@
     return submit(std::move(op), stream);
 }
 
+static int frames_u8_submit(const char* who, const float* frames, uint8_t* out, const int32_t* mode, const int32_t* row_slot, int32_t K,
+                            int32_t S, int32_t C, int32_t H, int32_t W, int32_t normalize, const v2v_frame_io* io, void* stream) {
+    if (!frames || !out || K < 1 || S < K || S > 65535 || C < 1 || C > 4 || H < 1 || W < 1) {
+        set_error("%s: bad argument (1 <= K <= S <= 65535 rows / images, 1..4 planes)", who); return V2V_EINVAL;
+    }
+    if (!row_slot && K != S) { set_error("%s: without row_slot row k is image k: K == S", who); return V2V_EINVAL; }
+    const long long hw = (long long)H * W;
+    const unsigned char* const fb = reinterpret_cast<const unsigned char*>(frames);
+    if (fb + 4 * hw * C * K > out && fb < out + hw * C * S) { set_error("%s: out must not overlap frames", who); return V2V_EINVAL; }
+    auto op = std::make_unique<FramesU8Op>();
+    op->a = FramesU8Args{frames, out, mode, row_slot, hw, K, S, C, normalize};
+    op->wide = hw % 4 == 0 && reinterpret_cast<uintptr_t>(frames) % 16 == 0 && (io || reinterpret_cast<uintptr_t>(out) % 4 == 0);
+    op->a.io = io;
+    return submit(std::move(op), stream);
+}
+
 extern "C" int v2v_frames_u8(const float* frames, uint8_t* out, const int32_t* mode, const int32_t* row_slot, int32_t K, int32_t S,
                              int32_t C, int32_t H, int32_t W, int32_t normalize, void* stream) {
-    if (!frames || !out || K < 1 || S < K || S > 65535 || C < 1 || C > 4 || H < 1 || W < 1) {
-        set_error("frames_u8: bad argument (1 <= K <= S <= 65535 rows / images, 1..4 planes)"); return V2V_EINVAL;
-    }
-    if (!row_slot && K != S) { set_error("frames_u8: without row_slot row k is image k: K == S"); return V2V_EINVAL; }
-    const long long hw = (long long)H * W;
-    const unsigned char* const fb = reinterpret_cast<const unsigned char*>(frames);
-    if (fb + 4 * hw * C * K > out && fb < out + hw * C * S) { set_error("frames_u8: out must not overlap frames"); return V2V_EINVAL; }
-    auto op = std::make_unique<FramesU8Op>();
-    op->a = FramesU8Args{frames, out, mode, row_slot, hw, K, S, C, normalize};
-    op->wide = hw % 4 == 0 && reinterpret_cast<uintptr_t>(frames) % 16 == 0 && reinterpret_cast<uintptr_t>(out) % 4 == 0;
-    return submit(std::move(op), stream);
+    return frames_u8_submit("frames_u8", frames, out, mode, row_slot, K, S, C, H, W, normalize, nullptr, stream);
+}
+
+extern "C" int v2v_frames_u8_io(const float* frames, uint8_t* out, const int32_t* mode, const int32_t* row_slot, int32_t K, int32_t S,
+                                int32_t C, int32_t H, int32_t W, int32_t normalize, const v2v_frame_io* io, void* stream) {
+    if (!frame_io_arg_ok("frames_u8_io", io)) return V2V_EINVAL;
+    return frames_u8_submit("frames_u8_io", frames, out, mode, row_slot, K, S, C, H, W, normalize, io, stream);
 }
 
 extern "C" int v2v_tensor2label(const float* x, uint8_t* out, const uint8_t* cmap, int32_t n_label, int32_t C, int32_t H, int32_t W,
diff --git a/vid2vid_amd/engine.py b/vid2vid_amd/engine.py
--- a/vid2vid_amd/engine.py
+++ b/vid2vid_amd/engine.py
@@ -338,6 +338,7 @@
     def __init__(self):
         self.h = C.c_void_p(lib.v2v_plan_create())
         self.keep = []
+        self.io_entries = []
         self.graph_ready = False
 
     def __enter__(self):
@@ -439,6 +440,7 @@
         self._lane = 0
         self._sset = 0
         self.per_stream = False
+        self.blend_io = None
         self.last_rows_per_sample = 0
         self.twin_enabled = False
         self.pair_override = None
@@ -518,6 +520,14 @@
         if self.plan is not None:
             self.plan.label(text)
 
+    def _io_ptr(self, io, entry):
+        if io.dtype != torch.uint8 or io.numel() != 128 or not io.is_contiguous():
+            raise ValueError("%s: the frame I/O table is 128 contiguous bytes" % entry)
+        self._keep(io)
+        if self.plan is not None:
+            self.plan.io_entries.append(entry)
+        return _ptr(io)
+
     @property
     def _sk_counter(self):
         return self._sk_counters.get((0, 0))
@@ -662,7 +672,7 @@
         src.codes = codes
         return codes
 
-    def frame_prologue(self, src, H, W, fg_labels, want_mask, window=None, last_C=0, row_slot=None):
+    def frame_prologue(self, src, H, W, fg_labels, want_mask, window=None, last_C=0, row_slot=None, io=None):
         labels, inst, T = src.labels, src.inst, src.T
         N = labels.shape[0] if labels.dim() == 4 else 1
         u8 = labels.dtype == torch.uint8
@@ -694,10 +704,15 @@
             if last_C:
                 last = self.empty_f32(N, last_C, H, W)
         entry, pool = ("frame_prologue_batch", ()) if row_slot is None else ("frame_prologue_pool", (window.shape[0], _ptr(row_slot)))
+        tail = ()
+        if io is not None:
+            if row_slot is not None:
+                raise ValueError("frame_prologue: the frame I/O table goes with plain plans")
+            entry, tail = "frame_prologue_io", (self._io_ptr(io, "frame_prologue_io"),)
         check(getattr(lib, "v2v_" + entry)(_ptr(labels), _ptr(inst), int(u8), _ptr(codes), _ptr(mask), _ptr(fg),
                                            0 if fg is None else fg.numel(), N, T, H, W, src.label_nc, _ptr(window), *pool, win_C,
                                            _ptr(None if packed is None else packed.t), cs, _ptr(last), last_C, self.dtype,
-                                           _stream()), entry)
+                                           *tail, _stream()), entry)
         self.label("frame_prologue")
         src.codes = codes
         x0 = Act(torch.empty((N, H, W, pad_channels(T * per, self.dtype)), dtype=self.tdtype, device="meta"), T * per, onehot=src)
@@ -1810,8 +1825,21 @@
             self.label("instance_mean")
         return out
 
-    def onehot_planar(self, labels, inst, H, W, label_nc):
+    def onehot_planar(self, labels, inst, H, W, label_nc, io=None, out=None):
         per = label_nc + (1 if inst is not None else 0)
+        if io is not None:
+            N = labels.shape[0] if labels.dim() == 4 else 1
+            T = labels.shape[-3]
+            if not labels.is_contiguous() or (inst is not None and (not inst.is_contiguous() or inst.shape != labels.shape)):
+                raise ValueError("onehot_planar: dense maps (T, H, W) or (N, T, H, W), the same for labels and instance maps")
+            shape = (N, per, H, W) if labels.dim() == 4 else (per, H, W)
+            if out is None or tuple(out.shape) != shape or out.dtype != torch.float32 or not out.is_contiguous():
+                raise ValueError("onehot_planar: with the frame I/O table, out is the plan's fp32 buffer %s" % (shape,))
+            self._keep(out)
+            check(lib.v2v_onehot_planar_io(_ptr(labels), _ptr(inst), int(labels.dtype == torch.uint8), _ptr(out), N, T, H, W,
+                                           label_nc, self._io_ptr(io, "onehot_planar_io"), _stream()), "onehot_planar_io")
+            self.label("onehot_planar")
+            return out
         if labels.dim() == 3:
             N = labels.shape[0]
             if labels.stride(1) != W or labels.stride(2) != 1 or (inst is not None and inst.stride() != labels.stride()):
@@ -1836,7 +1864,7 @@
         self.label("avgpool3s2_planar")
         return out
 
-    def warp_blend(self, img_raw, flow, weight, prev, fg, mask, want_warp=False, roll=None, slot_mode=None, row_slot=None):
+    def warp_blend(self, img_raw, flow, weight, prev, fg, mask, want_warp=False, roll=None, slot_mode=None, row_slot=None, io=None):
         N, Cc, H, W = img_raw.shape
         if self._training() and any(t is not None and t.requires_grad for t in (img_raw, flow, weight, prev, fg)):
             from . import autograd as AG
@@ -1869,8 +1897,19 @@
             entry, extra = "warp_blend", (N,)
         else:
             entry, extra = ("warp_blend_roll", win) if roll.dim() == 4 else ("warp_blend_roll_batch", win + (N,))
+        tail = ()
+        if io is None and self.blend_io is not None:
+            io, final = self.blend_io
+            if tuple(final.shape) != (N, Cc, H, W) or final.dtype != torch.float32 or not final.is_contiguous():
+                raise ValueError("warp_blend: the plan's frame buffer is fp32 (N, C, H, W)")
+            self._keep(final)
+        if io is not None:
+            if roll is None or words:
+                raise ValueError("warp_blend: the frame I/O table goes with the rolling blend of a plain plan")
+            entry, extra, tail = "warp_blend_roll_io", win + (N,), (self._io_ptr(io, "warp_blend_roll_io"),)
         check(getattr(lib, "v2v_" + entry)(_ptr(img_raw), _ptr(flow), _ptr(weight), _ptr(prev), _ptr(fg), _ptr(mask), _ptr(final),
-                                           _ptr(warp), _ptr(gx), _ptr(gy), *extra, Cc, H, W, int(self.align_corners), _stream()), entry)
+                                           _ptr(warp), _ptr(gx), _ptr(gy), *extra, Cc, H, W, int(self.align_corners), *tail,
+                                           _stream()), entry)
         self.label("warp_blend")
         return final, warp
 
@@ -1904,7 +1943,7 @@
               "window_scatter_pool")
         self.label("window_scatter")
 
-    def frames_u8(self, frames, mode=None, row_slot=None, S=None, normalize=True):
+    def frames_u8(self, frames, mode=None, row_slot=None, S=None, normalize=True, io=None, out=None):
         K, Cc, H, W = frames.shape
         S = K if S is None else int(S)
         if frames.dtype != torch.float32 or not frames.is_contiguous():
@@ -1914,14 +1953,21 @@
                 raise ValueError("frames_u8: mode and row_slot are int32 (K,)")
             if t is not None:
                 self._keep(t)
-        out = torch.empty((S, H, W, Cc), dtype=torch.uint8, device=self.device)
+        if out is None:
+            out = torch.empty((S, H, W, Cc), dtype=torch.uint8, device=self.device)
+        elif tuple(out.shape) != (S, H, W, Cc) or out.dtype != torch.uint8 or not out.is_contiguous():
+            raise ValueError("frames_u8: out is uint8 (S, H, W, C)")
         self._keep(out)
-        check(lib.v2v_frames_u8(_ptr(frames), _ptr(out), _ptr(mode), _ptr(row_slot), K, S, Cc, H, W, int(bool(normalize)),
-                                _stream()), "frames_u8")
+        if io is not None:
+            check(lib.v2v_frames_u8_io(_ptr(frames), _ptr(out), _ptr(mode), _ptr(row_slot), K, S, Cc, H, W, int(bool(normalize)),
+                                       self._io_ptr(io, "frames_u8_io"), _stream()), "frames_u8_io")
+        else:
+            check(lib.v2v_frames_u8(_ptr(frames), _ptr(out), _ptr(mode), _ptr(row_slot), K, S, Cc, H, W, int(bool(normalize)),
+                                    _stream()), "frames_u8")
         self.label("frames_u8")
         return out
 
-    def label_image(self, labels, inst, label_nc, slot_mode=None, row_slot=None, S=None):
+    def label_image(self, labels, inst, label_nc, slot_mode=None, row_slot=None, S=None, io=None, out=None):
         if labels.dim() != 4 or not labels.is_contiguous() or labels.dtype not in (torch.uint8, torch.float32):
             raise ValueError("label_image: contiguous uint8 or fp32 label maps (K, T, H, W)")
         K, T, H, W = labels.shape
@@ -1941,12 +1987,19 @@
         if cmap is None:
             from .visual import labelcolormap
             cmap = self._label_cmaps[label_nc] = torch.from_numpy(labelcolormap(label_nc)[:label_nc].copy()).to(self.device)
-        out = torch.empty((S, H, W, 3), dtype=torch.uint8, device=self.device)
+        if out is None:
+            out = torch.empty((S, H, W, 3), dtype=torch.uint8, device=self.device)
+        elif tuple(out.shape) != (S, H, W, 3) or out.dtype != torch.uint8 or not out.is_contiguous():
+            raise ValueError("label_image: out is uint8 (S, H, W, 3)")
         for t in (labels, inst, cmap, out):
             if t is not None:
                 self._keep(t)
-        check(lib.v2v_label_image(_ptr(labels), _ptr(inst), int(u8), _ptr(cmap), label_nc, _ptr(out), _ptr(slot_mode), _ptr(row_slot),
-                                  K, S, T, H, W, _stream()), "label_image")
+        if io is not None:
+            check(lib.v2v_label_image_io(_ptr(labels), _ptr(inst), int(u8), _ptr(cmap), label_nc, _ptr(out), _ptr(slot_mode),
+                                         _ptr(row_slot), K, S, T, H, W, self._io_ptr(io, "label_image_io"), _stream()), "label_image_io")
+        else:
+            check(lib.v2v_label_image(_ptr(labels), _ptr(inst), int(u8), _ptr(cmap), label_nc, _ptr(out), _ptr(slot_mode),
+                                      _ptr(row_slot), K, S, T, H, W, _stream()), "label_image")
         self.label("label_image")
         return out
 
diff --git a/vid2vid_amd/frame_io.py b/vid2vid_amd/frame_io.py
--- /dev/null
+++ b/vid2vid_amd/frame_io.py
@@ -0,0 +1,62 @@
+import ctypes as C
+import os
+
+from .lib import FrameIO
+
+TABLE_BYTES = C.sizeof(FrameIO)
+RING_SLOTS = 32
+
+
+def enabled():
+    return os.environ.get("V2V_FRAME_IO", "1") != "0"
+
+
+class TensorInfo:
+    __slots__ = ("device", "dtype", "shape", "strides", "data_ptr", "itemsize")
+
+    def __init__(self, device, dtype, shape, strides, data_ptr, itemsize):
+        self.device, self.dtype, self.shape, self.strides = device, dtype, tuple(shape), tuple(strides)
+        self.data_ptr, self.itemsize = int(data_ptr), int(itemsize)
+
+    @classmethod
+    def of(cls, t):
+        return cls(t.device, t.dtype, t.shape, t.stride(), t.data_ptr(), t.element_size())
+
+
+def check_window(info, device, dtype, B, tG, H, W):
+    if info.device != device:
+        return "on %s, the plan runs on %s" % (info.device, device)
+    if info.dtype != dtype:
+        return "%s, the plan was built for %s" % (info.dtype, dtype)
+    if len(info.shape) != 5 or len(info.strides) != 5:
+        return "not (B, t, c, H, W)"
+    b, t, c, h, w = info.shape
+    if b != B or t < tG or c < 1 or (h, w) != (H, W):
+        return "shape %s, the plan takes (%d, >=%d, >=1, %d, %d)" % (info.shape, B, tG, H, W)
+    ss, fs, _, rs, ps = info.strides
+    if ps != 1 or rs != W:
+        return "rows are not dense (strides %s)" % (info.strides,)
+    if fs < H * W or (B > 1 and ss < (tG - 1) * fs + H * W):
+        return "frames or samples overlap (strides %s)" % (info.strides,)
+    if info.data_ptr == 0 or info.data_ptr % 16 != 0 or (fs * info.itemsize) % 16 != 0 or (B > 1 and (ss * info.itemsize) % 16 != 0):
+        return "the frames do not start on 16-byte boundaries"
+    return (ss if B > 1 else 0, fs, rs)
+
+
+def check_result(info, device, dtype, shape):
+    dense, n = [], 1
+    for d in reversed(shape):
+        dense.insert(0, n)
+        n *= d
+    return (info.device == device and info.dtype == dtype and info.shape == tuple(shape) and info.strides == tuple(dense)
+            and info.data_ptr != 0 and info.data_ptr % 16 == 0)
+
+
+def pack(labels, labels_strides, inst, inst_strides, fake_B, real_A_last, image, real_A_image):
+    t = FrameIO()
+    t.labels = labels or None
+    t.labels_sample_stride, t.labels_frame_stride, t.labels_row_stride = labels_strides
+    t.inst = inst or None
+    t.inst_sample_stride, t.inst_frame_stride, t.inst_row_stride = inst_strides if inst else (0, 0, 0)
+    t.fake_B, t.real_A_last, t.image, t.real_A_image = (fake_B or None, real_A_last or None, image or None, real_A_image or None)
+    return bytes(t)
diff --git a/vid2vid_amd/lib.py b/vid2vid_amd/lib.py
--- a/vid2vid_amd/lib.py
+++ b/vid2vid_amd/lib.py
@@ -60,6 +60,16 @@
         ("rows", C.c_int32), ("cols", C.c_int32), ("p_stride", C.c_int32), ("q_stride", C.c_int32),
         ("KH", C.c_int32), ("KW", C.c_int32), ("stride", C.c_int32), ("pad", C.c_int32), ("pad_mode", C.c_int32),
         ("dtype", C.c_int32), ("accumulate", C.c_int32),
+    ]
+
+
+class FrameIO(C.Structure):
+    _fields_ = [
+        ("labels", C.c_void_p), ("labels_sample_stride", C.c_int64), ("labels_frame_stride", C.c_int64),
+        ("labels_row_stride", C.c_int64),
+        ("inst", C.c_void_p), ("inst_sample_stride", C.c_int64), ("inst_frame_stride", C.c_int64), ("inst_row_stride", C.c_int64),
+        ("fake_B", C.c_void_p), ("real_A_last", C.c_void_p), ("image", C.c_void_p), ("real_A_image", C.c_void_p),
+        ("reserved", C.c_int64 * 4),
     ]
 
 
@@ -169,7 +179,12 @@
     "v2v_image_prologue": (C.c_int, [_P, _P, _I, _P, _I, _P, _I, _I, _I, _I, _I, _P, _I, _P, _I, _P, _I, _I, _P]),
     "v2v_image_prologue_slots": (C.c_int, [_P, _P, _I, _P, _I, _P, _I, _I, _I, _I, _I, _P, _I, _P, _I, _P, _I, _I, _P,
                                            _P, _P, _I, _I]),
-    "v2v_warp_blend_pool": (C.c_int, [_P] * 11 + [_I] + [_P, _P] + [_I] * 6 + [_P]),
+    "v2v_frame_prologue_io": (C.c_int, [_P, _P, _I, _P, _P, _P, _I, _I, _I, _I, _I, _I, _P, _I, _P, _I, _P, _I, _I, _P, _P]),
+    "v2v_warp_blend_roll_io": (C.c_int, [_P] * 11 + [_I] * 6 + [_P, _P]),
+    "v2v_onehot_planar_io": (C.c_int, [_P, _P, _I, _P, _I, _I, _I, _I, _I, _P, _P]),
+    "v2v_frames_u8_io": (C.c_int, [_P, _P, _P, _P, _I, _I, _I, _I, _I, _I, _P, _P]),
+    "v2v_label_image_io": (C.c_int, [_P, _P, _I, _P, _I, _P, _P, _P, _I, _I, _I, _I, _I, _P, _P]),
+    "v2v_warp_blend_pool": (C.c_int,[_P] * 11 + [_I] + [_P, _P] + [_I] * 6 + [_P]),
     "v2v_window_gather_pool": (C.c_int, [_P, _P, _P, _I, _I, _I, _I, _I, _I, _P]),
     "v2v_window_scatter_pool": (C.c_int, [_P, _P, _P, _I, _I, _I, _I, _I, _I, _P]),
     "v2v_resample_flow": (C.c_int, [_P, _P, _P, _P, _P, _I, _I, _I, _I, _I, _P]),
diff --git a/vid2vid_amd/models/vid2vid_model_G.py b/vid2vid_amd/models/vid2vid_model_G.py
--- a/vid2vid_amd/models/vid2vid_model_G.py
+++ b/vid2vid_amd/models/vid2vid_model_G.py
@@ -2,6 +2,7 @@
 
 import torch
 
+from .. import frame_io as FIO
 from .. import lib as L
 from .. import networks
 from ..engine import Act, Plan
@@ -99,6 +100,23 @@
             if dev.type == "cuda":
                 self._words_host = self._words_host.pin_memory()
         self.out = {}
+        self.io = self._io_cur = None
+        self.io_live = False
+        if FIO.enabled() and self.label_mode and not self.slots and pool is None and S == 1:
+            per = opt.label_nc + int(has_inst)
+            self.io = torch.zeros(FIO.TABLE_BYTES, dtype=torch.uint8, device=dev)
+            self.sinks = {"fake_B": torch.zeros(B, opt.output_nc, H, W, dtype=torch.float32, device=dev),
+                          "image": torch.zeros(B, H, W, opt.output_nc, dtype=torch.uint8, device=dev) if self.frames_u8 else None,
+                          "real_A_image": torch.zeros(B, H, W, 3, dtype=torch.uint8, device=dev) if self.real_A_u8 else None,
+                          "real_A_last": None if self.real_A_u8 else torch.zeros(*lead, per, H, W, dtype=torch.float32, device=dev)}
+            self._io_ring = torch.zeros(FIO.RING_SLOTS, FIO.TABLE_BYTES, dtype=torch.uint8)
+            if dev.type == "cuda":
+                self._io_ring = self._io_ring.pin_memory()
+            self._io_ring_np = self._io_ring.numpy()
+            self._io_events = [None] * FIO.RING_SLOTS
+            self._io_next, self._io_bytes, self._io_held = 0, None, ()
+            self.io_calls = {"direct": 0, "staged_labels": 0, "staged_inst": 0}
+            self.set_io()
         self.lanes = bool(int(getattr(opt, "lanes", os.environ.get("V2V_LANES", "1")))) and use_graph
         self.twin = bool(int(getattr(opt, "twin", os.environ.get("V2V_TWIN", "1"))))
         eng.lanes_enabled = self.lanes
@@ -291,7 +309,12 @@
             if self.pool is not None:
                 self.out["real_A_image"] = self.eng.label_image(labels, inst, opt.label_nc, self.slot_mode, self.row_slot, S=self.pool.S)
             else:
-                self.out["real_A_image"] = self.eng.label_image(labels, inst, opt.label_nc, self.slot_mode if self.slots else None)
+                io = self._io_cur
+                self.out["real_A_image"] = self.eng.label_image(labels, inst, opt.label_nc, self.slot_mode if self.slots else None,
+                                                                io=io, out=None if io is None else self.sinks["real_A_image"])
+        elif self._io_cur is not None:
+            self.out["real_A_last"] = self.eng.onehot_planar(self.labels, self.inst, self.H, self.W, self.model.opt.label_nc,
+                                                             io=self._io_cur, out=self.sinks["real_A_last"])
         else:
             self.out["real_A_last"] = self._real_A_last()
 
@@ -331,13 +354,19 @@
         else:
             if self.pool is not None:
                 prev = self._gathered(0)
+            io = self._io_cur = self.io if (self.io is not None and rolls) else None
+            self.io_live = io is not None
             x0, mask0, prev_act, last = eng.frame_prologue(src, H, W, opt.fg_labels, opt.fg, window=prev.view(self.B, -1, H, W),
-                                                           last_C=opt.output_nc)
+                                                           last_C=opt.output_nc, io=io)
 
         roll = prev if rolls else None
-        fake_B, flow, weight, raw, _, _, _ = netG.emit(eng, x0, prev_act, last, mask0, None, None, None, self.use_raw_only,
-                                                       tag="G0", roll=roll, side=self._emit_real_A,
-                                                       slot_mode=self.slot_mode, row_slot=row_slot)
+        eng.blend_io = None if self._io_cur is None else (self._io_cur, self.sinks["fake_B"])
+        try:
+            fake_B, flow, weight, raw, _, _, _ = netG.emit(eng, x0, prev_act, last, mask0, None, None, None, self.use_raw_only,
+                                                           tag="G0", roll=roll, side=self._emit_real_A,
+                                                           slot_mode=self.slot_mode, row_slot=row_slot)
+        finally:
+            eng.blend_io = None
         if roll is None:
             self._roll(prev, fake_B)
             if self.pool is not None:
@@ -391,7 +420,9 @@
         if self.pool is not None:
             self.out["image"] = self.eng.frames_u8(fake_B, self.slot_mode, self.row_slot, S=self.pool.S)
         else:
-            self.out["image"] = self.eng.frames_u8(fake_B, self.slot_mode if self.slots else None)
+            io = self._io_cur
+            self.out["image"] = self.eng.frames_u8(fake_B, self.slot_mode if self.slots else None, io=io,
+                                                   out=None if io is None else self.sinks["image"])
 
     def _gathered(self, si):
         dense = self.dense.get(si)
@@ -428,6 +459,33 @@
         if self._words.device.type == "cuda":
             self._words_copied = torch.cuda.Event()
             self._words_copied.record()
+
+    def set_io(self, labels=None, inst=None, results=None, held=()):
+        tG, H, W, B = self.model.opt.n_frames_G, self.H, self.W, self.B
+        own = ((tG * H * W if B > 1 else 0), H * W, W)
+        lab = labels if labels is not None else (self.labels.data_ptr(), own)
+        ins = inst if inst is not None else ((self.inst.data_ptr(), own) if self.inst is not None else (0, (0, 0, 0)))
+        dst = {}
+        for name, sink in self.sinks.items():
+            t = (results or {}).get(name)
+            dst[name] = t.data_ptr() if t is not None else (0 if sink is None else sink.data_ptr())
+        raw = FIO.pack(lab[0], lab[1], ins[0], ins[1], dst["fake_B"], dst["real_A_last"], dst["image"], dst["real_A_image"])
+        self._io_held = tuple(held)
+        if raw == self._io_bytes:
+            return
+        self._io_bytes = raw
+        if self.io.device.type != "cuda":
+            self.io.copy_(torch.frombuffer(bytearray(raw), dtype=torch.uint8))
+            return
+        import numpy as np
+        k = self._io_next
+        self._io_next = (k + 1) % FIO.RING_SLOTS
+        if self._io_events[k] is not None:
+            self._io_events[k].synchronize()
+        self._io_ring_np[k, :] = np.frombuffer(raw, dtype=np.uint8)
+        self.io.copy_(self._io_ring[k], non_blocking=True)
+        ev = self._io_events[k] = self._io_events[k] or torch.cuda.Event()
+        ev.record()
 
     def run(self):
         if self.eng.record_only:
@@ -634,6 +692,10 @@
                 return self._inference_slots(input_A, input_B, inst_A, act, rst, has_inst, u8, img, pic, lut)
             use_raw_only = bool(opt.no_first_img and self.is_first_frame)
             fp = self._frame_plan(H, W, in_ch, has_inst, use_raw_only, u8, B, frames_u8=img, inputs_u8=in_u8, real_A_u8=pic)
+            if fp.io_live and not self.is_first_frame and self._active_plan is fp:
+                return self._inference_direct(fp, input_A, inst_A, has_inst, img, pic)
+            if fp.io is not None:
+                fp.set_io()
             if not in_u8:
                 self._stage_inputs(fp, input_A, inst_A, has_inst, list(range(B)))
             if self.is_first_frame:
@@ -648,6 +710,33 @@
             self.fake_B_prev = fp.prev
             fp.run()
             return fp.out["image" if img else "fake_B"].clone(), fp.out["real_A_image" if pic else "real_A_last"].clone()
+
+    def _inference_direct(self, fp, input_A, inst_A, has_inst, img, pic):
+        tG, B, H, W = self.opt.n_frames_G, fp.B, fp.H, fp.W
+        sel = slice(None) if B > 1 else 0
+        named, held = [], []
+        for key, t, buf in (("labels", input_A, fp.labels), ("inst", inst_A if has_inst else None, fp.inst)):
+            if t is None:
+                named.append(None)
+                continue
+            ok = FIO.check_window(FIO.TensorInfo.of(t), buf.device, buf.dtype, B, tG, H, W)
+            if isinstance(ok, str):
+                buf.copy_(t[sel, :tG, 0].to(buf.device, buf.dtype, non_blocking=True))
+                fp.io_calls["staged_" + key] += 1
+                named.append(None)
+            else:
+                named.append((t.data_ptr(), ok))
+                held.append(t)
+        first, second = ("image" if img else "fake_B"), ("real_A_image" if pic else "real_A_last")
+        results = {name: torch.empty_like(fp.out[name]) for name in (first, second)}
+        for name, t in results.items():
+            if not FIO.check_result(FIO.TensorInfo.of(t), fp.out[name].device, fp.out[name].dtype, fp.out[name].shape):
+                raise RuntimeError("inference: the allocator returned a %s tensor the frame plan cannot write in place" % name)
+        fp.set_io(named[0], named[1], results, held)
+        fp.io_calls["direct"] += 1
+        self.fake_B_prev = fp.prev
+        fp.run()
+        return results[first], results[second]
 
     def _picture_channels(self, in_ch):
         return 3 if self.opt.label_nc != 0 or in_ch == 3 else 1
```

Result: no change. 400.5 frames/s, median of 4 (+0.7%).
